# jtschwar/tomo_TV

Measured on AMD Instinct MI355X. Metric: SART+TV Gvoxel-updates/s (ASD-POCS outer iterations x voxels, 512x512x512 x 90 tilts, at 1/2/4/8 GPU), higher is better.
Workload: dtype f32; 1 GPU; ASD-POCS iteration (SART sweep beta0=0.25 + 10 TV-GD steps) on ONE 512x512x512 volume, 90 tilts -70..70 deg (headline SART+TV 512^3x90 = BASELINE configs[2] shape), 512 slices on rank 0; volume=512x512x512, slices_per_gpu=512, nray=512, nproj=90, sub_slab_engines_per_gpu=1, sart_chains_per_engine=1

## Files before the change

### tomo_tv_amd/csrc/engine_api.inc

```


const char *tomo_last_error(void) { return g_err.c_str(); }

int tomo_device_count(int *count)
{
    if (!count) return fail(TOMO_ERR_ARG, "null count");
    int n = 0;
    hipError_t err = hipGetDeviceCount(&n);
    if (err != hipSuccess) { n = 0; (void)hipGetLastError(); }
    *count = n;
    return TOMO_OK;
}

int tomo_system_matrix(int nray, int nproj, const double *angles_rad, int64_t cap, float *rows, float *cols,
                       float *vals, int64_t *nnz)
{
    if (!angles_rad || !nnz) return fail(TOMO_ERR_ARG, "null argument");
    int rc = check_dims(1, nray, nproj);
    if (rc) return rc;
    Coo m;
    build_parallel_ray(nray, nproj, angles_rad, m);
    *nnz = m.ptr[m.nrow];
    if (cap == 0) return TOMO_OK;
    if (cap < *nnz || !rows || !cols || !vals) return fail(TOMO_ERR_ARG, "output capacity too small");
    for (int64_t r = 0; r < m.nrow; ++r)
        for (int64_t k = m.ptr[r]; k < m.ptr[r + 1]; ++k) { rows[k] = (float)r; cols[k] = (float)m.col[k]; vals[k] = m.val[k]; }
    return TOMO_OK;
}

int tomo_create(int nslice, int nray, int nproj, const double *angles_rad, int device, tomo_engine **out)
{
    if (!angles_rad || !out) return fail(TOMO_ERR_ARG, "null argument");
    int rc = check_dims(nslice, nray, nproj);
    if (rc) return rc;
    tomo_engine *e = new_engine(nslice, nray, nproj, device);
    const double t_begin = std::chrono::duration<double>(std::chrono::steady_clock::now().time_since_epoch()).count();
    e->angles.assign(angles_rad, angles_rad + nproj);
    Coo m;
    build_parallel_ray(nray, nproj, angles_rad, m);
    return finish_create(e, m, out, t_begin);
}

int tomo_create_from_matrix(int nslice, int nray, int nproj, int64_t nnz, const float *rows, const float *cols,
                            const float *vals, int device, tomo_engine **out)
{
    if (!rows || !cols || !vals || !out) return fail(TOMO_ERR_ARG, "null argument");
    int rc = check_dims(nslice, nray, nproj);
    if (rc) return rc;
    const double t_begin = std::chrono::duration<double>(std::chrono::steady_clock::now().time_since_epoch()).count();
    Coo m;
    std::string err;
    if (!coo_from_triplets((int64_t)nray * nproj, (int64_t)nray * nray, nnz, rows, cols, vals, m, err))
        return fail(TOMO_ERR_ARG, err);
    tomo_engine *e = new_engine(nslice, nray, nproj, device);
    return finish_create(e, m, out, t_begin);
}

static void free_geometry(tomo_engine *e)
{
    e->pool.release_life(GEOMETRY);
    e->rs_ok = false; e->rs_angs_cap = 0; e->rs_angs_host.clear(); e->seg_ready = false;
    e->pdhg_begun = false;
    e->yk_claim.valid = false;
    e->g_prev_valid = e->mom_p_ok = e->mom.set = false;
    e->geometry_released = true;
}

int tomo_destroy(tomo_engine *e)
{
    if (!e) return TOMO_OK;
    (void)hipSetDevice(e->device);
    if (e->stream) (void)hipStreamSynchronize(e->stream);
    if (e->aux) { (void)hipStreamSynchronize(e->aux); (void)hipStreamDestroy(e->aux); (void)hipEventDestroy(e->ev_fork); (void)hipEventDestroy(e->ev_join); }
    for (int u = 0; u < tomo_engine::MAX_CHAINS; ++u) if (e->sub_stream[u]) { (void)hipStreamSynchronize(e->sub_stream[u]); (void)hipStreamDestroy(e->sub_stream[u]); (void)hipEventDestroy(e->ev_sjoin[u]); }
    for (int w = 0; w < 2; ++w) if (e->fp_red_stream[w]) { (void)hipStreamSynchronize(e->fp_red_stream[w]); (void)hipStreamDestroy(e->fp_red_stream[w]); for (int h = 0; h < 2; ++h) { (void)hipEventDestroy(e->ev_fp_tile[w][h]); (void)hipEventDestroy(e->ev_fp_red[w][h]); } }
    comm_release(e);
    if (e->ev_sfork) (void)hipEventDestroy(e->ev_sfork);
    if (e->ev_peer) (void)hipEventDestroy(e->ev_peer);
    if (e->ev_snap) (void)hipEventDestroy(e->ev_snap);
    if (e->h_snap) (void)hipHostFree(e->h_snap);
    if (e->rs_abort) (void)hipHostFree(e->rs_abort);
    if (e->rs_done) (void)hipHostFree(e->rs_done);
    e->pool.release_all();
    for (auto &p : e->prof) { for (auto ev : p.ev) (void)hipEventDestroy(ev); if (p.ref) (void)hipEventDestroy(p.ref); }
    if (e->own_stream && e->stream) (void)hipStreamDestroy(e->stream);
    delete e;
    return TOMO_OK;
}

int tomo_release_geometry(tomo_engine *e)
{
    NEED(e);
    HIPCHK(hipStreamSynchronize(e->stream));
    if (e->aux) HIPCHK(hipStreamSynchronize(e->aux));
    for (int u = 0; u < tomo_engine::MAX_CHAINS; ++u) if (e->sub_stream[u]) HIPCHK(hipStreamSynchronize(e->sub_stream[u]));
    e->async_pending = false;
    free_geometry(e);
    return TOMO_OK;
}

int tomo_adopt_volumes(tomo_engine *dst, tomo_engine *src)
{
    if (!dst || !src) return fail(TOMO_ERR_ARG, "null engine");
    if (dst->nx != src->nx || dst->n != src->n || dst->sx != src->sx || dst->device != src->device) return fail(TOMO_ERR_ARG, "engines differ in slab shape or device");
    HIPCHK(hipSetDevice(dst->device));
    HIPCHK(hipStreamSynchronize(src->stream));
    if (src->aux) HIPCHK(hipStreamSynchronize(src->aux));
    for (int u = 0; u < tomo_engine::MAX_CHAINS; ++u) if (src->sub_stream[u]) HIPCHK(hipStreamSynchronize(src->sub_stream[u]));
    src->async_pending = false;
    HIPCHK(hipStreamSynchronize(dst->stream));
    for (int i = 0; i < TOMO_VOL_SLOTS; ++i) {
        if (!src->vol[i]) continue;
        if (dst->vol[i] && dst->pool.release(dst->vol[i])) return fail(TOMO_ERR_STATE, "a volume of the adopting engine is not its own");
        if (src->pool.move_to(dst->pool, src->vol[i], (void **)&dst->vol[i])) return fail(TOMO_ERR_STATE, "a volume of the adopted engine is not its own");
        src->vol[i] = nullptr;
    }
    dst->old_is_recon = src->old_is_recon;
    src->old_is_recon = false;
    for (int i = 0; i < TOMO_VOL_SLOTS; ++i) ++dst->vol_version[i];
    g_clear(dst);
    return TOMO_OK;
}

int tomo_set_stream(tomo_engine *e, void *hip_stream)
{
    NEED(e);
    HIPCHK(hipStreamSynchronize(e->stream));
    if (e->own_stream) { HIPCHK(hipStreamDestroy(e->stream)); e->own_stream = false; }
    e->stream = (hipStream_t)hip_stream;
    return TOMO_OK;
}

int tomo_synchronize(tomo_engine *e) { NEED(e); HIPCHK(hipStreamSynchronize(e->stream)); return TOMO_OK; }
int tomo_get_device(tomo_engine *e, int *device) { if (!e || !device) return fail(TOMO_ERR_ARG, "null"); *device = e->device; return TOMO_OK; }
int tomo_get_dims(tomo_engine *e, int *nslice, int *nray, int *nproj, int64_t *nnz)
{
    if (!e) return fail(TOMO_ERR_ARG, "null engine");
    if (nslice) *nslice = e->nx;
    if (nray) *nray = e->n;
    if (nproj) *nproj = e->np;
    if (nnz) *nnz = e->nnz;
    return TOMO_OK;
}

int tomo_sart_chain_count(tomo_engine *e, int *count)
{
    if (!e || !count) return fail(TOMO_ERR_ARG, "null");
    *count = chain_count(e);
    return TOMO_OK;
}

static int upload(tomo_engine *e, const float *host, float *dst, int64_t m)
{
    size_t bytes = (size_t)e->nx * m * sizeof(float);
    int rc = ensure_stage(e, bytes);
    if (rc) return rc;
    HIPCHK(hipMemcpyAsync(e->stage, host, bytes, hipMemcpyHostToDevice, e->stream));
    dim3 grid((unsigned)((m + 31) / 32), (unsigned)((e->sx + 31) / 32)), block(256);
    hipLaunchKernelGGL(k_transpose_in, grid, block, 0, e->stream, e->stage, dst, e->nx, m, e->sx);
    LAUNCHCHK();
    HIPCHK(hipStreamSynchronize(e->stream));
    return TOMO_OK;
}

static int download(tomo_engine *e, const float *src, float *host, int64_t m)
{
    size_t bytes = (size_t)e->nx * m * sizeof(float);
    int rc = ensure_stage(e, bytes);
    if (rc) return rc;
    dim3 grid((unsigned)((m + 31) / 32), (unsigned)((e->sx + 31) / 32)), block(256);
    hipLaunchKernelGGL(k_transpose_out, grid, block, 0, e->stream, src, e->stage, e->nx, m, e->sx);
    LAUNCHCHK();
    HIPCHK(hipMemcpyAsync(host, e->stage, bytes, hipMemcpyDeviceToHost, e->stream));
    HIPCHK(hipStreamSynchronize(e->stream));
    return TOMO_OK;
}

int tomo_set_sinogram(tomo_engine *e, int which, const float *b)
{
    NEED(e);
    if (!b) return fail(TOMO_ERR_ARG, "null sinogram");
    float *dst; int rc = sino_slot(e, which, &dst); if (rc) return rc;
    return upload(e, b, dst, e->nrows);
}

int tomo_set_tilt_series(tomo_engine *e, const float *b) { return tomo_set_sinogram(e, TOMO_SINO_B, b); }

int tomo_get_sinogram(tomo_engine *e, int which, float *out)
{
    NEED(e);
    if (!out) return fail(TOMO_ERR_ARG, "null output");
    if (which == TOMO_SINO_YK_MODEL) {
        const float *yk = projection_in_hand(e, TOMO_VOL_YK);
        if (!yk) return fail(TOMO_ERR_STATE, "no projection of the extrapolated point in hand (tomo_fista_project_yk)");
        return download(e, yk, out, e->nrows);
    }
    float *src;
    int rc = sino_slot(e, which, &src);
    if (rc) return rc;
    return download(e, src, out, e->nrows);
}

int tomo_set_volume(tomo_engine *e, int vol, const float *data)
{
    NEED(e);
    { int rc_ = order_after_async(e); if (rc_) return rc_; }
    float *dst; int rc = get_vol(e, vol, &dst); if (rc) return rc;
    if (!data) return fail(TOMO_ERR_ARG, "null volume");
    return upload(e, data, dst, e->npix);
}

int tomo_get_volume(tomo_engine *e, int vol, float *data)
{
    NEED(e);
    float *src; int rc = get_vol_ro(e, vol, &src); if (rc) return rc;
    if (!data) return fail(TOMO_ERR_ARG, "null volume");
    return download(e, src, data, e->npix);
}

int tomo_set_slice(tomo_engine *e, int vol, int s, const float *img)
{
    NEED(e);
    { int rc_ = order_after_async(e); if (rc_) return rc_; }
    float *dst; int rc = get_vol(e, vol, &dst); if (rc) return rc;
    if (s < 0 || s >= e->nx || !img) return fail(TOMO_ERR_ARG, "slice index out of range");
    if ((rc = ensure_stage(e, e->npix * sizeof(float)))) return rc;
    HIPCHK(hipMemcpyAsync(e->stage, img, e->npix * sizeof(float), hipMemcpyHostToDevice, e->stream));
    hipLaunchKernelGGL(k_scatter_slice, dim3((unsigned)((e->npix + 255) / 256)), dim3(256), 0, e->stream, e->stage, dst, e->npix, e->sx, s);
    LAUNCHCHK();
    HIPCHK(hipStreamSynchronize(e->stream));
    return TOMO_OK;
}

int tomo_get_slice(tomo_engine *e, int vol, int s, float *img)
{
    NEED(e);
    float *src; int rc = get_vol_ro(e, vol, &src); if (rc) return rc;
    if (s < 0 || s >= e->nx || !img) return fail(TOMO_ERR_ARG, "slice index out of range");
    if ((rc = ensure_stage(e, e->npix * sizeof(float)))) return rc;
    hipLaunchKernelGGL(k_gather_slice, dim3((unsigned)((e->npix + 255) / 256)), dim3(256), 0, e->stream, src, e->stage, e->npix, e->sx, s);
    LAUNCHCHK();
    HIPCHK(hipMemcpyAsync(img, e->stage, e->npix * sizeof(float), hipMemcpyDeviceToHost, e->stream));
    HIPCHK(hipStreamSynchronize(e->stream));
    return TOMO_OK;
}

int tomo_restart_recon(tomo_engine *e)
{
    NEED(e);
    { int rc_ = order_after_async(e); if (rc_) return rc_; }
    HIPCHK(hipMemsetAsync(e->vol[TOMO_VOL_RECON], 0, e->vol_elems() * sizeof(float), e->stream));
    if (e->vol[TOMO_VOL_YK]) HIPCHK(hipMemsetAsync(e->vol[TOMO_VOL_YK], 0, e->vol_elems() * sizeof(float), e->stream));
    if (e->vol[TOMO_VOL_RECON_OLD]) HIPCHK(hipMemsetAsync(e->vol[TOMO_VOL_RECON_OLD], 0, e->vol_elems() * sizeof(float), e->stream));
    e->old_is_recon = false;
    ++e->vol_version[TOMO_VOL_RECON]; ++e->vol_version[TOMO_VOL_YK]; ++e->vol_version[TOMO_VOL_RECON_OLD];
    return TOMO_OK;
}

int tomo_copy_volume(tomo_engine *e, int dst, int src)
{
    NEED(e);
    { int rc_ = order_after_async(e); if (rc_) return rc_; }
    float *d, *s; int rc;
    const bool g_src = g_is_projection_of(e, src);
    if ((rc = get_vol(e, dst, &d)) || (rc = get_vol_ro(e, src, &s))) return rc;
    if (d != s) HIPCHK(hipMemcpyAsync(d, s, e->vol_elems() * sizeof(float), hipMemcpyDeviceToDevice, e->stream));
    if (g_src && dst != src) { e->g_valid[1].vol = dst; e->g_valid[1].ver = e->vol_version[dst]; }
    return TOMO_OK;
}

int tomo_forward_projection(tomo_engine *e, int vol, int sino)
{
    NEED(e);
    { int rc_ = order_after_async(e); if (rc_) return rc_; }
    float *x, *g; int rc;
    if ((rc = get_vol_ro(e, vol, &x))) return rc;
    if ((rc = sino_slot(e, sino, &g))) return rc;
    if ((rc = launch_fp_all<FP_STORE>(e, x, nullptr, g))) return rc;
    if (sino == TOMO_SINO_G) g_set(e, vol);
    return TOMO_OK;
}

int tomo_back_projection(tomo_engine *e, int sino, int vol)
{
    NEED(e);
    float *x, *g; int rc;
    if ((rc = get_vol(e, vol, &x))) return rc;
    if ((rc = sino_slot(e, sino, &g))) return rc;
    return launch_bp_all(e, x, g, nullptr, 0.f, 1.f, 0);
}

int tomo_lipschitz(tomo_engine *e, float *L) { if (!e || !L) return fail(TOMO_ERR_ARG, "null"); *L = e->lipschitz; return TOMO_OK; }
int tomo_lipschitz_cimmino(tomo_engine *e, float *L) { if (!e || !L) return fail(TOMO_ERR_ARG, "null"); *L = e->lipschitz_cimmino; return TOMO_OK; }
int tomo_row_inner_product(tomo_engine *e) { if (!e) return fail(TOMO_ERR_ARG, "null engine"); return TOMO_OK;  }

int tomo_sirt_landweber(tomo_engine *e, int vol, float beta, int niter)
{
    NEED(e);
    float *x, *r; int rc;
    if ((rc = get_vol(e, vol, &x)) || (rc = get_sino(e, &e->sino[TOMO_SINO_R], &r))) return rc;
    for (int it = 0; it < niter; ++it) {
        if ((rc = launch_fp_all<FP_RESID>(e, x, e->sino[TOMO_SINO_B], r))) return rc;
        if ((rc = launch_bp_all(e, x, r, nullptr, 1.f, beta, 1))) return rc;
    }
    return TOMO_OK;
}

int tomo_sirt_cimmino(tomo_engine *e, int vol, float beta, int niter)
{
    NEED(e);
    float *x, *r; int rc;
    if ((rc = get_vol(e, vol, &x)) || (rc = get_sino(e, &e->sino[TOMO_SINO_R], &r))) return rc;
    for (int it = 0; it < niter; ++it) {
        if ((rc = launch_fp_all<FP_RESID_MUL>(e, x, e->sino[TOMO_SINO_B], r, e->d_rowinner))) return rc;
        if ((rc = launch_bp_all(e, x, r, nullptr, 1.f, beta / (float)e->nrows, 1))) return rc;
    }
    return TOMO_OK;
}

int tomo_sirt(tomo_engine *e, int vol, int niter) { return tomo_sirt_data(e, vol, TOMO_SINO_B, niter); }

int tomo_sirt_data(tomo_engine *e, int vol, int sino_b, int niter)
{
    NEED(e);
    float *x, *r, *b; int rc;
    const float *have = (niter > 0 && sino_b != TOMO_SINO_G) ? projection_in_hand(e, vol) : nullptr;
    const bool reuse = have != nullptr;
    if (reuse) { if ((rc = order_after_async(e))) return rc; }
    if ((rc = get_vol(e, vol, &x)) || (rc = get_sino(e, &e->sino[TOMO_SINO_R], &r)) || (rc = sino_slot(e, sino_b, &b))) return rc;
    for (int it = 0; it < niter; ++it) {
        if (it == 0 && reuse) { if ((rc = launch_sino_resid<FP_RESID_NORM>(e, b, have, r))) return rc; }
        else if ((rc = launch_fp_all<FP_RESID_NORM>(e, x, b, r))) return rc;
        if ((rc = launch_bp_all(e, x, r, e->d_colsum_all, 1.f, 1.f, 1))) return rc;
    }
    return TOMO_OK;
}

static std::mutex g_rs_mu;
static hipEvent_t g_rs_last[64] = {};

static int launch_sart_resident(tomo_engine *e, float *x, float beta, int64_t steps, const std::function<int(int64_t)> &angle_at, float *track,
                                std::vector<std::pair<int, int>> &failed)
{
    failed.clear();
    if (steps > (int64_t)1 << 24) return fail(TOMO_ERR_ARG, "too many SART steps in one call");
    const Chunks all = chunks64(e, whole(e));
    const int c0 = all.c0, nc = all.n;
    const int groups = std::max(1, std::min(e->rs_groups, nc)), rounds = (nc + groups - 1) / groups;
    {
        std::vector<int> seq((size_t)steps);
        for (int64_t k = 0; k < steps; ++k) seq[(size_t)k] = angle_at(k);
        if (seq != e->rs_angs_host) {
            HIPCHK(hipStreamSynchronize(e->stream));
            if ((size_t)steps > e->rs_angs_cap) {
                if (e->d_rs_angs) { e->pool.release(e->d_rs_angs); e->rs_angs_cap = 0; }
                if (int rc = dev_alloc(e, GEOMETRY, (void **)&e->d_rs_angs, (size_t)steps * sizeof(int), false)) return rc;
                e->rs_angs_cap = (size_t)steps;
            }
            HIPCHK(hipMemcpy(e->d_rs_angs, seq.data(), (size_t)steps * sizeof(int), hipMemcpyHostToDevice));
            e->rs_angs_host.swap(seq);
        }
    }
    const uint64_t need = (uint64_t)rounds * (uint64_t)steps;
    if ((uint64_t)e->rs_epoch + need + 16 > 0xFFFFFFFFull) {
        HIPCHK(hipMemsetAsync(e->rs_pb, 0, e->rs_pb_bytes, e->stream));
        HIPCHK(hipMemsetAsync(e->rs_rb, 0, e->rs_rb_bytes, e->stream));
        e->rs_epoch = 0;
    }
    if (c0 != 0 || nc != e->sxc / 64) return fail(TOMO_ERR_STATE, "the resident sweep covers the whole slab");
    if (e->rs_commit_dirty || e->rs_commit_base > 0x7F000000u) {
        HIPCHK(hipMemsetAsync(e->d_rs_commit, 0, (size_t)(e->sxc / 64) * sizeof(unsigned), e->stream));
        e->rs_commit_base = 0; e->rs_commit_dirty = false;
    }
    if (++e->rs_seq >= 0x7FFFFFF0u) { std::memset(e->rs_done, 0, (size_t)(e->sxc / 64) * sizeof(int)); e->rs_seq = 1; }
    RsArgs A{};
    A.x = x; A.b = e->cur_b; A.rowsum = e->d_rowsum; A.hdr = e->d_rs_hdr; A.cell = e->d_rs_cell; A.ts = e->d_rs_ts; A.rl = e->d_rs_rl;
    A.pb = e->rs_pb; A.rb = e->rs_rb; A.angs = e->d_rs_angs; A.track = track; A.part = e->d_part; A.abort_word = e->d_rs_abort; A.abort_host = e->rs_abort;
    A.commit = e->d_rs_commit; A.done_host = e->rs_done; A.seq = e->rs_seq; A.commit_base = e->rs_commit_base; A.test_fail = e->rs_test_fail;
    A.n = e->n; A.sx = e->sx; A.np = e->np; A.ntiles = e->rs_ntiles; A.tiles = e->rs_tiles; A.rpt = e->rs_rpt; A.steps = (int)steps; A.chunk0 = c0; A.nchunk = nc;
    A.epoch0 = e->rs_epoch; A.spin_limit = e->rs_spin_limit; A.beta = beta; A.prof = nullptr;
    e->rs_epoch += (uint32_t)need;
    if (e->device < 0 || e->device >= 64) return fail(TOMO_ERR_ARG, "device index");
    {
        std::lock_guard<std::mutex> lk(g_rs_mu);
        hipEvent_t &last = g_rs_last[e->device];
        if (!last) HIPCHK(hipEventCreateWithFlags(&last, hipEventDisableTiming));
        else HIPCHK(hipStreamWaitEvent(e->stream, last, 0));
        {
            ProfScope ps(e, TOMO_K_SART_RESIDENT);
            hipLaunchKernelGGL(k_sart_resident, dim3((unsigned)(e->rs_ntiles * groups)), dim3(RS_THREADS), 0, e->stream, A);
            LAUNCHCHK();
        }
        HIPCHK(hipEventRecord(last, e->stream));
    }
    HIPCHK(hipStreamSynchronize(e->stream));
    int nfailed = 0;
    for (int c = c0; c < c0 + nc; ++c) {
        if (e->rs_done[c] == (int)e->rs_seq) continue;
        ++nfailed;
        if (!failed.empty() && failed.back().first + failed.back().second == c) ++failed.back().second;
        else failed.emplace_back(c, 1);
    }
    if (nfailed) {
        e->rs_commit_dirty = true;
        e->rs_last_code = *e->rs_abort;
        *e->rs_abort = 0;
        HIPCHK(hipMemsetAsync(e->d_rs_abort, 0, sizeof(int), e->stream));
        ++e->rs_fallbacks;
        e->rs_fallback_chunks += nfailed;
        e->rs_backoff = std::min(64, std::max(1, 2 * e->rs_backoff));
        e->rs_skip = e->rs_backoff;
    } else {
        e->rs_commit_base += (unsigned)e->rs_ntiles;
        e->rs_backoff = 0;
    }
    return TOMO_OK;
}

int tomo_sart(tomo_engine *e, int vol, float beta, int niter, const int32_t *order)
{
    return tomo_sart_data(e, vol, TOMO_SINO_B, beta, niter, order);
}

static int sart_impl(tomo_engine *e, int vol, int sino_b, float beta, int niter, const int32_t *order, int track_vol, int slot)
{
    NEED(e);
    float *x, *r, *track = nullptr; int rc;
    if ((rc = get_vol(e, vol, &x)) || (rc = get_sino(e, &e->sino[TOMO_SINO_R], &r)) || (rc = sino_slot(e, sino_b, &e->cur_b))) return rc;
    if (track_vol >= 0) {
        if (track_vol == vol) return fail(TOMO_ERR_ARG, "the tracked volume must differ from the swept one");
        if (slot < 0 || slot >= TOMO_S_COUNT) return fail(TOMO_ERR_ARG, "bad scalar slot");
        if ((rc = get_vol(e, track_vol, &track))) return rc;
        if ((int64_t)niter * e->np <= 0) {
            if ((rc = tomo_diff_norm_sq(e, vol, track_vol, slot))) return rc;
            return tomo_copy_volume(e, track_vol, vol);
        }
        if ((rc = reduce_begin(e))) return rc;
    }
    auto finish = [&]() -> int { return track ? reduce_end(e, slot) : TOMO_OK; };
    if (order) {
        std::vector<char> seen(e->np, 0);
        for (int q = 0; q < e->np; ++q) {
            if (order[q] < 0 || order[q] >= e->np || seen[order[q]]) return fail(TOMO_ERR_ARG, "SART order is not a permutation of the angles");
            seen[order[q]] = 1;
        }
    }
    const int64_t steps = (int64_t)niter * e->np;
    auto angle_at = [&](int64_t k) { int q = (int)(k % e->np); return order ? order[q] : q; };
    if (!e->sart_fused) {
        for (int64_t k = 0; k < steps; ++k) {
            int i = angle_at(k);
            {
                ProfScope ps(e, TOMO_K_FP_ANGLE);
                if ((rc = launch_fp<FP_RESID_NORM>(e, x, i * e->n, e->n, e->cur_b, r))) return rc;
            }
            if ((rc = launch_bp_angle(e, x, i, r + (size_t)i * e->n * e->sx, beta, k == steps - 1 ? track : nullptr))) return rc;
        }
        return finish();
    }
    if (steps <= 0) return TOMO_OK;
    int form = select_forms(e).sart;
    if (form == TOMO_FORM_SART_RESIDENT && e->rs_skip > 0 && e->sart_resident != 1) {
        --e->rs_skip;
        form = TOMO_FORM_SART_TILE;
    }
    auto sweep_tiles = [&](const std::vector<std::pair<int, int>> *ranges) -> int {
        const bool coop = e->sart_coop && e->np >= 2 && steps >= 2 && !ranges;
        int rc2;
        if ((rc2 = sart_tile_prepare(e, coop))) return rc2;
        const uint32_t epoch0 = e->st_epoch + 1;
        if (coop) e->st_epoch += (uint32_t)(steps + 1);
        auto link = [&](int64_t k, const Sub &sb) -> int {
            int rc3;
            if (coop) {
                float *pk = (k & 1) ? e->st_partial2 : e->st_partial, *pk1 = (k & 1) ? e->st_partial : e->st_partial2;
                if (k == 0) return launch_sart_tile<false>(e, sb, x, 0, angle_at(0), r, beta, pk, false);
                if (k == steps) {
                    int last = angle_at(steps - 1);
                    if ((rc3 = launch_resid_finish_tile(e, sb, pk1, last, r))) return rc3;
                    return launch_bp_angle(e, sb, x, last, r + (size_t)last * e->n * e->sx, beta, track);
                }
                return launch_sart_coop(e, sb, x, angle_at(k - 1), angle_at(k), r, beta, pk1, pk, epoch0 + (uint32_t)k, k);
            }
            if (k == 0) return launch_sart_tile<false>(e, sb, x, 0, angle_at(0), r, beta);
            if (k == steps) { int last = angle_at(steps - 1); return launch_bp_angle(e, sb, x, last, r + (size_t)last * e->n * e->sx, beta, track); }
            int prev = angle_at(k - 1), next = angle_at(k);
            if (prev == next) {
                if ((rc3 = launch_bp_angle(e, sb, x, prev, r + (size_t)prev * e->n * e->sx, beta))) return rc3;
                return launch_sart_tile<false>(e, sb, x, 0, next, r, beta);
            }
            return launch_sart_tile<true>(e, sb, x, prev, next, r, beta, nullptr, true, k);
        };
        auto chain = [&](const Sub &sb) -> int {
            for (int64_t k = 0; k <= steps; ++k) { int rc3 = link(k, sb); if (rc3) return rc3; }
            return TOMO_OK;
        };
        if (!ranges) return run_chains(e, chain);
        for (const auto &rg : *ranges) {
            const int c0 = rg.first, nc = rg.second;
            const int vec = (c0 % 4 == 0 && nc % 4 == 0) ? 4 : (c0 % 2 == 0 && nc % 2 == 0) ? 2 : 1;
            if ((rc2 = chain(Sub{e->stream, c0, nc, vec}))) return rc2;
        }
        return TOMO_OK;
    };
    if (form == TOMO_FORM_SART_RESIDENT) {
        std::vector<std::pair<int, int>> failed;
        if ((rc = launch_sart_resident(e, x, beta, steps, angle_at, track, failed))) return rc;
        if (!failed.empty() && (rc = sweep_tiles(&failed))) return rc;
        return finish();
    }
    if (e->sart_resident == 1 && !e->rs_ok) return fail(TOMO_ERR_STATE, "\"sart_resident\" = 1, but this engine has no tables of the resident sweep (N not a multiple of 8, more 32 x 32 tiles than CUs, or a matrix whose ray windows do not fit)");
    if (form == TOMO_FORM_SART_TILE) {
        if ((rc = sweep_tiles(nullptr))) return rc;
        return finish();
    }
    float *alt;
    if ((rc = ensure_seg_tables(e))) return rc;
    if ((rc = get_scratch(e, &e->sart_alt, &alt))) return rc;
    float *cur = x;
    if ((rc = launch_sart_seg<false>(e, cur, nullptr, 0, angle_at(0), r, beta))) return rc;
    for (int64_t k = 1; k < steps; ++k) {
        int prev = angle_at(k - 1), next = angle_at(k);
        if (prev == next) {
            if ((rc = launch_bp_angle(e, cur, prev, r + (size_t)prev * e->n * e->sx, beta))) return rc;
            if ((rc = launch_fp<FP_RESID_NORM>(e, cur, next * e->n, e->n, e->cur_b, r))) return rc;
            continue;
        }
        if ((rc = launch_sart_seg<true>(e, cur, alt, prev, next, r, beta))) return rc;
        std::swap(cur, alt);
    }
    int last = angle_at(steps - 1);
    if ((rc = launch_bp_angle(e, cur, last, r + (size_t)last * e->n * e->sx, beta, track))) return rc;
    if (cur != x) { e->vol[vol] = cur; e->sart_alt = x; }
    return finish();
}

int tomo_sart_data(tomo_engine *e, int vol, int sino_b, float beta, int niter, const int32_t *order)
{
    return sart_impl(e, vol, sino_b, beta, niter, order, -1, 0);
}

int tomo_sart_tracked(tomo_engine *e, int vol, int sino_b, float beta, int niter, const int32_t *order, int track_vol, int slot)
{
    return sart_impl(e, vol, sino_b, beta, niter, order, track_vol, slot);
}

int tomo_art(tomo_engine *e, float beta) { return tomo_art_order(e, beta, nullptr); }

int tomo_art_order(tomo_engine *e, float beta, const int32_t *order_host)
{
    NEED(e);
    float *x;
    { int rc_ = get_vol(e, TOMO_VOL_RECON, &x); if (rc_) return rc_; }
    int32_t *d_order = nullptr;
    if (order_host) {
        std::vector<char> seen(e->nrows, 0);
        for (int64_t q = 0; q < e->nrows; ++q) {
            if (order_host[q] < 0 || order_host[q] >= e->nrows || seen[order_host[q]]) return fail(TOMO_ERR_ARG, "row order is not a permutation");
            seen[order_host[q]] = 1;
        }
        int rc = ensure_stage(e, e->nrows * sizeof(int32_t)); if (rc) return rc;
        HIPCHK(hipMemcpyAsync(e->stage, order_host, e->nrows * sizeof(int32_t), hipMemcpyHostToDevice, e->stream));
        d_order = (int32_t *)e->stage;
    }
    if (!order_host && e->art_chain && e->art_chain_ok) {
        float *d, *a; int rc;
        if ((rc = get_sino(e, &e->sino[TOMO_SINO_G], &d)) || (rc = get_sino(e, &e->sino[TOMO_SINO_R], &a))) return rc;
        const float *b = e->sino[TOMO_SINO_B];
        if (e->art_tile && e->sart_tile && e->st_ok && e->np >= 1) {
            if ((rc = sart_tile_prepare(e, false))) return rc;
            e->cur_b = const_cast<float *>(b);
            const int np = e->np;
            auto chain = [&](const Sub &sb) -> int {
                const Chunks ch = chunks64(e, sb);
                for (int i = 0; i < np; ++i) {
                    int rc2 = i == 0 ? launch_sart_tile<false, true>(e, sb, x, 0, 0, a, beta, nullptr, true, -1, d)
                                     : launch_sart_tile<true, true>(e, sb, x, i - 1, i, a, beta, nullptr, true, i, d);
                    if (rc2) return rc2;
                    hipLaunchKernelGGL(k_art_chain, dim3((unsigned)ch.n), dim3(64 * ART_CW), 0, sb.stream, d, b, e->d_rowinner, e->d_rowcross, a, beta, i * e->n, e->n, e->sx, ch.c0);
                    LAUNCHCHK();
                }
                return launch_bp_art(e, sb, x, np - 1, a, beta);
            };
            if ((rc = run_chains(e, chain))) return rc;
            return tomo_positivity(e, TOMO_VOL_RECON);
        }
        for (int i = 0; i < e->np; ++i) {
            if ((rc = launch_fp<FP_STORE>(e, x, i * e->n, e->n, nullptr, d))) return rc;
            hipLaunchKernelGGL(k_art_chain, dim3((unsigned)(e->sx / 64)), dim3(64 * ART_CW), 0, e->stream, d, b, e->d_rowinner, e->d_rowcross, a, beta, i * e->n, e->n, e->sx, 0);
            LAUNCHCHK();
            if ((rc = launch_bp_art(e, whole(e), x, i, a, beta))) return rc;
        }
        return tomo_positivity(e, TOMO_VOL_RECON);
    }
    hipLaunchKernelGGL(k_art, dim3(e->sxc / 64), dim3(64 * ART_WAVES), 0, e->stream, x, e->d_rptr, e->d_rent, e->sino[TOMO_SINO_B], e->d_rowinner, beta, (int)e->nrows, e->sx, d_order);
    LAUNCHCHK();
    int rc = tomo_positivity(e, TOMO_VOL_RECON);
    if (!rc && order_host) HIPCHK(hipStreamSynchronize(e->stream));
    return rc;
}

int tomo_poisson_ml(tomo_engine *e, float lambda)
{
    int rc;
    if ((rc = tomo_poisson_residual(e, TOMO_VOL_RECON, TOMO_SINO_B, TOMO_SINO_R))) return rc;
    float *x;
    if ((rc = get_vol(e, TOMO_VOL_RECON, &x))) return rc;
    return launch_bp_all(e, x, e->sino[TOMO_SINO_R], nullptr, 1.f, -(lambda / e->lipschitz), 1);
}

int tomo_poisson_residual(tomo_engine *e, int vol, int sino_b, int sino_out)
{
    NEED(e);
    float *x, *b, *r; int rc;
    if ((rc = get_vol(e, vol, &x)) || (rc = sino_slot(e, sino_b, &b)) || (rc = sino_slot(e, sino_out, &r))) return rc;
    if ((rc = reduce_begin(e))) return rc;
    if ((rc = launch_fp_all<FP_POISSON>(e, x, b, r))) return rc;
    return reduce_end(e, TOMO_S_COST);
}

static int slice_sumsq(tomo_engine *e, const float *v, int64_t m, double *sums)
{
    const int cols = e->sx / 4, per = cols >= 256 ? 256 : (cols >= 128 ? 128 : 64);
    const int nby = (int)std::min<int64_t>(1024, std::max<int64_t>(1, (m + 63) / 64));
    const int rpb = (int)((m + nby - 1) / nby);
    if (!e->cg_part) { int rc = dev_alloc(e, ENGINE, (void **)&e->cg_part, (size_t)1024 * e->sx * sizeof(double), false); if (rc) return rc; }
    dim3 grid((unsigned)((cols + per - 1) / per), (unsigned)nby);
    hipLaunchKernelGGL(k_slice_sumsq, grid, dim3(256), 0, e->stream, v, e->cg_part, m, e->sx, rpb);
    LAUNCHCHK();
    hipLaunchKernelGGL(k_slice_sumsq_finish, dim3((e->sx + 255) / 256), dim3(256), 0, e->stream, (const double *)e->cg_part, sums, nby, e->sx);
    LAUNCHCHK();
    return TOMO_OK;
}

static unsigned slice_grid(const tomo_engine *e, int64_t n4)
{
    const int64_t unit = std::max(1, e->sx / 64);
    int64_t b = std::min<int64_t>((n4 + 255) / 256, 8192);
    b = std::max<int64_t>(unit, (b / unit) * unit);
    return (unsigned)b;
}

int tomo_cgls(tomo_engine *e, int vol, int niter)
{
    NEED(e);
    float *x, *r, *b, *w; int rc;
    const bool reuse_g = g_is_projection_of(e, vol);
    if (reuse_g) { if ((rc = order_after_async(e))) return rc; }
    if ((rc = get_vol(e, vol, &x)) || (rc = get_sino(e, &e->sino[TOMO_SINO_R], &r)) || (rc = sino_slot(e, TOMO_SINO_B, &b))) return rc;
    if ((rc = get_scratch(e, &e->cg_p, &w)) || (rc = get_scratch(e, &e->cg_z, &w))) return rc;
    if ((rc = get_sino(e, &e->cg_w, &w))) return rc;
    if (!e->cg_sums) { if ((rc = dev_alloc(e, ENGINE, (void **)&e->cg_sums, 2 * e->sx * sizeof(double), true))) return rc; }
    if (!e->cg_coef) { if ((rc = dev_alloc(e, ENGINE, (void **)&e->cg_coef, e->sx * sizeof(float), true))) return rc; }
    double *gam = e->cg_sums, *tmp = e->cg_sums + e->sx;
    const int64_t nv = (int64_t)e->vol_elems(), ns = (int64_t)e->sino_elems();
    auto ratio = [&](const double *num, const double *den) {
        hipLaunchKernelGGL(k_slice_ratio, dim3((e->sx + 255) / 256), dim3(256), 0, e->stream, num, den, e->cg_coef, e->sx);
    };
    if (reuse_g) { if ((rc = launch_sino_resid<FP_RESID>(e, b, e->sino[TOMO_SINO_G], r))) return rc; }
    else if ((rc = launch_fp_all<FP_RESID>(e, x, b, r))) return rc;
    if ((rc = launch_bp_all(e, e->cg_z, r, nullptr, 0.f, 1.f, 0))) return rc;
// ... 21 lines not shown
    if (!taps_host) return fail(TOMO_ERR_ARG, "null filter");
    float *x, *b, *g; int rc;
    if ((rc = get_vol(e, TOMO_VOL_RECON, &x)) || (rc = sino_slot(e, TOMO_SINO_B, &b)) || (rc = get_sino(e, &e->sino[TOMO_SINO_R], &g))) return rc;
    if (!e->fbp_h) { if ((rc = dev_alloc(e, GEOMETRY, (void **)&e->fbp_h, e->n * sizeof(float), false))) return rc; }
    HIPCHK(hipMemcpyAsync(e->fbp_h, taps_host, e->n * sizeof(float), hipMemcpyHostToDevice, e->stream));
    HIPCHK(hipStreamSynchronize(e->stream));
    int nchunk = e->sxc / (64 * e->vec);
    int64_t waves = e->nrows * nchunk;
    dim3 grid((unsigned)((waves + 3) / 4)), block(256);
    with_vec(e->vec, [&](auto V) {
        hipLaunchKernelGGL((k_filter_rows<V()>), grid, block, 0, e->stream, b, g, e->fbp_h, e->n, (int)e->nrows, e->sx, nchunk);
    });
    LAUNCHCHK();
    return launch_bp_all(e, x, g, nullptr, 0.f, scale, apply_positivity ? 1 : 0);
}

int tomo_scale_volume(tomo_engine *e, int vol, float factor)
{
    NEED(e);
    { int rc_ = order_after_async(e); if (rc_) return rc_; }
    float *x; int rc; if ((rc = get_vol(e, vol, &x))) return rc;
    int64_t n4 = e->vol_elems() / 4;
    hipLaunchKernelGGL(k_scale, dim3(grid_1d(n4)), dim3(256), 0, e->stream, (f4 *)x, factor, n4);
    LAUNCHCHK();
    return TOMO_OK;
}

int tomo_sino_diff_norm_sq(tomo_engine *e, int a, int b, int slot)
{
    NEED(e);
    if (slot < 0 || slot >= TOMO_S_COUNT) return fail(TOMO_ERR_ARG, "bad scalar slot");
    float *pa, *pb; int rc;
    if ((rc = sino_slot(e, a, &pa)) || (rc = sino_slot(e, b, &pb))) return rc;
    if ((rc = reduce_begin(e))) return rc;
    int64_t n4 = e->sino_elems() / 4;
    hipLaunchKernelGGL(k_sqdiff, dim3(grid_1d(n4)), dim3(256), 0, e->stream, (const f4 *)pa, (const f4 *)pb, e->d_part, n4);
    LAUNCHCHK();
    return reduce_end(e, slot);
}

int tomo_sino_proj_max(tomo_engine *e, int sino, float *out_host)
{
    NEED(e);
    float *g; int rc; if ((rc = sino_slot(e, sino, &g))) return rc;
    if (!out_host) return fail(TOMO_ERR_ARG, "null output");
    if ((rc = ensure_stage(e, e->np * sizeof(float)))) return rc;
    hipLaunchKernelGGL(k_proj_max, dim3(e->np), dim3(256), 0, e->stream, g, e->stage, e->n, e->nx, e->sx);
    LAUNCHCHK();
    HIPCHK(hipMemcpyAsync(out_host, e->stage, e->np * sizeof(float), hipMemcpyDeviceToHost, e->stream));
    HIPCHK(hipStreamSynchronize(e->stream));
    return TOMO_OK;
}

int tomo_sino_proj_scale(tomo_engine *e, int sino, const float *div_host, const float *mul_host)
{
    NEED(e);
    float *g; int rc; if ((rc = sino_slot(e, sino, &g))) return rc;
    if (!div_host || !mul_host) return fail(TOMO_ERR_ARG, "null factors");
    if ((rc = ensure_stage(e, 2 * e->np * sizeof(float)))) return rc;
    HIPCHK(hipMemcpyAsync(e->stage, div_host, e->np * sizeof(float), hipMemcpyHostToDevice, e->stream));
    HIPCHK(hipMemcpyAsync(e->stage + e->np, mul_host, e->np * sizeof(float), hipMemcpyHostToDevice, e->stream));
    hipLaunchKernelGGL(k_proj_scale, dim3(e->np), dim3(256), 0, e->stream, g, e->stage, e->n, e->sx);
    LAUNCHCHK();
    HIPCHK(hipStreamSynchronize(e->stream));
    return TOMO_OK;
}

int tomo_copy_volume_from(tomo_engine *dst, int dst_vol, tomo_engine *src, int src_vol)
{
    if (!dst || !src) return fail(TOMO_ERR_ARG, "null engine");
    if (dst->nx != src->nx || dst->n != src->n || dst->sx != src->sx || dst->device != src->device) return fail(TOMO_ERR_ARG, "engines differ in slab shape or device");
    HIPCHK(hipSetDevice(dst->device));
    float *d, *s; int rc;
    if ((rc = get_vol(dst, dst_vol, &d)) || (rc = get_vol(src, src_vol, &s))) return rc;
    HIPCHK(hipStreamSynchronize(src->stream));
    HIPCHK(hipMemcpyAsync(d, s, dst->vol_elems() * sizeof(float), hipMemcpyDeviceToDevice, dst->stream));
    HIPCHK(hipStreamSynchronize(dst->stream));
    return TOMO_OK;
}

int tomo_get_stream(tomo_engine *e, void **out) { if (!e || !out) return fail(TOMO_ERR_ARG, "null"); *out = (void *)e->stream; return TOMO_OK; }

static int mm_check(tomo_engine *a, tomo_engine *b, int nel)
{
    if (!a || !b) return fail(TOMO_ERR_ARG, "null engine");
    if (a->nx != b->nx || a->n != b->n || a->sx != b->sx || a->device != b->device) return fail(TOMO_ERR_ARG, "engines differ in slab shape or device");
    if (a->stream != b->stream) return fail(TOMO_ERR_STATE, "engines must share one stream (tomo_set_stream)");
    if (nel < 1 || nel > MM_MAX_EL) return fail(TOMO_ERR_ARG, "element count out of range");
    return TOMO_OK;
}

int tomo_mm_model(tomo_engine *ce, const int32_t *xvols, int nel, const float *w, float gamma, tomo_engine *he, int model_vol)
{
    int rc = mm_check(ce, he, nel); if (rc) return rc;
    HIPCHK(hipSetDevice(ce->device));
    MMArgs a{};
    a.nel = nel; a.gamma = gamma;
    for (int i = 0; i < nel; ++i) { float *p; if ((rc = get_vol(ce, xvols[i], &p))) return rc; a.x[i] = p; a.w[i] = w[i]; }
    float *m; if ((rc = get_vol(he, model_vol, &m))) return rc;
    int64_t n4 = ce->vol_elems() / 4;
    hipLaunchKernelGGL(k_mm_model, dim3(grid_1d(n4)), dim3(256), 0, ce->stream, a, (f4 *)m, n4);
    LAUNCHCHK();
    return TOMO_OK;
}

int tomo_mm_update(tomo_engine *ce, const int32_t *xvols, const int32_t *uvols, int nel, const float *w, float gamma,
                   float lamC_over_L, float lamH, tomo_engine *he, int upd_vol, int model_vol)
{
    int rc = mm_check(ce, he, nel); if (rc) return rc;
    HIPCHK(hipSetDevice(ce->device));
    MMArgs a{};
    a.nel = nel; a.gamma = gamma;
    for (int i = 0; i < nel; ++i) {
        float *p, *u;
        if ((rc = get_vol(ce, xvols[i], &p)) || (rc = get_vol(ce, uvols[i], &u))) return rc;
        a.x[i] = p; a.u[i] = u; a.w[i] = w[i];
    }
    float *upd = nullptr, *m = nullptr;
    if (lamH != 0.f) { if ((rc = get_vol(he, upd_vol, &upd)) || (rc = get_vol(he, model_vol, &m))) return rc; }
    int64_t n4 = ce->vol_elems() / 4;
    hipLaunchKernelGGL(k_mm_update, dim3(grid_1d(n4)), dim3(256), 0, ce->stream, a, (const f4 *)upd, (const f4 *)m, lamC_over_L, lamH, n4);
    LAUNCHCHK();
    return TOMO_OK;
}

int tomo_positivity(tomo_engine *e, int vol)
{
    NEED(e);
    { int rc_ = order_after_async(e); if (rc_) return rc_; }
    float *x; int rc; if ((rc = get_vol(e, vol, &x))) return rc;
    int64_t n4 = e->vol_elems() / 4;
    hipLaunchKernelGGL(k_clamp, dim3(grid_1d(n4)), dim3(256), 0, e->stream, (f4 *)x, n4);
    LAUNCHCHK();
    return TOMO_OK;
}

int tomo_soft_threshold(tomo_engine *e, int vol, float lambda)
{
    NEED(e);
    float *x; int rc; if ((rc = get_vol(e, vol, &x))) return rc;
    int64_t n4 = e->vol_elems() / 4;
    hipLaunchKernelGGL(k_soft_threshold, dim3(grid_1d(n4)), dim3(256), 0, e->stream, (f4 *)x, lambda, n4);
    LAUNCHCHK();
    return TOMO_OK;
}

int tomo_fista_momentum(tomo_engine *e, float beta)
{
    NEED(e);
    { int rc_ = order_after_async(e); if (rc_) return rc_; }
    e->mom_p_ok = e->g_prev_valid && e->mom.set && e->vol_version[TOMO_VOL_RECON] == e->mom.ver_recon
                  && e->vol_version[TOMO_VOL_RECON_OLD] == e->mom.ver_old && e->g_prev_recon_ver == e->vol_version[TOMO_VOL_RECON];
    float *x, *yk, *old; int rc;
    const bool aliased = e->old_is_recon;
    if ((rc = get_vol_ro(e, TOMO_VOL_RECON, &x)) || (rc = get_vol_ro(e, TOMO_VOL_YK, &yk))) return rc;
    if (aliased) old = x;
    else if ((rc = get_vol_ro(e, TOMO_VOL_RECON_OLD, &old))) return rc;
    int64_t n4 = e->vol_elems() / 4;
    hipLaunchKernelGGL(k_momentum, dim3(grid_1d(n4)), dim3(256), 0, e->stream, (const f4 *)yk, (const f4 *)old, (f4 *)x, beta, n4);
    LAUNCHCHK();
    ++e->vol_version[TOMO_VOL_RECON]; ++e->vol_version[TOMO_VOL_YK]; ++e->vol_version[TOMO_VOL_RECON_OLD];
    e->vol[TOMO_VOL_RECON] = yk;
    e->vol[TOMO_VOL_YK] = x;
    e->old_is_recon = true;
    e->mom.beta = beta; e->mom.set = true;
    e->mom.ver_recon = e->vol_version[TOMO_VOL_RECON]; e->mom.ver_yk = e->vol_version[TOMO_VOL_YK]; e->mom.ver_old = e->vol_version[TOMO_VOL_RECON_OLD];
    return TOMO_OK;
}

int tomo_fista_project_yk(tomo_engine *e, int *done)
{
    NEED(e);
    if (done) *done = 0;
    if (!e->fp_reuse || !g_is_projection_of(e, TOMO_VOL_RECON) || !e->mom.set) return TOMO_OK;
    if (e->vol_version[TOMO_VOL_RECON] != e->mom.ver_recon || e->vol_version[TOMO_VOL_YK] != e->mom.ver_yk) return TOMO_OK;
    { int rc_ = order_after_async(e); if (rc_) return rc_; }
    int rc; float *p, *q;
    if ((rc = get_sino(e, &e->g_prev, &p)) || (rc = get_sino(e, &e->g_yk, &q))) return rc;
    const float *g = e->sino[TOMO_SINO_G];
    const int64_t n4 = (int64_t)e->sino_elems() / 4;
    const bool have_prev = e->mom_p_ok;
    e->yk_claim.valid = false;
    if (have_prev) {
        hipLaunchKernelGGL(k_sino_extrapolate, dim3(grid_1d(n4)), dim3(256), 0, e->stream, (const VecOf<4>::T *)g, (VecOf<4>::T *)p, (VecOf<4>::T *)q, e->mom.beta, n4);
        LAUNCHCHK();
    } else {
        HIPCHK(hipMemcpyAsync(p, g, e->sino_elems() * sizeof(float), hipMemcpyDeviceToDevice, e->stream));
    }
    e->g_prev_valid = true;
    e->g_prev_recon_ver = e->vol_version[TOMO_VOL_RECON];
    if (have_prev) {
        e->yk_claim.valid = true; e->yk_claim.ver = e->vol_version[TOMO_VOL_YK];
        if (done) *done = 1;
    } else if (e->mom.beta == 0.f) {
        e->g_valid[1].vol = TOMO_VOL_YK; e->g_valid[1].ver = e->vol_version[TOMO_VOL_YK];
        if (done) *done = 1;
    }
    return TOMO_OK;
}

int tomo_data_distance_sq(tomo_engine *e, int vol)
{
    NEED(e);
    float *x, *g; int rc;
    if ((rc = get_vol_ro(e, vol, &x)) || (rc = get_sino(e, &e->sino[TOMO_SINO_G], &g))) return rc;
    if ((rc = reduce_begin(e))) return rc;
    if ((rc = launch_fp_all<FP_DD>(e, x, e->sino[TOMO_SINO_B], g))) return rc;
    g_set(e, vol);
    return reduce_end(e, TOMO_S_DD);
}

int tomo_data_distance_sq_async(tomo_engine *e, int vol)
{
    NEED(e);
    if (e->async_pending) return fail(TOMO_ERR_STATE, "an asynchronous evaluation is already in flight");
    if (!e->aux) {
        HIPCHK(hipStreamCreateWithFlags(&e->aux, hipStreamNonBlocking));
        HIPCHK(hipEventCreateWithFlags(&e->ev_fork, hipEventDisableTiming));
        HIPCHK(hipEventCreateWithFlags(&e->ev_join, hipEventDisableTiming));
        if (int rc = dev_alloc(e, ENGINE, (void **)&e->d_part_aux, NPART * sizeof(double), true)) return rc;
    }
    float *tmp; int rc;
    if ((rc = get_vol_ro(e, vol, &tmp)) || (rc = get_sino(e, &e->sino[TOMO_SINO_G], &tmp))) return rc;
    HIPCHK(hipEventRecord(e->ev_fork, e->stream));
    HIPCHK(hipStreamWaitEvent(e->aux, e->ev_fork, 0));
    hipStream_t main_stream = e->stream;
    double *main_part = e->d_part;
    e->stream = e->aux; e->d_part = e->d_part_aux;
    rc = tomo_data_distance_sq(e, vol);
    e->stream = main_stream; e->d_part = main_part;
    if (rc) return rc;
    HIPCHK(hipEventRecord(e->ev_join, e->aux));
    e->async_pending = true;
    return TOMO_OK;
}

int tomo_async_wait(tomo_engine *e)
{
    NEED(e);
    if (e->async_pending) {
        HIPCHK(hipStreamWaitEvent(e->stream, e->ev_join, 0));
        e->async_pending = false;
    }
    return TOMO_OK;
}

int tomo_diff_norm_sq(tomo_engine *e, int a, int b, int slot)
{
    NEED(e);
    if (slot < 0 || slot >= TOMO_S_COUNT) return fail(TOMO_ERR_ARG, "bad scalar slot");
    float *pa, *pb; int rc;
    if ((rc = get_vol_ro(e, a, &pa)) || (rc = get_vol_ro(e, b, &pb))) return rc;
    if ((rc = reduce_begin(e))) return rc;
    int64_t n4 = e->vol_elems() / 4;
    hipLaunchKernelGGL(k_sqdiff, dim3(grid_1d(n4)), dim3(256), 0, e->stream, (const f4 *)pa, (const f4 *)pb, e->d_part, n4);
    LAUNCHCHK();
    return reduce_end(e, slot);
}

int tomo_l1_norm(tomo_engine *e, int vol)
{
    NEED(e);
    float *x; int rc; if ((rc = get_vol_ro(e, vol, &x))) return rc;
    if ((rc = reduce_begin(e))) return rc;
    int64_t n4 = e->vol_elems() / 4;
    hipLaunchKernelGGL(k_l1, dim3(grid_1d(n4)), dim3(256), 0, e->stream, (const f4 *)x, e->d_part, n4);
    LAUNCHCHK();
    return reduce_end(e, TOMO_S_L1);
}

int tomo_read_scalars(tomo_engine *e, double *out, int count)
{
    NEED(e);
    if (!out || count < 0 || count > TOMO_S_COUNT) return fail(TOMO_ERR_ARG, "bad scalar count");
    { int rc = tomo_async_wait(e); if (rc) return rc; }
    HIPCHK(hipMemcpyAsync(out, e->d_scal, count * sizeof(double), hipMemcpyDeviceToHost, e->stream));
    HIPCHK(hipStreamSynchronize(e->stream));
    return TOMO_OK;
}

int tomo_scalars_snapshot(tomo_engine *e)
{
    NEED(e);
    { int rc = tomo_async_wait(e); if (rc) return rc; }
    if (!e->h_snap) {
        HIPCHK(hipHostMalloc((void **)&e->h_snap, TOMO_S_COUNT * sizeof(double), hipHostMallocDefault));
        HIPCHK(hipEventCreateWithFlags(&e->ev_snap, hipEventDisableTiming));
    }
    hipLaunchKernelGGL(k_scalars_to_host, dim3(1), dim3(64), 0, e->stream, (const double *)e->d_scal, e->h_snap, (int)TOMO_S_COUNT);
    LAUNCHCHK();
    HIPCHK(hipEventRecord(e->ev_snap, e->stream));
    e->snap_pending = true;
    return TOMO_OK;
}

int tomo_scalars_snapshot_read(tomo_engine *e, double *out, int count)
{
    NEED(e);
    if (!out || count < 0 || count > TOMO_S_COUNT) return fail(TOMO_ERR_ARG, "bad scalar count");
    if (!e->snap_pending) return fail(TOMO_ERR_STATE, "no scalar snapshot in flight");
    HIPCHK(hipEventSynchronize(e->ev_snap));
    std::memcpy(out, e->h_snap, count * sizeof(double));
    e->snap_pending = false;
    return TOMO_OK;
}

// ... 8 lines not shown
```

### tomo_tv_amd/csrc/engine_options.inc

```

int tomo_get_option(tomo_engine *e, const char *name, int *value)
{
    if (!e || !name || !value) return fail(TOMO_ERR_ARG, "null argument");
    if (std::strcmp(name, "fp_strip") == 0) { *value = e->fp_strip; return TOMO_OK; }
    if (std::strcmp(name, "fp_strip_ready") == 0) { *value = e->fs_ok ? 1 : 0; return TOMO_OK; }
    if (std::strcmp(name, "fp_strip_slots") == 0) { *value = e->fs_ok ? e->fs_kused : 0; return TOMO_OK; }
    if (std::strcmp(name, "fp_tile") == 0) { *value = e->fp_tile; return TOMO_OK; }
    if (std::strcmp(name, "bp_tile") == 0) { *value = e->bp_tile; return TOMO_OK; }
    if (std::strcmp(name, "bp_list") == 0) { *value = e->bp_list; return TOMO_OK; }
    if (std::strcmp(name, "fgp_pair") == 0) { *value = e->fgp_pair; return TOMO_OK; }
    if (std::strcmp(name, "fp_list") == 0) { *value = e->fp_list; return TOMO_OK; }
    if (std::strcmp(name, "fp_list_ready") == 0) { *value = e->fl_ok ? 1 : 0; return TOMO_OK; }
    if (std::strcmp(name, "bp_list_ready") == 0) { *value = e->bl_ok ? 1 : 0; return TOMO_OK; }
    if (std::strcmp(name, "fp_reuse") == 0) { *value = e->fp_reuse; return TOMO_OK; }
    if (std::strcmp(name, "art_chain_ready") == 0) { *value = e->art_chain_ok ? 1 : 0; return TOMO_OK; }
    if (std::strcmp(name, "sart_tile") == 0) { *value = e->sart_tile; return TOMO_OK; }
    if (std::strcmp(name, "sart_resident") == 0) { *value = e->sart_resident; return TOMO_OK; }
    if (std::strcmp(name, "sart_resident_ready") == 0) { *value = e->rs_ok ? 1 : 0; return TOMO_OK; }
    if (std::strcmp(name, "sart_resident_active") == 0) { *value = (e->rs_ok && e->sart_resident != 0) ? 1 : 0; return TOMO_OK; }
    if (std::strcmp(name, "sart_resident_spin") == 0) { *value = (int)std::min<uint32_t>(e->rs_spin_limit, 0x7FFFFFFFu); return TOMO_OK; }
    if (std::strcmp(name, "sart_resident_fallbacks") == 0) { *value = e->rs_fallbacks; return TOMO_OK; }
    if (std::strcmp(name, "sart_resident_fallback_chunks") == 0) { *value = e->rs_fallback_chunks; return TOMO_OK; }
    if (std::strcmp(name, "sart_resident_skip") == 0) { *value = e->rs_skip; return TOMO_OK; }
    if (std::strcmp(name, "sart_resident_last_code") == 0) { *value = e->rs_last_code; return TOMO_OK; }
    if (std::strcmp(name, "table_kib") == 0) { *value = (int)std::min<size_t>(e->table_bytes >> 10, 0x7FFFFFFF); return TOMO_OK; }
    if (std::strcmp(name, "create_ms") == 0) { *value = (int)std::min(e->create_ms + 0.5, 2147483647.0); return TOMO_OK; }
    if (std::strcmp(name, "tv_halo_fold") == 0) { *value = e->tv_halo_fold; return TOMO_OK; }
    if (std::strcmp(name, "form_fp") == 0) { *value = select_forms(e).fp; return TOMO_OK; }
    if (std::strcmp(name, "form_bp") == 0) { *value = select_forms(e).bp; return TOMO_OK; }
    if (std::strcmp(name, "form_sart") == 0) { *value = select_forms(e).sart; return TOMO_OK; }
    if (std::strcmp(name, "rccl_version") == 0) { *value = g_rccl.version; return TOMO_OK; }
    if (std::strcmp(name, "comm_rounds") == 0) { *value = (int)std::min<int64_t>(e->comm_rounds, 0x7FFFFFFF); return TOMO_OK; }
    return fail(TOMO_ERR_ARG, std::string("unknown option ") + name);
}

int tomo_set_option(tomo_engine *e, const char *name, int value)
{
    if (!e || !name) return fail(TOMO_ERR_ARG, "null argument");
    if (std::strcmp(name, "fgp_fused") == 0) { e->fgp_fused = value ? 1 : 0; return TOMO_OK; }
    if (std::strcmp(name, "fgp_pair") == 0) { e->fgp_pair = value ? 1 : 0; return TOMO_OK; }
    if (std::strcmp(name, "sart_fused") == 0) { e->sart_fused = value ? 1 : 0; return TOMO_OK; }
    if (std::strcmp(name, "fp_all_lpr") == 0) { e->fp_all_lpr = (value == 16 || value == 32) ? value : 0; return TOMO_OK; }
    if (std::strcmp(name, "art_chain") == 0) { e->art_chain = value ? 1 : 0; return TOMO_OK; }
    if (std::strcmp(name, "sart_tile") == 0) { e->sart_tile = value ? 1 : 0; return TOMO_OK; }
    if (std::strcmp(name, "sart_resident") == 0) { e->sart_resident = value < 0 ? -1 : (value ? 1 : 0); e->rs_skip = e->rs_backoff = 0; return TOMO_OK; }
    if (std::strcmp(name, "sart_resident_spin") == 0) { e->rs_spin_limit = value < 0 ? (1u << 21) : (uint32_t)value; return TOMO_OK; }
    if (std::strcmp(name, "sart_resident_test_fail") == 0) { e->rs_test_fail = std::max(0, value); return TOMO_OK; }
    if (std::strcmp(name, "fp_reuse") == 0) { e->fp_reuse = value != 0; g_clear(e); e->yk_claim.valid = false; return TOMO_OK; }
    if (std::strcmp(name, "fp_tile_pipe") == 0) { e->fp_tile_pipe = std::max(0, value); return TOMO_OK; }
    if (std::strcmp(name, "sart_streams") == 0) { e->sart_streams = value >= 2 ? std::min(value, (int)tomo_engine::MAX_CHAINS) : (value == 1 ? 1 : 0); return TOMO_OK; }
    if (std::strcmp(name, "art_tile") == 0) { e->art_tile = value ? 1 : 0; return TOMO_OK; }
    if (std::strcmp(name, "sart_skip_same") == 0) { e->sart_skip_same = value ? 1 : 0; return TOMO_OK; }
    if (std::strcmp(name, "sart_nt") == 0) { e->sart_nt = value < 0 ? -1 : (value ? 1 : 0); return TOMO_OK; }
    if (std::strcmp(name, "sart_coop") == 0) { e->sart_coop = value ? 1 : 0; return TOMO_OK; }
    if (std::strcmp(name, "sart_coop_spin") == 0) { e->sart_coop_spin = value < 0 ? -1 : value; return TOMO_OK; }
    if (std::strcmp(name, "bp_tile") == 0) { e->bp_tile = value ? 1 : 0; return TOMO_OK; }
    if (std::strcmp(name, "bp_list") == 0) { e->bp_list = value ? 1 : 0; return TOMO_OK; }
    if (std::strcmp(name, "bp_list_band") == 0) { e->bp_list_band = value ? 1 : 0; return TOMO_OK; }
    if (std::strcmp(name, "fp_list") == 0) { e->fp_list = value ? 1 : 0; return TOMO_OK; }
    if (std::strcmp(name, "fp_strip") == 0) { e->fp_strip = value ? 1 : 0; return TOMO_OK; }
    if (std::strcmp(name, "fp_tile") == 0) { e->fp_tile = value ? 1 : 0; e->fp_strip = 0; return TOMO_OK; }
    if (std::strcmp(name, "fp_tile_chunks_per_pass") == 0) {
        if (value < 0 || e->ft_part || e->ft_part_aux || e->fs_part || e->fs_part_aux || e->fl_part || e->fl_part_aux) return fail(TOMO_ERR_STATE, "fp_tile_chunks_per_pass must be set before the first projection");
        e->ft_ncp_forced = value; e->ft_ncp = 0; e->fs_ncp = 0; e->fl_ncp = 0; return TOMO_OK;
    }
    if (std::strcmp(name, "fp_tile_scratch_mib") == 0) {
        if (value <= 0 || e->ft_part || e->ft_part_aux || e->fs_part || e->fs_part_aux || e->fl_part || e->fl_part_aux) return fail(TOMO_ERR_STATE, "fp_tile_scratch_mib must be positive and set before the first projection");
        e->ft_scratch_cap = (size_t)value << 20; e->ft_ncp = 0; e->fs_ncp = 0; e->fl_ncp = 0; return TOMO_OK;
    }
    if (std::strcmp(name, "tv_gnorm_slot") == 0) {
        if (value < 0 || value >= TOMO_S_COUNT) return fail(TOMO_ERR_ARG, "bad scalar slot");
        e->gnorm_slot = value; return TOMO_OK;
    }
    if (std::strcmp(name, "tv_tz") == 0) { e->tv_tz = value == 4 ? 4 : 8; return TOMO_OK; }
    if (std::strcmp(name, "tv_halo_fold") == 0) { e->tv_halo_fold = value < 0 ? -1 : (value ? 1 : 0); return TOMO_OK; }
    if (std::strcmp(name, "tv_march4") == 0) { e->tv_march4 = value ? 1 : 0; return TOMO_OK; }
    if (std::strcmp(name, "tv_yseg") == 0) { e->tv_yseg = value < 0 ? 0 : value; return TOMO_OK; }
    if (std::strcmp(name, "tv_recompute") == 0) { e->tv_recompute = value ? 1 : 0; return TOMO_OK; }
    if (std::strcmp(name, "tv_lds") == 0) { e->tv_lds = value; return TOMO_OK; }
    return fail(TOMO_ERR_ARG, std::string("unknown option ") + name);
}

int tomo_profile_enable(tomo_engine *e, int kernel, int on)
{
    NEED(e);
    if (kernel < 0 || kernel >= PROF_MAX_KERNELS) return fail(TOMO_ERR_ARG, "bad kernel id");
    HIPCHK(hipStreamSynchronize(e->stream));
    e->prof[kernel].on = on != 0;
    e->prof[kernel].stride = on > 1 ? (unsigned)on : 1u;
    e->prof[kernel].seen = 0;
    e->prof[kernel].used = 0;
    e->prof[kernel].dropped = 0;
    if (on) {
        if (!e->prof[kernel].ref) HIPCHK(hipEventCreate(&e->prof[kernel].ref));
        HIPCHK(hipEventRecord(e->prof[kernel].ref, e->stream));
    }
    return TOMO_OK;
}

int tomo_profile_read2(tomo_engine *e, int kernel, int64_t *launches, double *total_ms, double *busy_ms)
{
    NEED(e);
    if (kernel < 0 || kernel >= PROF_MAX_KERNELS || !launches || !total_ms) return fail(TOMO_ERR_ARG, "bad argument");
    HIPCHK(hipStreamSynchronize(e->stream));
    for (int u = 0; u < tomo_engine::MAX_CHAINS; ++u) if (e->sub_stream[u]) HIPCHK(hipStreamSynchronize(e->sub_stream[u]));
    if (e->aux) HIPCHK(hipStreamSynchronize(e->aux));
    ProfSlot &p = e->prof[kernel];
    double tot = 0;
    std::vector<std::pair<float, float>> iv;
    for (size_t i = 0; i + 1 < p.used; i += 2) {
        float ms = 0;
        HIPCHK(hipEventElapsedTime(&ms, p.ev[i], p.ev[i + 1]));
        tot += ms;
        if (busy_ms && p.ref) {
            float t0 = 0;
            HIPCHK(hipEventElapsedTime(&t0, p.ref, p.ev[i]));
            iv.emplace_back(t0, t0 + ms);
        }
    }
    if (busy_ms) {
        std::sort(iv.begin(), iv.end());
        double busy = 0; float cur_a = 0, cur_b = -1;
        for (auto &q : iv) {
            if (cur_b < cur_a || q.first > cur_b) { if (cur_b >= cur_a) busy += cur_b - cur_a; cur_a = q.first; cur_b = q.second; }
            else cur_b = std::max(cur_b, q.second);
        }
        if (cur_b >= cur_a) busy += cur_b - cur_a;
        *busy_ms = busy;
    }
    *launches = (int64_t)(p.used / 2);
    *total_ms = tot;
    p.used = 0;
    if (p.dropped) {
        std::string msg = std::to_string(p.dropped) + " launches were not recorded (event log full)";
        p.dropped = 0;
        return fail(TOMO_ERR_STATE, msg);
    }
    return TOMO_OK;
}

int tomo_profile_intervals(tomo_engine *e, int kernel, tomo_engine *ref_engine, double *t0, double *t1, int cap, int *count)
{
    NEED(e);
    if (kernel < 0 || kernel >= PROF_MAX_KERNELS || !ref_engine || !count) return fail(TOMO_ERR_ARG, "bad argument");
    HIPCHK(hipStreamSynchronize(e->stream));
    ProfSlot &p = e->prof[kernel];
    hipEvent_t ref = ref_engine->prof[kernel].ref;
    if (!ref) return fail(TOMO_ERR_STATE, "the reference engine's log is not enabled");
    int n = (int)(p.used / 2);
    *count = n;
    if (!t0 || !t1 || cap < n) return cap == 0 ? TOMO_OK : fail(TOMO_ERR_ARG, "interval buffers too small");
    for (int i = 0; i < n; ++i) {
        float a = 0, d = 0;
        HIPCHK(hipEventElapsedTime(&a, ref, p.ev[2 * i]));
        HIPCHK(hipEventElapsedTime(&d, p.ev[2 * i], p.ev[2 * i + 1]));
        t0[i] = a; t1[i] = a + d;
    }
    return TOMO_OK;
}

int tomo_profile_read(tomo_engine *e, int kernel, int64_t *launches, double *total_ms)
{
    return tomo_profile_read2(e, kernel, launches, total_ms, nullptr);
}
```

### tomo_tv_amd/csrc/engine_tv.inc

```

static int field_ptr(tomo_engine *e, int field, float **out)
{
    if (field == TOMO_FIELD_FGP_D) return get_scratch(e, &e->tvg, out);
    if (field == TOMO_FIELD_FGP_P1) return get_scratch(e, &e->fgp_p[0], out);
    return get_vol_ro(e, field, out);
}

int tomo_bind_halo(tomo_engine *e, void *device_lo, void *device_hi)
{
    NEED(e);
    HIPCHK(hipStreamSynchronize(e->stream));
    e->halo_lo = device_lo ? (float *)device_lo : e->halo_lo_own;
    e->halo_hi = device_hi ? (float *)device_hi : e->halo_hi_own;
    return TOMO_OK;
}

int tomo_halo_pack(tomo_engine *e, int field, int last, void *device_dst)
{
    NEED(e);
    float *x; int rc; if ((rc = field_ptr(e, field, &x))) return rc;
    if (!device_dst) return fail(TOMO_ERR_ARG, "null destination");
    hipLaunchKernelGGL(k_halo_pack, dim3((unsigned)((e->npix + 255) / 256)), dim3(256), 0, e->stream, x, (float *)device_dst, (int)e->npix, e->sx, last ? e->nx - 1 : 0);
    LAUNCHCHK();
    return TOMO_OK;
}

int tomo_halo_pack_both(tomo_engine *e, int field, void *first_plane, void *last_plane)
{
    NEED(e);
    float *x; int rc; if ((rc = field_ptr(e, field, &x))) return rc;
    if (!first_plane || !last_plane) return fail(TOMO_ERR_ARG, "null destination");
    hipLaunchKernelGGL(k_halo_wrap, dim3((unsigned)((e->npix + 255) / 256)), dim3(256), 0, e->stream, x, (float *)last_plane, (float *)first_plane, (int)e->npix, e->sx, e->nx);
    LAUNCHCHK();
    return TOMO_OK;
}

int tomo_halo_local(tomo_engine *e, int field)
{
    NEED(e);
    float *x; int rc; if ((rc = field_ptr(e, field, &x))) return rc;
    hipLaunchKernelGGL(k_halo_wrap, dim3((unsigned)((e->npix + 255) / 256)), dim3(256), 0, e->stream, x, e->halo_lo, e->halo_hi, (int)e->npix, e->sx, e->nx);
    LAUNCHCHK();
    return TOMO_OK;
}


int tomo_wait_for(tomo_engine *e, tomo_engine *other)
{
    NEED(e);
    if (!other) return fail(TOMO_ERR_ARG, "null engine");
    if (other->device != e->device) return fail(TOMO_ERR_ARG, "engines on different devices");
    if (other == e || other->stream == e->stream) return TOMO_OK;
    if (!other->ev_peer) HIPCHK(hipEventCreateWithFlags(&other->ev_peer, hipEventDisableTiming));
    HIPCHK(hipEventRecord(other->ev_peer, other->stream));
    HIPCHK(hipStreamWaitEvent(e->stream, other->ev_peer, 0));
    return TOMO_OK;
}

int tomo_halo_from(tomo_engine *e, int field, tomo_engine *lo_src, tomo_engine *hi_src)
{
    NEED(e);
    if (!lo_src || !hi_src) return fail(TOMO_ERR_ARG, "null engine");
    if (lo_src->n != e->n || hi_src->n != e->n || lo_src->device != e->device || hi_src->device != e->device) return fail(TOMO_ERR_ARG, "engines differ in image size or device");
    float *xl, *xh; int rc;
    if ((rc = field_ptr(lo_src, field, &xl)) || (rc = field_ptr(hi_src, field, &xh))) return rc;
    dim3 grid((unsigned)((e->npix + 255) / 256));
    hipLaunchKernelGGL(k_halo_pack, grid, dim3(256), 0, e->stream, xl, e->halo_lo, (int)e->npix, lo_src->sx, lo_src->nx - 1);
    hipLaunchKernelGGL(k_halo_pack, grid, dim3(256), 0, e->stream, xh, e->halo_hi, (int)e->npix, hi_src->sx, 0);
    LAUNCHCHK();
    return TOMO_OK;
}

int tomo_scalar_sum_from(tomo_engine *e, int dst_slot, tomo_engine **srcs, int n, int src_slot)
{
    NEED(e);
    if (!srcs || n < 1 || n > 8 || dst_slot < 0 || dst_slot >= TOMO_S_COUNT || src_slot < 0 || src_slot >= TOMO_S_COUNT) return fail(TOMO_ERR_ARG, "bad argument");
    SumSrc s{};
    s.n = n;
    for (int i = 0; i < n; ++i) { if (!srcs[i] || srcs[i]->device != e->device) return fail(TOMO_ERR_ARG, "bad source engine"); s.p[i] = srcs[i]->d_scal + src_slot; }
    hipLaunchKernelGGL(k_sum_doubles, dim3(1), dim3(1), 0, e->stream, s, e->d_scal + dst_slot);
    LAUNCHCHK();
    return TOMO_OK;
}

int tomo_set_slab_edges(tomo_engine *e, int is_first, int is_last)
{
    if (!e) return fail(TOMO_ERR_ARG, "null engine");
    e->is_first = is_first ? 1 : 0; e->is_last = is_last ? 1 : 0;
    return TOMO_OK;
}

static int tv_grid(tomo_engine *e)
{
    int64_t items = e->npix * (e->sx / 64);
    return (int)std::min<int64_t>((items + 3) / 4, 256 * 16);
}

int tomo_tv_partial(tomo_engine *e, int vol, float eps)
{
    NEED(e);
    float *x; int rc; if ((rc = get_vol_ro(e, vol, &x))) return rc;
    Halo h{e->halo_lo, e->halo_hi};
    if (e->tv_lds != 8 && e->tv_lds != 1) {
        if ((rc = reduce_begin(e))) return rc;
        hipLaunchKernelGGL(k_tv_value, dim3(tv_grid(e)), dim3(256), 0, e->stream, x, h, e->d_part, eps, e->n, e->nx, e->sx);
        LAUNCHCHK();
        return reduce_end(e, TOMO_S_TV);
    }
    if (!e->d_part_tv) { if ((rc = dev_alloc(e, ENGINE, (void **)&e->d_part_tv, NPART * sizeof(double), true))) return rc; }
    if ((rc = part_begin(e, e->d_part_tv))) return rc;
    const int yseg = 32;
    if (e->tv_lds == 1 && e->tv_march4 && e->nx % 64 == 0 && e->n % 8 == 0) {
        hipLaunchKernelGGL((k_tv_march4<8, true, TVM_VALUE, false>), dim3(tv_march_grid(e->n, 8, e->sxc / 64, (e->n + yseg - 1) / yseg)), dim3(256), 0, e->stream, x, h, (double *)nullptr, eps, e->n, e->nx, e->sx, yseg, e->d_part_tv, TvUpd{});
    } else if (e->tv_lds == 1) {
        hipLaunchKernelGGL((k_tv_grad_reg<8, true, false>), dim3(tv_march_grid(e->n, 8, e->sxc / 64, (e->n + yseg - 1) / yseg)), dim3(256), 0, e->stream, x, h, (float *)nullptr, (double *)nullptr, eps, e->n, e->nx, e->sx, yseg, e->d_part_tv, TvUpd{});
    } else {
        dim3 grid((unsigned)(((e->n + 7) / 8) * (e->sxc / 64)), (unsigned)((e->n + yseg - 1) / yseg));
        hipLaunchKernelGGL((k_tv_grad_lds<8, true, false>), grid, dim3(256), 0, e->stream, x, h, (float *)nullptr, (double *)nullptr, eps, e->n, e->nx, e->sx, yseg, e->d_part_tv);
    }
    LAUNCHCHK();
    return part_end(e, e->d_part_tv, TOMO_S_TV);
}

static int tv_rows_per_wave(const tomo_engine *e, int tz)
{
    if (e->tv_yseg > 0) return e->tv_yseg;
    const int64_t cols = (int64_t)((e->n + tz - 1) / tz) * (e->sxc / 64);
    int yseg = 32;
    while (yseg > TV_YSEG_MIN && cols * ((e->n + yseg - 1) / yseg) < TV_WAVES_WANTED) yseg >>= 1;
    return yseg;
}

static int tv_grad_impl(tomo_engine *e, float eps, bool with_tv, float *g_first = nullptr, float *g_last = nullptr)
{
    NEED(e);
    float *x, *g; int rc;
    if ((rc = get_vol(e, e->tv_target, &x))) return rc;
    if ((rc = get_scratch(e, &e->tvg, &g))) return rc;
    if ((rc = reduce_begin(e))) return rc;
    Halo h{e->halo_lo, e->halo_hi};
    if ((g_first || g_last) && !(e->tv_lds == 1 && e->tv_recompute)) return fail(TOMO_ERR_STATE, "gradient planes need the recompute form of the TV march (tv_lds = 1, tv_recompute = 1)");
    if (with_tv && e->tv_lds != 8 && e->tv_lds != 1) with_tv = false;
    if (with_tv) {
        if (!e->d_part_tv) { if ((rc = dev_alloc(e, ENGINE, (void **)&e->d_part_tv, NPART * sizeof(double), true))) return rc; }
        if ((rc = part_begin(e, e->d_part_tv))) return rc;
    }
    {
        ProfScope ps(e, TOMO_K_TV_GRAD);
        e->tv_last_eps = eps;
        double *part_tv = with_tv ? e->d_part_tv : nullptr;
        if (e->tv_lds == 1 && e->tv_recompute) {
            TvUpd gp{};
            gp.wrap_lo = g_last; gp.wrap_hi = g_first;
            const int tz = e->tv_tz == 4 ? 4 : 8, yseg = tv_rows_per_wave(e, tz);
            dim3 grid(tv_march_grid(e->n, tz, e->sxc / 64, (e->n + yseg - 1) / yseg));
            const bool edge = e->nx % 64 != 0 || e->n % 8 != 0;
            with_flag(with_tv, [&](auto W) {
                if (tz == 8 && e->tv_march4) with_flag(edge, [&](auto E) {
                    hipLaunchKernelGGL((k_tv_march4<8, W(), TVM_NORM, E()>), grid, dim3(256), 0, e->stream, x, h, e->d_part, eps, e->n, e->nx, e->sx, yseg, part_tv, gp);
                });
                else with_int<4, 8>(tz, [&](auto TZ) {
                    hipLaunchKernelGGL((k_tv_grad_reg<TZ(), W(), true, TVM_NORM>), grid, dim3(256), 0, e->stream, x, h, (float *)nullptr, e->d_part, eps, e->n, e->nx, e->sx, yseg, part_tv, gp);
                });
            });
        } else if (e->tv_lds == 1) {
            int yseg = 32;
            dim3 grid(tv_march_grid(e->n, 8, e->sxc / 64, (e->n + yseg - 1) / yseg));
            with_flag(with_tv, [&](auto W) {
                hipLaunchKernelGGL((k_tv_grad_reg<8, W()>), grid, dim3(256), 0, e->stream, x, h, g, e->d_part, eps, e->n, e->nx, e->sx, yseg, part_tv, TvUpd{});
            });
        } else if (e->tv_lds) {
            int yseg = 32;
            if (e->tv_lds == 16) {
                dim3 grid((unsigned)(((e->n + 15) / 16) * (e->sxc / 64)), (unsigned)((e->n + yseg - 1) / yseg));
                hipLaunchKernelGGL((k_tv_grad_lds<16, false>), grid, dim3(256), 0, e->stream, x, h, g, e->d_part, eps, e->n, e->nx, e->sx, yseg, (double *)nullptr);
            } else {
                dim3 grid((unsigned)(((e->n + 7) / 8) * (e->sxc / 64)), (unsigned)((e->n + yseg - 1) / yseg));
                with_flag(with_tv, [&](auto W) {
                    hipLaunchKernelGGL((k_tv_grad_lds<8, W()>), grid, dim3(256), 0, e->stream, x, h, g, e->d_part, eps, e->n, e->nx, e->sx, yseg, part_tv);
                });
            }
        } else {
            hipLaunchKernelGGL(k_tv_grad, dim3(tv_grid(e)), dim3(256), 0, e->stream, x, h, g, e->d_part, eps, e->n, e->nx, e->sx);
        }
    }
    LAUNCHCHK();
    if (with_tv && (rc = part_end(e, e->d_part_tv, TOMO_S_TV))) return rc;
    return reduce_end(e, TOMO_S_GNORM);
}

int tomo_tv_set_target(tomo_engine *e, int vol)
{
    NEED(e);
    float *x;
    int rc = get_vol(e, vol, &x);
    if (rc) return rc;
    e->tv_target = vol;
    return TOMO_OK;
}

int tomo_tv_grad(tomo_engine *e, float eps) { return tv_grad_impl(e, eps, false); }
int tomo_tv_grad_tv(tomo_engine *e, float eps)
{
    if (e && e->tv_lds != 8 && e->tv_lds != 1) {
        int rc = tomo_tv_partial(e, e->tv_target, eps);
        return rc ? rc : tv_grad_impl(e, eps, false);
    }
    return tv_grad_impl(e, eps, true);
}

int tomo_tv_grad_planes(tomo_engine *e, float eps, int with_tv, void *g_first, void *g_last)
{
    if (!g_first || !g_last) return fail(TOMO_ERR_ARG, "null plane buffer");
    return tv_grad_impl(e, eps, with_tv != 0, (float *)g_first, (float *)g_last);
}

int tomo_tv_halo_apply(tomo_engine *e, float dPOCS, int clamp, const void *g_lo, const void *g_hi)
{
    NEED(e);
    if (!g_lo || !g_hi) return fail(TOMO_ERR_ARG, "null plane buffer");
    hipLaunchKernelGGL(k_halo_apply, dim3((unsigned)((e->npix + 255) / 256)), dim3(256), 0, e->stream, e->halo_lo, e->halo_hi,
                       (const float *)g_lo, (const float *)g_hi, gnorm_ptr(e), dPOCS, clamp, (int)e->npix);
    LAUNCHCHK();
    return TOMO_OK;
}

static int halo_other_pair(tomo_engine *e, float **lo, float **hi)
{
    int rc;
    if (!e->halo_lo_alt) {
        if ((rc = dev_alloc(e, ENGINE, (void **)&e->halo_lo_alt, e->npix * sizeof(float), true))) return rc;
        if ((rc = dev_alloc(e, ENGINE, (void **)&e->halo_hi_alt, e->npix * sizeof(float), true))) return rc;
    }
    *lo = e->halo_lo == e->halo_lo_own ? e->halo_lo_alt : e->halo_lo_own;
    *hi = e->halo_hi == e->halo_hi_own ? e->halo_hi_alt : e->halo_hi_own;
    return TOMO_OK;
}

static int tv_update_impl(tomo_engine *e, float dPOCS, int clamp, int track_vol, int slot, bool wrap = false,
                          float *plane_last = nullptr, float *plane_first = nullptr, const float *hg_lo = nullptr, const float *hg_hi = nullptr)
{
    NEED(e);
    float *x, *g, *track = nullptr; int rc;
    if ((rc = get_vol(e, e->tv_target, &x))) return rc;
    if ((rc = get_scratch(e, &e->tvg, &g))) return rc;
    if (track_vol >= 0) {
        if (track_vol == e->tv_target) return fail(TOMO_ERR_ARG, "the tracked volume must differ from the one descended");
        if (slot < 0 || slot >= TOMO_S_COUNT) return fail(TOMO_ERR_ARG, "bad scalar slot");
        if ((rc = get_vol(e, track_vol, &track))) return rc;
        if ((rc = order_after_async(e))) return rc;
        if ((rc = reduce_begin(e))) return rc;
    }
    if (e->tv_lds == 1 && e->tv_recompute) {
        float *alt;
        if ((rc = get_scratch(e, &e->tv_alt, &alt))) return rc;
        const bool own_halo = e->halo_lo == e->halo_lo_own || e->halo_lo == e->halo_lo_alt;
        float *wl = plane_last, *wh = plane_first;
        if (wrap && own_halo && (rc = halo_other_pair(e, &wl, &wh))) return rc;
        Halo h{e->halo_lo, e->halo_hi};
        TvUpd up{alt, gnorm_ptr(e), dPOCS, clamp, track, wl, wh, slab_streams(e) ? 1 : 0, nullptr, nullptr, nullptr, nullptr};
        const bool fold = hg_lo && hg_hi && (e->tv_halo_fold < 0 ? e->sxc >= 128 : e->tv_halo_fold != 0) && own_halo && !wrap && e->tv_tz != 4 && e->tv_march4;
        if (fold) {
            up.hg_lo = hg_lo; up.hg_hi = hg_hi;
            if ((rc = halo_other_pair(e, &up.ho_lo, &up.ho_hi))) return rc;
        }
        {
            ProfScope ps(e, TOMO_K_TV_UPDATE);
            const int tz = e->tv_tz == 4 ? 4 : 8, yseg = tv_rows_per_wave(e, tz);
            dim3 grid(tv_march_grid(e->n, tz, e->sxc / 64, (e->n + yseg - 1) / yseg));
            const bool edge = e->nx % 64 != 0 || e->n % 8 != 0;
            if (tz == 8 && e->tv_march4) with_flag(edge, [&](auto E) { with_flag(track != nullptr, [&](auto T) { with_flag(up.stream != 0, [&](auto S) {
                hipLaunchKernelGGL((k_tv_march4<8, false, TVM_UPDATE, E(), T(), S()>), grid, dim3(256), 0, e->stream, x, h, e->d_part, e->tv_last_eps, e->n, e->nx, e->sx, yseg, (double *)nullptr, up);
            }); }); });
            else with_int<4, 8>(tz, [&](auto TZ) {
                hipLaunchKernelGGL((k_tv_grad_reg<TZ(), false, true, TVM_UPDATE>), grid, dim3(256), 0, e->stream, x, h, (float *)nullptr, e->d_part, e->tv_last_eps, e->n, e->nx, e->sx, yseg, (double *)nullptr, up);
            });
        }
        LAUNCHCHK();
        e->vol[e->tv_target] = alt; e->tv_alt = x;
        if (wrap && own_halo) { e->halo_lo = wl; e->halo_hi = wh; }
        else if (wrap) { if ((rc = tomo_halo_local(e, e->tv_target))) return rc; }
        if (fold) { e->halo_lo = up.ho_lo; e->halo_hi = up.ho_hi; }
        else if (hg_lo && hg_hi && (rc = tomo_tv_halo_apply(e, dPOCS, clamp, hg_lo, hg_hi))) return rc;
        return track ? reduce_end(e, slot) : TOMO_OK;
    }
    int64_t n4 = e->vol_elems() / 4;
    {
        ProfScope ps(e, TOMO_K_TV_UPDATE);
        float *wl = wrap ? e->halo_lo : plane_last, *wh = wrap ? e->halo_hi : plane_first;
        double *part = track ? e->d_part : nullptr;
        with_flag(track != nullptr, [&](auto T) {
            hipLaunchKernelGGL(k_tv_update<T()>, dim3(grid_1d(n4)), dim3(256), 0, e->stream, (f4 *)x, (const f4 *)g, gnorm_ptr(e), dPOCS, clamp, n4, (f4 *)track, part, wl, wh, e->nx, e->sx / 4);
        });
    }
    LAUNCHCHK();
    if (hg_lo && hg_hi && (rc = tomo_tv_halo_apply(e, dPOCS, clamp, hg_lo, hg_hi))) return rc;
    return track ? reduce_end(e, slot) : TOMO_OK;
}

int tomo_tv_update(tomo_engine *e, float dPOCS, int clamp) { return tv_update_impl(e, dPOCS, clamp, -1, 0); }

int tomo_tv_update_planes(tomo_engine *e, float dPOCS, int clamp, void *first_plane, void *last_plane)
{
    if (!first_plane || !last_plane) return fail(TOMO_ERR_ARG, "null plane buffer");
    return tv_update_impl(e, dPOCS, clamp, -1, 0, false, (float *)last_plane, (float *)first_plane);
}

int tomo_tv_update_tracked(tomo_engine *e, float dPOCS, int clamp, int track_vol, int slot)
{
    return tv_update_impl(e, dPOCS, clamp, track_vol, slot);
}

int tomo_fgp_begin(tomo_engine *e) { return tomo_fgp_begin_vol(e, TOMO_VOL_RECON); }

static int fgp_begin_impl(tomo_engine *e, int vol, bool zero_p)
{
    NEED(e);
    float *d, *p; int rc;
    if ((rc = get_vol(e, vol, &d))) return rc;
    e->fgp_target = vol;
    if (zero_p) {
        if ((rc = get_scratch(e, &e->tvg, &d))) return rc;
        HIPCHK(hipMemsetAsync(d, 0, e->vol_elems() * sizeof(float), e->stream));
    }
    for (int i = 0; i < 3; ++i) {
        if ((rc = get_scratch(e, &e->fgp_p[i], &p))) return rc;
        if (zero_p) HIPCHK(hipMemsetAsync(p, 0, e->vol_elems() * sizeof(float), e->stream));
    }
    return TOMO_OK;
}

int tomo_fgp_begin_vol(tomo_engine *e, int vol) { return fgp_begin_impl(e, vol, true); }

int tomo_fgp_obj(tomo_engine *e, float lambda)
{
    NEED(e);
    if (!e->tvg || !e->fgp_p[2]) return fail(TOMO_ERR_STATE, "tomo_fgp_begin has not been called");
    ProfScope ps(e, TOMO_K_FGP_OBJ);
    hipLaunchKernelGGL(k_fgp_obj, dim3(tv_grid(e)), dim3(256), 0, e->stream, e->vol[e->fgp_target], e->tvg, e->fgp_p[0], e->fgp_p[1], e->fgp_p[2], e->halo_lo, e->is_first, lambda, e->n, e->nx, e->sx);
    LAUNCHCHK();
    return TOMO_OK;
}

int tomo_fgp_grad(tomo_engine *e, float lambda)
{
    NEED(e);
    if (!e->tvg || !e->fgp_p[2]) return fail(TOMO_ERR_STATE, "tomo_fgp_begin has not been called");
    float multip = 1.0f / (26.0f * lambda);
    ProfScope ps(e, TOMO_K_FGP_GRAD);
    hipLaunchKernelGGL(k_fgp_grad, dim3(tv_grid(e)), dim3(256), 0, e->stream, e->tvg, e->fgp_p[0], e->fgp_p[1], e->fgp_p[2], e->halo_hi, e->is_last, multip, e->n, e->nx, e->sx);
    LAUNCHCHK();
    return TOMO_OK;
}

int tomo_fgp_end(tomo_engine *e, int iters)
{
    if (e && e->fgp_target >= 0 && e->fgp_target < TOMO_VOL_SLOTS) ++e->vol_version[e->fgp_target];

    NEED(e);
    if (!e->tvg) return fail(TOMO_ERR_STATE, "tomo_fgp_begin has not been called");
    (void)iters;
    HIPCHK(hipMemcpyAsync(e->vol[e->fgp_target], e->tvg, e->vol_elems() * sizeof(float), hipMemcpyDeviceToDevice, e->stream));
    return TOMO_OK;
}

int tomo_tv(tomo_engine *e, int vol, float eps)
{
    int rc;
    if ((rc = tomo_halo_local(e, vol))) return rc;
    return tomo_tv_partial(e, vol, eps);
}

static int tv_gd_impl(tomo_engine *e, int ng, float dPOCS, float eps, int track_vol, int slot)
{
    int rc;
    if (!e) return fail(TOMO_ERR_ARG, "null engine");
    const bool fold_tv = ng > 0 && (e->tv_lds == 8 || e->tv_lds == 1);
    if (fold_tv) { if ((rc = tomo_halo_local(e, e->tv_target))) return rc; }
    else if ((rc = tomo_tv(e, e->tv_target, eps))) return rc;
    for (int g = 0; g < ng; ++g) {
        if ((rc = tv_grad_impl(e, eps, fold_tv && g == 0))) return rc;
        if ((rc = tv_update_impl(e, dPOCS, g == ng - 1, g == ng - 1 ? track_vol : -1, slot, g < ng - 1))) return rc;
    }
    if (ng <= 0) {
        if ((rc = tomo_positivity(e, e->tv_target))) return rc;
        if (track_vol >= 0) {
            if ((rc = tomo_diff_norm_sq(e, e->tv_target, track_vol, slot))) return rc;
            return tomo_copy_volume(e, track_vol, e->tv_target);
        }
    }
    return TOMO_OK;
}

int tomo_tv_gd(tomo_engine *e, int ng, float dPOCS, float eps) { return tv_gd_impl(e, ng, dPOCS, eps, -1, 0); }

int tomo_tv_gd_tracked(tomo_engine *e, int ng, float dPOCS, float eps, int track_vol, int slot)
{
    if (track_vol < 0) return fail(TOMO_ERR_ARG, "bad tracked volume");
    return tv_gd_impl(e, ng, dPOCS, eps, track_vol, slot);
}

int tomo_tv_fgp(tomo_engine *e, int iters, float lambda) { return tomo_tv_fgp_vol(e, TOMO_VOL_RECON, iters, lambda); }

int tomo_bind_fgp_halo(tomo_engine *e, void *lo, void *hi, void *send_first, void *send_last)
{
    NEED(e);
    if (!lo || !hi || !send_first || !send_last) return fail(TOMO_ERR_ARG, "null plane buffer");
    HIPCHK(hipStreamSynchronize(e->stream));
    e->fgp_lo = (float *)lo; e->fgp_hi = (float *)hi; e->fgp_send_first = (float *)send_first; e->fgp_send_last = (float *)send_last;
    e->fgp_planes2 = false;
    return TOMO_OK;
}

int tomo_bind_fgp_halo2(tomo_engine *e, void *lo, void *hi, void *send_first, void *send_last)
{
    int rc = tomo_bind_fgp_halo(e, lo, hi, send_first, send_last);
    if (rc) return rc;
    e->fgp_planes2 = true;
    return TOMO_OK;
}

static bool fgp_sharded(const tomo_engine *e) { return !(e->is_first && e->is_last); }

int tomo_fgp_fused_begin(tomo_engine *e, int vol)
{
    int rc;
    if ((rc = fgp_begin_impl(e, vol, false))) return rc;
    float *q;
    for (int i = 0; i < 3; ++i) if ((rc = get_scratch(e, &e->fgp_q[i], &q))) return rc;
    if (fgp_sharded(e)) {
        if (!e->fgp_lo) return fail(TOMO_ERR_STATE, "slab-sharded fused FGP needs tomo_bind_fgp_halo");
        hipLaunchKernelGGL(k_halo_pack, dim3((unsigned)((e->npix + 255) / 256)), dim3(256), 0, e->stream, e->vol[vol], e->fgp_send_first, (int)e->npix, e->sx, 0);
// ... 120 lines not shown
```

### tomo_tv_amd/csrc/kernels_fp.hip.h

```cpp
#pragma once

namespace tomo {

constexpr int RAY_GROUP = 16;

__device__ __forceinline__ void ray_block_map(int bid, int nb, int nrows, int &chunk, int &rowidx)
{
    if ((nrows % (8 * RAY_GROUP)) == 0 && (nb & 7) == 0) {
        int xcd = bid & 7, l = bid >> 3;
        int per = nrows >> 3;
        chunk = l / per;
        int li = l - chunk * per;
        int g = li / RAY_GROUP, w = li - g * RAY_GROUP;
        rowidx = (g * 8 + xcd) * RAY_GROUP + w;
    } else {
        chunk = bid / nrows;
        rowidx = bid - chunk * nrows;
    }
}

enum { FP_STORE = 0, FP_RESID = 1, FP_RESID_NORM = 2, FP_DD = 3, FP_POISSON = 4, FP_RESID_MUL = 5 };

template <int VEC, int MODE>
__global__ __launch_bounds__(256) void k_fp_rows(const float *__restrict__ x, const uint32_t *__restrict__ rptr,
// ... 219 lines not shown
    for (; __any(b < nb); b += FT_PF, epn += FT_PF * FT_BATCH) {
        FT_ISSUE(e1, 1, xb, wb, lb) FT_CONSUME(e0, 0, xa, wa, la)
        FT_ISSUE(e2, 2, xa, wa, la) FT_CONSUME(e1, 1, xb, wb, lb)
        FT_ISSUE(e3, 3, xb, wb, lb) FT_CONSUME(e2, 2, xa, wa, la)
        FT_ISSUE(e4, 4, xa, wa, la) FT_CONSUME(e3, 3, xb, wb, lb)
        FT_ISSUE(e5, 5, xb, wb, lb) FT_CONSUME(e4, 4, xa, wa, la)
        FT_ISSUE(e6, 6, xa, wa, la) FT_CONSUME(e5, 5, xb, wb, lb)
        FT_ISSUE(e7, 7, xb, wb, lb) FT_CONSUME(e6, 6, xa, wa, la)
        FT_ISSUE(e0, FT_PF, xa, wa, la)
        FT_CONSUME(e7, 7, xb, wb, lb)
    }
#undef FT_CONSUME
#undef FT_ISSUE
#undef FT_FM1
#undef FT_LD1
}

constexpr int FS_W = 16, FS_H = 16, FS_PIX = FS_W * FS_H, FS_THREADS = 512, FS_WAVES = FS_THREADS / 64, FS_GROUPS = FS_THREADS / 16;
constexpr int FS_RING = 7;
struct FsItemD { int pass, v0; uint32_t tile0, ntiles, cnt0, g0, work, pad; };
#ifndef FS_DMA_STAGE
#define FS_DMA_STAGE 1
#endif

template <int K>
__global__ __launch_bounds__(FS_THREADS) __attribute__((amdgpu_waves_per_eu(4, 4)))
void k_fp_strip(const float *__restrict__ x, const FsItemD *__restrict__ items, const int *__restrict__ orient,
                const int *__restrict__ shift, const uint4 *__restrict__ cnt, const uint32_t *__restrict__ gstart,
                const uint32_t *__restrict__ gseg0, const uint2 *__restrict__ ent, float *__restrict__ part, int n, int sx,
                int nitems, int chunk0, int ncp, const float *__restrict__ zero16)
{
    typedef VecOf<4>::T V;
    static_assert(K >= 1 && K <= 16, "slots per lane group");
    __shared__ V fs_tile[(FS_PIX + 1) * 16];
    __shared__ uint2 fs_ring[FS_WAVES * FS_RING * 32];
    const int xcd = blockIdx.x & 7, l = blockIdx.x >> 3;
    const int it = (l / ncp) * 8 + xcd, c = l % ncp;
    if (it >= nitems) return;
    const FsItemD I = items[it];
    const int t = threadIdx.x, gl = t & 15, g = t >> 4;
    const int wave = __builtin_amdgcn_readfirstlane(t >> 6);
    const int o = orient[I.pass];
    const int *sh = shift + (size_t)I.pass * n;
    const float *xc = x + (size_t)(chunk0 + c) * 64 + gl * 4;
    const char *gsrc = reinterpret_cast<const char *>(ent + (size_t)gstart[I.g0 + g] * FT_BATCH) + gl * 4;
    uint2 *ring_w = fs_ring + wave * (FS_RING * 32);
    const uint32_t ring_l = (uint32_t)(size_t)(__attribute__((address_space(3))) uint2 *)(ring_w + ((t >> 4) & 3) * 8 + (gl & 7));
#define FS_DMA(SLOT) __builtin_amdgcn_global_load_lds((const __attribute__((address_space(1))) void *)gsrc, \
                                                      (__attribute__((address_space(3))) void *)(ring_w + (SLOT) * 32), 4, 0, 0); gsrc += 64;
#pragma unroll
    for (int b = 0; b < FS_RING; ++b) { FS_DMA(b) }
    float *pp = part + ((size_t)gseg0[I.g0 + g] * ncp + c) * 64 + gl * 4;
    const size_t pstep = (size_t)ncp * 64;
    V acc[K];
#pragma unroll
    for (int k = 0; k < K; ++k) acc[k] = vzero<4>();
    const char *base = reinterpret_cast<const char *>(fs_tile) + gl * 16;
    const uint4 *cp = cnt + I.cnt0 + wave;
    if (t < 16) fs_tile[FS_PIX * 16 + t] = vzero<4>();
    uint32_t slot = 0;
    uint2 en;
    asm volatile("s_waitcnt vmcnt(%1)\n\tds_read_b64 %0, %2" : "=v"(en) : "n"(FS_RING - 1), "v"(ring_l) : "memory");
    for (uint32_t tt = 0; tt < I.ntiles; ++tt) {
        if (tt) __syncthreads();
#if FS_DMA_STAGE
        {
            const int u0 = (int)(I.tile0 + tt) * FS_H;
#pragma unroll
            for (int i = 0; i < FS_PIX / FS_GROUPS; ++i) {
                const int q = g + FS_GROUPS * i;
                const int u = u0 + q / FS_W;
                const int vv = I.v0 + sh[min(u, n - 1)] + q % FS_W;
                const bool ok = u < n && (unsigned)vv < (unsigned)n;
                const size_t pix = o ? (size_t)vv * n + u : (size_t)u * n + vv;
                const float *src = ok ? xc + pix * sx : zero16 + gl * 4;
                __builtin_amdgcn_global_load_lds((const __attribute__((address_space(1))) void *)src,
                                                 (__attribute__((address_space(3))) void *)(fs_tile + (4 * wave + FS_GROUPS * i) * 16), 16, 0, 0);
            }
            asm volatile("s_waitcnt vmcnt(0)" ::: "memory");
        }
#else
        {
            const int u0 = (int)(I.tile0 + tt) * FS_H;
            V v[FS_PIX / FS_GROUPS];
#pragma unroll
            for (int i = 0; i < FS_PIX / FS_GROUPS; ++i) {
                const int q = g + FS_GROUPS * i;
                const int u = u0 + q / FS_W;
                const int vv = I.v0 + sh[min(u, n - 1)] + q % FS_W;
                const bool ok = u < n && (unsigned)vv < (unsigned)n;
                const size_t pix = o ? (size_t)vv * n + u : (size_t)u * n + vv;
                v[i] = ok ? nt_ld<16>(reinterpret_cast<const V *>(xc + pix * sx)) : vzero<4>();
            }
#pragma unroll
            for (int i = 0; i < FS_PIX / FS_GROUPS; ++i) fs_tile[(g + FS_GROUPS * i) * 16 + gl] = v[i];
        }
#endif
        __syncthreads();
        const uint4 c4 = cp[(size_t)tt * FS_WAVES];
#define FS_LD1(J) xv[J] = *reinterpret_cast<const V *>(base + row_ror<J>(off));
#define FS_FM1(J) acc[k] += __uint_as_float(row_ror<J>(wb)) * xv[J];
#define FS_NEXT                                                                                           \
        FS_DMA(slot)            \
        slot = slot == FS_RING - 1 ? 0u : slot + 1u;                                                      \
                            \
        asm volatile("s_waitcnt vmcnt(%1)\n\tds_read_b64 %0, %2" : "=v"(en) : "n"(FS_RING - 1), "v"(ring_l + slot * 256u) : "memory");
#define FS_UNIT(FULL)                                                                                     \
        {                                                                                                 \
            asm volatile("s_waitcnt lgkmcnt(0)" : "+v"(en) : : "memory");    \
            const uint2 e = en;                                                                           \
            FS_NEXT                                                                                       \
            const uint32_t off = e.x & 0x7FFFFFFFu, wb = e.y;                                             \
            V xv[FT_BATCH];                                                                               \
            FS_LD1(0) FS_LD1(1) FS_LD1(2) FS_LD1(3)                                                       \
            if (FULL) { FS_LD1(4) FS_LD1(5) FS_LD1(6) FS_LD1(7) }                                         \
            FS_FM1(0) FS_FM1(1) FS_FM1(2) FS_FM1(3)                                                       \
            if (FULL) { FS_FM1(4) FS_FM1(5) FS_FM1(6) FS_FM1(7) }                                         \
            if (e.x >> 31) {    \
                nt_st<32>(acc[k], reinterpret_cast<V *>(pp));                                             \
                acc[k] = vzero<4>();                                                                      \
                pp += pstep;                                                                              \
            }                                                                                             \
        }
#pragma unroll
        for (int k = 0; k < K; ++k) {
            const uint32_t word = k < 4 ? c4.x : k < 8 ? c4.y : k < 12 ? c4.z : c4.w;
            const uint32_t h = __builtin_amdgcn_readfirstlane((word >> (8 * (k & 3))) & 0xFFu);
            for (uint32_t b = h >> 1; b > 0; --b) FS_UNIT(true)
            if (h & 1) FS_UNIT(false)
        }
#undef FS_UNIT
#undef FS_NEXT
#undef FS_FM1
#undef FS_LD1
    }
    asm volatile("s_waitcnt vmcnt(0) lgkmcnt(0)" : "+v"(en) : : "memory");
#undef FS_DMA
}

template <int LPR, int MODE>
__global__ __launch_bounds__(256) void k_fp_tile_reduce(const float *__restrict__ part, const uint32_t *__restrict__ rsptr,
                                                         const uint32_t *__restrict__ rsidx, const float *__restrict__ b,
                                                         const float *__restrict__ rowsum, float *__restrict__ out,
                                                         double *__restrict__ dpart, int nrows, int sx, int chunk0, int ncp)
{
    typedef VecOf<4>::T V;
    constexpr int R = 64 / LPR, U = 8;
    const int lane = threadIdx.x & 63, wave = threadIdx.x >> 6;
    const int grp = lane / LPR, gl = lane - grp * LPR;
    const int spans = ncp * 16 / LPR;
    int64_t item = ((int64_t)blockIdx.x * 4 + wave) * R + grp;
    int row = (int)(item / spans), span = (int)(item - (int64_t)row * spans);
    bool valid = row < nrows;
    if (!__any(valid)) return;
    if (!valid) row = 0;
    uint32_t kb = rsptr[row], ke = valid ? rsptr[row + 1] : kb;
    const float *pp = part + (size_t)span * (LPR * 4) + gl * 4;
    V acc = vzero<4>();
    uint32_t sidx[U], sn[U];
#pragma unroll
    for (int u = 0; u < U; ++u) sidx[u] = (kb + u < ke) ? rsidx[kb + u] : 0xFFFFFFFFu;
    for (uint32_t k = kb; __any(k < ke); k += U) {
        V pv[U];
#pragma unroll
        for (int u = 0; u < U; ++u) pv[u] = (sidx[u] != 0xFFFFFFFFu) ? nt_ld<32>(reinterpret_cast<const V *>(pp + (size_t)sidx[u] * ncp * 64)) : vzero<4>();
#pragma unroll
        for (int u = 0; u < U; ++u) sn[u] = (k + U + u < ke) ? rsidx[k + U + u] : 0xFFFFFFFFu;
#pragma unroll
        for (int u = 0; u < U; ++u) acc += pv[u];
#pragma unroll
        for (int u = 0; u < U; ++u) sidx[u] = sn[u];
    }
    double local = 0.0;
    if (valid) {
        size_t o = (size_t)row * sx + (size_t)chunk0 * 64 + (size_t)span * (LPR * 4) + gl * 4;
        if (MODE == FP_STORE) {
            *reinterpret_cast<V *>(out + o) = acc;
        } else {
            V bv = *reinterpret_cast<const V *>(b + o);
            V r;
            if (MODE == FP_RESID) {
                r = bv - acc;
            } else if (MODE == FP_RESID_NORM) {
                float rs = rowsum[row];
                r = rs > 0.f ? (bv - acc) / rs : vzero<4>();
            } else if (MODE == FP_RESID_MUL) {
                r = (bv - acc) * rowsum[row];
            } else if (MODE == FP_DD) {
                r = acc;
#pragma unroll
                for (int i = 0; i < 4; ++i) { float d = acc[i] - bv[i]; local += (double)(d * d); }
            } else {
                const float eps = 1e-1f;
#pragma unroll
                for (int i = 0; i < 4; ++i) {
                    float a = acc[i], bb = bv[i];
                    r[i] = (a - bb) / (a + eps);
                    local += (double)(a - bb * logf(a + eps));
                }
            }
            *reinterpret_cast<V *>(out + o) = r;
        }
    }
    if (MODE == FP_DD || MODE == FP_POISSON) {
        local = wave_sum(local);
        if (lane == 0) atomicAdd(&dpart[blockIdx.x & (NPART - 1)], local);
    }
}

template <int MODE>
__global__ __launch_bounds__(256) void k_sino_resid(const float *__restrict__ b, const float *__restrict__ g,
                                                     const float *__restrict__ rowsum, float *__restrict__ out, int64_t n4, int sx4)
{
    typedef VecOf<4>::T V;
    for (int64_t i = (int64_t)blockIdx.x * 256 + threadIdx.x; i < n4; i += (int64_t)gridDim.x * 256) {
        V bv = reinterpret_cast<const V *>(b)[i], acc = reinterpret_cast<const V *>(g)[i], r;
        if (MODE == FP_RESID) {
            r = bv - acc;
        } else {
            float rs = rowsum[i / sx4];
            r = rs > 0.f ? (bv - acc) / rs : vzero<4>();
        }
        reinterpret_cast<V *>(out)[i] = r;
    }
}

__global__ __launch_bounds__(256) void k_sino_extrapolate(const VecOf<4>::T *__restrict__ g, VecOf<4>::T *__restrict__ p,
                                                          VecOf<4>::T *__restrict__ q, float beta, int64_t n4)
{
    for (int64_t i = (int64_t)blockIdx.x * 256 + threadIdx.x; i < n4; i += (int64_t)gridDim.x * 256) {
        VecOf<4>::T a = g[i], b = p[i];
        q[i] = a + beta * (a - b);
        p[i] = a;
    }
}

constexpr int FL_W = 16, FL_TH = 8, FL_PIX = FL_W * FL_TH, FL_THREADS = 1024, FL_WAVES = FL_THREADS / 64, FL_BATCH = 16, FL_PIXB = 512;
constexpr int FL_TILE_BYTES = 2 * FL_PIX * FL_PIXB, FL_MAXSTEPS = 64 * FL_TH, FL_LDS_BYTES = FL_TILE_BYTES + FL_MAXSTEPS * 4;
struct FlItemD { int pass, v0; uint32_t tile0, ntiles, lp0, work, pad0, pad1; };

#define FL_RD(SB, K)                                                                                      \
    "v_and_or_b32 v[32+2*" #K "], s[" #SB "+2*" #K "], %[mask], %[base]\n"                                \
    "ds_read_b64 v[32+2*" #K ":33+2*" #K "], v[32+2*" #K "]\n"
#define FL_FMA(SB, K, W)                                                                                  \
    "s_waitcnt lgkmcnt(" #W ")\n"                                                                         \
    "s_set_gpr_idx_on s[" #SB "+2*" #K "], gpr_idx(SRC2,DST)\n"                                           \
    "v_pk_fma_f32 v[64:65], s[" #SB "+2*" #K ":" #SB "+2*" #K "+1], v[32+2*" #K ":33+2*" #K "], v[64:65] op_sel:[1,0,0] op_sel_hi:[1,1,1]\n"
#define FL_READS(SB)                                                                                      \
    FL_RD(SB, 0) FL_RD(SB, 1) FL_RD(SB, 2) FL_RD(SB, 3) FL_RD(SB, 4) FL_RD(SB, 5) FL_RD(SB, 6) FL_RD(SB, 7)             \
    FL_RD(SB, 8) FL_RD(SB, 9) FL_RD(SB, 10) FL_RD(SB, 11) FL_RD(SB, 12) FL_RD(SB, 13) FL_RD(SB, 14) FL_RD(SB, 15)
#define FL_FMAS(SB)                                                                                       \
    FL_FMA(SB, 0, 15) FL_FMA(SB, 1, 14) FL_FMA(SB, 2, 13) FL_FMA(SB, 3, 12) FL_FMA(SB, 4, 11) FL_FMA(SB, 5, 10) FL_FMA(SB, 6, 9) FL_FMA(SB, 7, 8) \
    FL_FMA(SB, 8, 7) FL_FMA(SB, 9, 6) FL_FMA(SB, 10, 5) FL_FMA(SB, 11, 4) FL_FMA(SB, 12, 3) FL_FMA(SB, 13, 2) FL_FMA(SB, 14, 1) FL_FMA(SB, 15, 0) \
    "s_set_gpr_idx_off\n"
#define FL_CLOB4(P, A, B, C, D) #P #A, #P #B, #P #C, #P #D
#define FL_CLOBBERS                                                                                       \
    FL_CLOB4(s, 68, 69, 70, 71), FL_CLOB4(s, 72, 73, 74, 75), FL_CLOB4(s, 76, 77, 78, 79), FL_CLOB4(s, 80, 81, 82, 83),      \
    FL_CLOB4(s, 84, 85, 86, 87), FL_CLOB4(s, 88, 89, 90, 91), FL_CLOB4(s, 92, 93, 94, 95), FL_CLOB4(s, 96, 97, 98, 99),      \
    "s33",                                                                                                \
    FL_CLOB4(v, 32, 33, 34, 35), FL_CLOB4(v, 36, 37, 38, 39), FL_CLOB4(v, 40, 41, 42, 43), FL_CLOB4(v, 44, 45, 46, 47),      \
    FL_CLOB4(v, 48, 49, 50, 51), FL_CLOB4(v, 52, 53, 54, 55), FL_CLOB4(v, 56, 57, 58, 59), FL_CLOB4(v, 60, 61, 62, 63),      \
    "vcc", "scc", "memory"

__global__ __launch_bounds__(FL_THREADS)
void k_fp_list(const float *__restrict__ x, const FlItemD *__restrict__ items, const int *__restrict__ orient, const int *__restrict__ shift,
               const uint2 *__restrict__ lent, const uint32_t *__restrict__ lptr, const uint2 *__restrict__ fent, const uint32_t *__restrict__ fptr,
               float *__restrict__ part, int n, int sx, int nitems, int cpair0, int ncpp, int ncp, const float *__restrict__ zero)
{
    typedef VecOf<4>::T V;
    extern __shared__ V fl_lds[];
    const int xcd = blockIdx.x & 7, l = blockIdx.x >> 3;
    const int it = (l / ncpp) * 8 + xcd, c2 = l % ncpp;
    if (it >= nitems) return;
    const FlItemD I = items[it];
    const int t = threadIdx.x, lane = t & 63, jl = lane >> 5;
    const int wave = __builtin_amdgcn_readfirstlane(t >> 6);
    const int o = orient[I.pass];
    const int ntiles = (int)I.ntiles;
    int *sh_l = reinterpret_cast<int *>(reinterpret_cast<char *>(fl_lds) + FL_TILE_BYTES);
    {
        const int *sh = shift + (size_t)I.pass * n;
        for (int i = t; i < ntiles * FL_TH; i += FL_THREADS) sh_l[i] = sh[min((int)I.tile0 * FL_TH + i, n - 1)];
    }
    const float *xc = x + (size_t)(cpair0 + c2) * 128 + (lane & 31) * 4;
    const float *zsrc = zero + (lane & 31) * 4;
    const uint32_t *lp = lptr + I.lp0 + wave, *fp = fptr + I.lp0 + wave;
    uint32_t pv0 = 0, pv1 = 0, fv0 = 0, fv1 = 0;
    if (lane < ntiles) {
        pv0 = lp[(size_t)lane * FL_WAVES]; pv1 = lp[(size_t)lane * FL_WAVES + 1];
        fv0 = fp[(size_t)lane * FL_WAVES]; fv1 = fp[(size_t)lane * FL_WAVES + 1];
    }
    __syncthreads();
#define FL_STAGE(TT)                                                                                      \
    _Pragma("unroll") for (int q = 0; q < FL_PIX / 2 / FL_WAVES; ++q) {                                   \
        const int p = wave + FL_WAVES * q;                                                                \
        const int lu = p >> 3, u = ((int)I.tile0 + (TT)) * FL_TH + lu;                                    \
        const int vv = I.v0 + sh_l[(TT) * FL_TH + lu] + 2 * (p & 7) + jl;                                 \
        const bool ok = u < n && (unsigned)vv < (unsigned)n;                                              \
        const size_t pix = o ? (size_t)vv * n + u : (size_t)u * n + vv;                                   \
        const float *src = ok ? xc + pix * sx : zsrc;                                                     \
        __builtin_amdgcn_global_load_lds((const __attribute__((address_space(1))) void *)src,             \
                                         (__attribute__((address_space(3))) void *)(fl_lds + (((TT) & 1) * FL_PIX + 2 * p) * (FL_PIXB / 16)), 16, 0, 0); \
    }
#define FL_TOUCH(TT)                                                                                      \
    {                                                                                                     \
        const uint32_t t0 = __builtin_amdgcn_readlane(pv0, (TT)), t1 = __builtin_amdgcn_readlane(pv1, (TT)); \
        if (t0 + lane < t1) touched = *reinterpret_cast<const uint32_t *>(lent + (size_t)(t0 + lane) * FL_BATCH);    \
    }
    uint32_t touched = 0;
    FL_STAGE(0)
    FL_TOUCH(0)
    v32f acc_lo, acc_hi;
#pragma unroll
    for (int q = 0; q < 32; ++q) { acc_lo[q] = 0.f; acc_hi[q] = 0.f; }
    if ((uint32_t)(size_t)(__attribute__((address_space(3))) V *)fl_lds != 0u) __builtin_trap();
    const uint32_t base = (uint32_t)lane * 8u, mask = ~(uint32_t)(FL_PIXB - 1);
    const uint64_t pb = (uint64_t)(size_t)(part + (size_t)c2 * 128);
    const uint32_t pb_lo = (uint32_t)pb, pb_hi = (uint32_t)(pb >> 32), pstride = (uint32_t)ncp * 256u;
    asm volatile("s_waitcnt vmcnt(0)" : "+v"(touched) :: "memory");
    __syncthreads();
    for (int tt = 0; tt < ntiles; ++tt) {
        const uint32_t b0 = __builtin_amdgcn_readlane(pv0, tt);
        uint32_t nb = __builtin_amdgcn_readlane(pv1, tt) - b0;
        const uint2 *ep = lent + (size_t)b0 * FL_BATCH;
        u16v ea, eb;
        asm volatile("s_load_dwordx16 %0, %2, 0x0\n"
                     "s_load_dwordx16 %1, %2, 0x40\n" : "={s[36:51]}"(ea), "={s[52:67]}"(eb) : "s"(ep));
        if (tt + 1 < ntiles) { FL_STAGE(tt + 1) FL_TOUCH(tt + 1) }
        {
            asm volatile("s_waitcnt lgkmcnt(0)\n"
                         "s_cmp_eq_u32 %[nb], 0\n"
                         "s_cbranch_scc1 3f\n"
                         "s_mov_b32 s33, m0\n"
                         "s_mov_b64 vcc, %[ep]\n"
                         "1:\n"
                         "s_load_dwordx16 s[68:83], vcc, 0x80\n"
                         "s_load_dwordx16 s[84:99], vcc, 0xc0\n"
                         FL_READS(36)
                         FL_FMAS(36)
                         "s_sub_u32 %[nb], %[nb], 1\n"
                         "s_cmp_eq_u32 %[nb], 0\n"
                         "s_cbranch_scc1 2f\n"
                         "s_add_u32 vcc_lo, vcc_lo, 0x100\n"
                         "s_addc_u32 vcc_hi, vcc_hi, 0\n"
                         "s_load_dwordx16 s[36:51], vcc, 0x0\n"
                         "s_load_dwordx16 s[52:67], vcc, 0x40\n"
                         FL_READS(68)
                         FL_FMAS(68)
                         "s_sub_u32 %[nb], %[nb], 1\n"
                         "s_cmp_lg_u32 %[nb], 0\n"
                         "s_cbranch_scc1 1b\n"
                         "2:\n"
                         "s_waitcnt lgkmcnt(0)\n"
                         "s_mov_b32 m0, s33\n"
                         "3:\n"
                         : "+{v[64:95]}"(acc_lo), "+{v[96:127]}"(acc_hi), [nb] "+s"(nb), "+{s[36:51]}"(ea), "+{s[52:67]}"(eb)
                         : [ep] "s"(ep), [base] "v"(base), [mask] "v"(mask)
                         : FL_CLOBBERS);
        }
        asm volatile("s_waitcnt vmcnt(0)" : "+v"(touched) :: "memory");
// ... 48 lines not shown
```

### tomo_tv_amd/csrc/kernels_tv.hip.h

```cpp
#pragma once

namespace tomo {

struct Halo { const float *lo; const float *hi; };

__device__ __forceinline__ float ldx(const float *__restrict__ x, const Halo &h, int pix, int s, int nx, int sx)
{
    if (s < 0) return h.lo[pix];
    if (s >= nx) return h.hi[pix];
    return x[(size_t)pix * sx + s];
}

__global__ void k_halo_pack(const float *__restrict__ x, float *__restrict__ dst, int npix, int sx, int s)
{
    int i = blockIdx.x * blockDim.x + threadIdx.x;
    if (i < npix) dst[i] = x[(size_t)i * sx + s];
}

__global__ void k_scalars_to_host(const double *__restrict__ src, double *__restrict__ host_dst, int n)
{
    int i = threadIdx.x;
    if (i < n) host_dst[i] = src[i];
}

// ... 304 lines not shown
    int bs, bz, ys;
    bool live;
    if ((nzb & 7) == 0) {
        const int zpx = nzb >> 3;
        const int64_t li = (int64_t)(blockIdx.x >> 3) * 4 + wave;
        bs = (int)(li % nchunk); bz = (int)(blockIdx.x & 7) * zpx + (int)((li / nchunk) % zpx); ys = (int)(li / ((int64_t)nchunk * zpx));
        live = ys < nys;
    } else {
        const int64_t item = (int64_t)blockIdx.x * 4 + wave;
        bs = (int)(item % nchunk); bz = (int)((item / nchunk) % nzb); ys = (int)(item / ((int64_t)nchunk * nzb));
        live = ys < nys;
    }
    if (live) {
        const int y0 = ys * yseg, y1 = min(y0 + yseg, n);
        const int z0 = bz * TZ, s0 = bs * 64, s = s0 + lane;
        const int se = lane == 0 ? s0 - 1 : (lane == 63 ? s0 + 64 : s);
        int zc[TZ + 2];
#pragma unroll
        for (int j = 0; j < TZ + 2; ++j) { int z = (z0 - 1 + j) % n; zc[j] = z < 0 ? z + n : z; }
        auto yrow = [&](int y) { int r = y % n; return r < 0 ? r + n : r; };
        float cm[TZ + 2], c0[TZ + 2], cp[TZ + 2], cn[TZ + 2], E0[TZ + 2], Ep[TZ + 2], En[TZ + 2], Rm[TZ + 1], R0[TZ + 1];
        const bool interior = s0 > 0 && s0 + 64 < nx;
        auto fetch = [&](int y, float *c, float *E) {
            int yy = yrow(y) * n;
            if (interior) {
#pragma unroll
                for (int j = 0; j < TZ + 2; ++j) {
                    const float *rp = x + (size_t)(yy + zc[j]) * sx;
                    c[j] = nt_ld<8>(rp + (unsigned)s);
                    E[j] = nt_ld<8>(rp + (unsigned)se);
                }
            } else {
#pragma unroll
                for (int j = 0; j < TZ + 2; ++j) {
                    c[j] = tv_ld(x, h, yy + zc[j], s, nx, sx);
                    E[j] = tv_ld(x, h, yy + zc[j], se, nx, sx);
                }
            }
        };
#define TVR_RINV(C, IP, JP, KP, RR, DD)                                                                   \
        {                                                                                                 \
            float d1_ = (C) - (IP), d2_ = (C) - (JP), d3_ = (C) - (KP);                                   \
            float q_ = __fmaf_rn(d3_, d3_, __fmaf_rn(d2_, d2_, __fmaf_rn(d1_, d1_, eps)));                \
            RR = tv_rsqrt(q_);                                                                            \
            DD = __fmul_rn(q_, RR);                                                                       \
        }
        auto shr = [&](float old, float v) {
            return __builtin_bit_cast(float, __builtin_amdgcn_update_dpp(__builtin_bit_cast(int, old), __builtin_bit_cast(int, v), 0x138, 0xf, 0xf, false));
        };
        auto shl = [&](float old, float v) {
            return __builtin_bit_cast(float, __builtin_amdgcn_update_dpp(__builtin_bit_cast(int, old), __builtin_bit_cast(int, v), 0x130, 0xf, 0xf, false));
        };
        float PE0 = 0.f, PEp = 0.f, PEn = 0.f, PC0 = 0.f, PCn = 0.f;
        int zl;
        { int z = (z0 - 1 + (lane < TZ + 2 ? lane : 0)) % n; zl = z < 0 ? z + n : z; }
        auto fetch_ph = [&](int y, float &pe, float &pc) {
            int pix = yrow(y) * n + zl;
            pe = tv_ld(x, h, pix, s0 - 1, nx, sx);
            pc = tv_ld(x, h, pix, s0, nx, sx);
        };
        if (GRAD) fetch(y0 - 1, cm, En);
        fetch(y0, c0, E0);
        fetch(y0 + 1, cp, Ep);
        if (GRAD) { float pcp; fetch_ph(y0, PE0, PC0); fetch_ph(y0 + 1, PEp, pcp); PCn = pcp; }
#pragma unroll
        for (int j = 1; GRAD && j <= TZ; ++j) {
            float xip = shl(En[j], cm[j]), dd;
            TVR_RINV(cm[j], xip, c0[j], cm[j + 1], Rm[j], dd)
            (void)dd;
        }
        for (int y = y0; y < y1; ++y) {
            float PCp = PCn;
            if (y + 1 < y1) { fetch(y + 2, cn, En); if (GRAD) fetch_ph(y + 2, PEn, PCn); }
            float REp;
            if (GRAD) {
                float kp = __builtin_bit_cast(float, __builtin_amdgcn_update_dpp(0, __builtin_bit_cast(int, PE0), 0x101, 0xf, 0xf, false));
                float dd;
                TVR_RINV(PE0, PC0, PEp, kp, REp, dd)
                (void)dd;
            }
            float xip[TZ + 1];
#pragma unroll
            for (int j = 0; j <= TZ; ++j) {
                float dd;
                xip[j] = shl(E0[j], c0[j]);
                TVR_RINV(c0[j], xip[j], cp[j], c0[j + 1], R0[j], dd)
                if (WITH_TV && j >= 1 && z0 + j - 1 < n && s < nx) tvacc += (double)dd;
            }
#pragma unroll
            for (int j = 1; GRAD && j <= TZ; ++j) {
                float re = __builtin_bit_cast(float, __builtin_amdgcn_readlane(__builtin_bit_cast(int, REp), j));
                float rim = shr(re, R0[j]);
                float xim = shr(E0[j], c0[j]);
                float c = c0[j];
                float gv = tv_gval(c, xip[j], cp[j], c0[j + 1], R0[j], xim, rim, cm[j], Rm[j], c0[j - 1], R0[j - 1]);
                int z = z0 + j - 1;
                if (z < n && s < nx) {
                    if (MODE == TVM_STORE) {
                        float *gr = g + (size_t)(y * n + z) * sx;
                        gr[(unsigned)s] = gv;
                        acc += (double)(gv * gv);
                    } else if (MODE == TVM_NORM) {
                        acc += (double)(gv * gv);
                        if (up.wrap_lo) {
                            const size_t pix = (size_t)(y * n + z);
                            if (s == 0) up.wrap_hi[pix] = gv;
                            if (s == nx - 1) up.wrap_lo[pix] = gv;
                        }
                    } else {
                        const size_t pix = (size_t)(y * n + z);
                        float v = tv_step(c, gv, nrm_);
                        if (up.clamp) v = fmaxf(v, 0.f);
                        if (up.stream) __builtin_nontemporal_store(v, up.x_out + pix * sx + (unsigned)s);
                        else up.x_out[pix * sx + (unsigned)s] = v;
                        if (up.wrap_lo) {
                            if (s == 0) up.wrap_hi[pix] = v;
                            if (s == nx - 1) up.wrap_lo[pix] = v;
                        }
                        if (up.track) {
                            float *tr = up.track + pix * sx;
                            float d = v - tr[(unsigned)s];
                            acc += (double)(d * d);
                            if (up.stream) __builtin_nontemporal_store(v, tr + (unsigned)s);
                            else tr[(unsigned)s] = v;
                        }
                    }
                }
            }
#pragma unroll
            for (int j = 0; j < TZ + 2; ++j) { cm[j] = c0[j]; c0[j] = cp[j]; cp[j] = cn[j]; E0[j] = Ep[j]; Ep[j] = En[j]; }
            PE0 = PEp; PEp = PEn; PC0 = PCp;
#pragma unroll
            for (int j = 1; j <= TZ; ++j) Rm[j] = R0[j];
        }
#undef TVR_RINV
    }
    if (GRAD) block_accumulate(acc, part);
    if (WITH_TV) {
        __syncthreads();
        block_accumulate(tvacc, part_tv);
    }
}

#ifndef TV4_PACKED
#define TV4_PACKED 1
#endif
#ifndef TV4_PACKED_EDGE
#define TV4_PACKED_EDGE 0
#endif
#ifndef TV4_UPD_WAVES
#define TV4_UPD_WAVES 4
#endif
#define TV4_OCC __attribute__((amdgpu_waves_per_eu((MODE == TVM_UPDATE && !TRACK) ? TV4_UPD_WAVES : 4, (MODE == TVM_UPDATE && !TRACK) ? TV4_UPD_WAVES : 8)))
template <int TZ, bool WITH_TV, int MODE, bool EDGE, bool TRACK = false, bool STREAM = false>
__global__ __launch_bounds__(256) TV4_OCC void k_tv_march4(const float *__restrict__ x, Halo h, double *__restrict__ part, float eps,
                                                    int n, int nx, int sx, int yseg, double *__restrict__ part_tv, TvUpd up)
{
    static_assert(MODE == TVM_NORM || MODE == TVM_UPDATE || MODE == TVM_VALUE, "modes without a stored gradient");
    static_assert(MODE != TVM_VALUE || WITH_TV, "the value mode sums the TV integrand");
    const int lane = threadIdx.x & 63, wave = __builtin_amdgcn_readfirstlane(threadIdx.x >> 6);
    const int nzb = (n + TZ - 1) / TZ, nchunk = (nx + 63) >> 6   , nys = (n + yseg - 1) / yseg;
    double acc = 0.0, tvacc = 0.0;
    float nrm_ = 1.f;
    if (MODE == TVM_UPDATE) nrm_ = tv_step_len(up.dPOCS, up.gnorm2);
    int bs, bz, ys;
    if ((nzb & 7) == 0) {
        const int zpx = nzb >> 3;
        const int64_t li = (int64_t)(blockIdx.x >> 3) * 4 + wave;
        bs = (int)(li % nchunk); bz = (int)(blockIdx.x & 7) * zpx + (int)((li / nchunk) % zpx); ys = (int)(li / ((int64_t)nchunk * zpx));
    } else {
        const int64_t item = (int64_t)blockIdx.x * 4 + wave;
        bs = (int)(item % nchunk); bz = (int)((item / nchunk) % nzb); ys = (int)(item / ((int64_t)nchunk * nzb));
    }
    if (ys < nys) {
        const int y0 = ys * yseg, y1 = min(y0 + yseg, n);
        const int z0 = bz * TZ, s0 = bs * 64, s = s0 + lane;
        int zc[TZ + 2];
#pragma unroll
        for (int j = 0; j < TZ + 2; ++j) { int z = (z0 - 1 + j) % n; zc[j] = z < 0 ? z + n : z; }
        int zl;
        { int z = (z0 - 1 + (lane < TZ + 2 ? lane : 0)) % n; zl = z < 0 ? z + n : z; }
        auto yrow = [&](int y) { int r = y % n; return r < 0 ? r + n : r; };
        float rows[4][TZ + 2], Ta[TZ + 1], Tb[TZ + 1];
        float pe[4], pf[4], pc[4];
        const bool lo_in = s0 > 0, hi_in = s0 + 64 < nx;
        const unsigned zls = (unsigned)zl * (unsigned)sx;
        const unsigned off_lo = lo_in ? zls + (unsigned)(s0 - 1) : (unsigned)zl, off_hi = hi_in ? zls + (unsigned)(s0 + 64) : (unsigned)zl;
        constexpr bool SOFF = !EDGE && !(WITH_TV && MODE == TVM_NORM);
        unsigned vb[TZ + 2];
#pragma unroll
        for (int j = 0; j < TZ + 2; ++j) vb[j] = ((unsigned)zc[j] * (unsigned)sx + (unsigned)s0 + (unsigned)lane) * 4u;
        unsigned eb_c = (zls + (unsigned)s0) * 4u, eb_lo = off_lo * 4u, eb_hi = off_hi * 4u;
        auto fetch = [&](int y, float *c, float &e_lo, float &e_hi, float &e_c) __attribute__((always_inline)) {
            int yy = yrow(y) * n;
            if (!EDGE) {
                const float *rowp = x + (size_t)yy * sx;
                if constexpr (SOFF) {
                    const SBase rb = sgpr_base(rowp);
#pragma unroll
                    for (int j = 0; j < TZ + 2; ++j) c[j] = ld_so(rb, vb[j]);
                    e_c = ld_so(rb, eb_c);
                    e_lo = ld_so(sgpr_base(lo_in ? rowp : h.lo + yy), eb_lo);
                    e_hi = ld_so(sgpr_base(hi_in ? rowp : h.hi + yy), eb_hi);
                } else {
#pragma unroll
                    for (int j = 0; j < TZ + 2; ++j) c[j] = (rowp + ((unsigned)zc[j] * (unsigned)sx + (unsigned)s0))[(unsigned)lane];
                    e_c = rowp[zls + (unsigned)s0];
                    e_lo = (lo_in ? rowp : h.lo + yy)[off_lo];
                    e_hi = (hi_in ? rowp : h.hi + yy)[off_hi];
                }
            } else {
#pragma unroll
                for (int j = 0; j < TZ + 2; ++j) c[j] = tv_ld(x, h, yy + zc[j], s, nx, sx);
                e_lo = tv_ld(x, h, yy + zl, s0 - 1, nx, sx);
                e_hi = tv_ld(x, h, yy + zl, s0 + 64, nx, sx);
                e_c = tv_ld(x, h, yy + zl, s0, nx, sx);
            }
        };
        const float vmin = up.clamp ? 0.f : -INFINITY;
        const bool planes = up.wrap_lo != nullptr && (EDGE || s0 == 0 || s0 + 64 == nx);
#define TV4_RINV(C, IP, JP, KP, RR, DD, D1, D2, D3)                                                       \
        {                                                                                                 \
            D1 = (C) - (IP); D2 = (C) - (JP); D3 = (C) - (KP);                                            \
            float q_ = __fmaf_rn(D3, D3, __fmaf_rn(D2, D2, __fmaf_rn(D1, D1, eps)));                      \
            RR = tv_rsqrt(q_);                                                                            \
            DD = __fmul_rn(q_, RR);                                                                       \
        }
        auto shr = [&](float old, float v) {
            return __builtin_bit_cast(float, __builtin_amdgcn_update_dpp(__builtin_bit_cast(int, old), __builtin_bit_cast(int, v), 0x138, 0xf, 0xf, false));
        };
        auto shl = [&](float old, float v) {
            return __builtin_bit_cast(float, __builtin_amdgcn_update_dpp(__builtin_bit_cast(int, old), __builtin_bit_cast(int, v), 0x130, 0xf, 0xf, false));
        };
        auto col = [&](float packed, int j) {
            return __builtin_bit_cast(float, __builtin_amdgcn_readlane(__builtin_bit_cast(int, packed), j));
        };
        auto row = [&](int y, const float *c0, const float *cp, float *cn, float pe0, float pf0, float pc0, float pep,
                       float &pen, float &pfn, float &pcn, const float *Tp, float *Tn
                       ) __attribute__((always_inline)) {
            if (y + 1 < y1) fetch(y + 2, cn, pen, pfn, pcn);
            float TEp = 0.f;
            float out[TZ + 1];
            float tk_prev = 0.f;
            if constexpr (TV4_PACKED && (!EDGE || TV4_PACKED_EDGE)) {
            static_assert((TZ & 1) == 0, "column pairs");
#define TV4_RINV2(C, IP, JP, KP, RR, DD, D1, D2, D3)                                                      \
            {                                                                                             \
                D1 = (C) - (IP); D2 = (C) - (JP); D3 = (C) - (KP);                                        \
                const v2f q_ = fma2(D3, D3, fma2(D2, D2, fma2(D1, D1, v2f{eps, eps})));                   \
                RR = v2f{tv_rsqrt(q_.x), tv_rsqrt(q_.y)};                                                 \
                DD = nc_mul2(q_, RR);                                                                     \
            }
            {
                const float kpe = MODE != TVM_VALUE ? shl(0.f, pe0) : 0.f;
                const v2f c = {c0[0], pe0}, ip = {shl(col(pf0, 0), c0[0]), pc0}, jp = {cp[0], pep}, kp = {c0[1], kpe};
                v2f r, dd, d1, d2, d3;
                TV4_RINV2(c, ip, jp, kp, r, dd, d1, d2, d3)
                (void)dd; (void)d2;
                tk_prev = nc_mul(d3.x, r.x);
                if (MODE != TVM_VALUE) TEp = nc_mul(d1.y, r.y);
            }
#pragma unroll
            for (int j = 1; j < TZ; j += 2) {
                const v2f c = {c0[j], c0[j + 1]}, xip = {shl(col(pf0, j), c0[j]), shl(col(pf0, j + 1), c0[j + 1])};
                const v2f jp = {cp[j], cp[j + 1]}, kp = {c0[j + 1], c0[j + 2]};
                v2f r, dd, d1, d2, d3;
                TV4_RINV2(c, xip, jp, kp, r, dd, d1, d2, d3)
                const bool ok0 = !EDGE || (z0 + j - 1 < n && s < nx), ok1 = !EDGE || (z0 + j < n && s < nx);
                if (WITH_TV) { tvacc += (double)(ok0 ? dd.x : 0.f); tvacc += (double)(ok1 ? dd.y : 0.f); }
                const v2f tk = nc_mul2(d3, r);
                if (MODE != TVM_VALUE) {
                    const v2f ti = nc_mul2(d1, r);
                    const v2f tn = nc_mul2(d2, r);
                    Tn[j] = tn.x; Tn[j + 1] = tn.y;
                    #if TV_V1N_DIFFS
                    const v2f g1 = nc_mul2(nc_add2(nc_add2(d1, d2), d3), r);
#else
                    const v2f g1 = nc_mul2(nc_sub2(nc_sub2(fma2(v2f{3.0f, 3.0f}, c, -xip), jp), kp), r);
#endif
                    const v2f t2 = {shr(col(TEp, j), ti.x), shr(col(TEp, j + 1), ti.y)};
                    const v2f tp = {Tp[j], Tp[j + 1]}, tkp = {tk_prev, tk.x};
                    const v2f gv = nc_sub2(nc_sub2(nc_sub2(g1, t2), tp), tkp);
                    if (MODE == TVM_NORM) {
                        out[j] = gv.x; out[j + 1] = gv.y;
                        const v2f g2 = gv * gv;
                        acc += (double)(ok0 ? g2.x : 0.f);
                        acc += (double)(ok1 ? g2.y : 0.f);
                    } else {
                        const v2f xn = fma2(-gv, v2f{nrm_, nrm_}, c);
                        out[j] = fmaxf(xn.x, vmin); out[j + 1] = fmaxf(xn.y, vmin);
                    }
                }
                tk_prev = tk.y;
            }
#undef TV4_RINV2
            } else {
            if (MODE != TVM_VALUE) {
                float kp = shl(0.f, pe0), r_, dd_, d1, d2, d3;
                TV4_RINV(pe0, pc0, pep, kp, r_, dd_, d1, d2, d3)
                (void)dd_; (void)d2; (void)d3;
                TEp = nc_mul(d1, r_);
            }
#pragma unroll
            for (int j = 0; j <= TZ; ++j) {
                float dd, d1, d2, d3, r;
                const float c = c0[j], xip = shl(col(pf0, j), c);
                TV4_RINV(c, xip, cp[j], c0[j + 1], r, dd, d1, d2, d3)
                if (WITH_TV && j >= 1) tvacc += (double)((!EDGE || (z0 + j - 1 < n && s < nx)) ? dd : 0.f);
                const float tk = nc_mul(d3, r);
                if (j >= 1 && MODE != TVM_VALUE) {
                    const float ti = nc_mul(d1, r);
                    Tn[j] = nc_mul(d2, r);
                    #if TV_V1N_DIFFS
                    const float g1 = nc_mul(nc_add(nc_add(d1, d2), d3), r);
#else
                    const float g1 = nc_mul(nc_sub(nc_sub(__fmaf_rn(3.0f, c, -xip), cp[j]), c0[j + 1]), r);
#endif
                    const float t2 = shr(col(TEp, j), ti);
                    const float gv = nc_sub(nc_sub(nc_sub(g1, t2), Tp[j]), tk_prev);
                    const bool ok = !EDGE || (z0 + j - 1 < n && s < nx);
                    if (MODE == TVM_NORM) {
                        out[j] = gv;
                        float g2 = gv * gv;
                        acc += (double)(ok ? g2 : 0.f);
                    } else {
                        out[j] = fmaxf(tv_step(c, gv, nrm_), vmin);
                    }
                }
                tk_prev = tk;
            }
            }
            const size_t pix0 = (size_t)(y * n + z0);
            if (MODE == TVM_UPDATE) {
                const SBase xo = sgpr_base(up.x_out + (size_t)y * n * sx);
                float *xo_e = up.x_out + pix0 * sx + (unsigned)s0;
#pragma unroll
                for (int j = 1; j <= TZ; ++j) {
                    if (EDGE && !(z0 + j - 1 < n && s < nx)) continue;
                    if constexpr (SOFF) st_so<STREAM>(xo, vb[j], out[j]);
                    else if (STREAM) __builtin_nontemporal_store(out[j], xo_e + (size_t)(j - 1) * sx + (unsigned)lane);
                    else (xo_e + (size_t)(j - 1) * sx)[(unsigned)lane] = out[j];
                }
                if (TRACK) {
                    const SBase tr = sgpr_base(up.track + (size_t)y * n * sx);
                    float *tr_e = up.track + pix0 * sx + (unsigned)s0;
                    float told[TZ + 1];
#pragma unroll
                    for (int j = 1; j <= TZ; ++j) {
                        if constexpr (SOFF) told[j] = ld_so(tr, vb[j]);
                        else told[j] = (z0 + j - 1 < n && s < nx) ? (tr_e + (size_t)(j - 1) * sx)[(unsigned)lane] : out[j];
                    }
#pragma unroll
                    for (int j = 1; j <= TZ; ++j) {
                        float d = out[j] - told[j];
                        acc += (double)(d * d);
                        if (EDGE && !(z0 + j - 1 < n && s < nx)) continue;
                        if constexpr (SOFF) st_so<STREAM>(tr, vb[j], out[j]);
                        else if (STREAM) __builtin_nontemporal_store(out[j], tr_e + (size_t)(j - 1) * sx + (unsigned)lane);
                        else (tr_e + (size_t)(j - 1) * sx)[(unsigned)lane] = out[j];
                    }
                }
            }
            if (planes) {
                if (s == 0) {
#pragma unroll
                    for (int j = 1; j <= TZ; ++j) if (!EDGE || z0 + j - 1 < n) up.wrap_hi[pix0 + (j - 1)] = out[j];
                }
                if (s == nx - 1) {
#pragma unroll
                    for (int j = 1; j <= TZ; ++j) if (!EDGE || z0 + j - 1 < n) up.wrap_lo[pix0 + (j - 1)] = out[j];
                }
            }
            if (MODE == TVM_UPDATE && up.hg_lo != nullptr && (EDGE || s0 == 0 || s0 + 64 == nx)) {
                if (!EDGE) {
                    const unsigned hp = (unsigned)(y * n) + (unsigned)zl;
                    if (lane >= 1 && lane <= TZ) {
                        if (s0 == 0) up.ho_lo[hp] = fmaxf(tv_step(pe0, up.hg_lo[hp], nrm_), vmin);
                        if (s0 + 64 == nx) up.ho_hi[hp] = fmaxf(tv_step(pf0, up.hg_hi[hp], nrm_), vmin);
                    }
                } else {
                    if (s == 0) {
#pragma unroll
                        for (int j = 1; j <= TZ; ++j)
                            if (z0 + j - 1 < n) up.ho_lo[pix0 + (j - 1)] = fmaxf(tv_step(h.lo[pix0 + (j - 1)], up.hg_lo[pix0 + (j - 1)], nrm_), vmin);
                    }
                    if (s == nx - 1) {
#pragma unroll
                        for (int j = 1; j <= TZ; ++j)
                            if (z0 + j - 1 < n) up.ho_hi[pix0 + (j - 1)] = fmaxf(tv_step(h.hi[pix0 + (j - 1)], up.hg_hi[pix0 + (j - 1)], nrm_), vmin);
                    }
                }
            }
        };
        fetch(y0 - 1, rows[0], pe[0], pf[0], pc[0]);
        fetch(y0, rows[1], pe[1], pf[1], pc[1]);
        fetch(y0 + 1, rows[2], pe[2], pf[2], pc[2]);
#pragma unroll
        for (int j = 1; MODE != TVM_VALUE && j <= TZ; ++j) {
            float xi = shl(col(pf[0], j), rows[0][j]), r, dd, d1, d2, d3;
            TV4_RINV(rows[0][j], xi, rows[1][j], rows[0][j + 1], r, dd, d1, d2, d3)
            (void)dd; (void)d1; (void)d3;
            Ta[j] = nc_mul(d2, r);
        }
#define TV4_ROW(S0, SP, SN, TP, TN) row(y, rows[S0], rows[SP], rows[SN], pe[S0], pf[S0], pc[S0], pe[SP], pe[SN], pf[SN], pc[SN], TP, TN)
        for (int y = y0; y < y1;) {
            TV4_ROW(1, 2, 3, Ta, Tb); if (++y >= y1) break;
            TV4_ROW(2, 3, 0, Tb, Ta); if (++y >= y1) break;
            TV4_ROW(3, 0, 1, Ta, Tb); if (++y >= y1) break;
            TV4_ROW(0, 1, 2, Tb, Ta); ++y;
        }
#undef TV4_ROW
#undef TV4_RINV
    }
    if (MODE != TVM_VALUE) block_accumulate(acc, part);
    if (WITH_TV) {
        __syncthreads();
        block_accumulate(tvacc, part_tv);
    }
}

__global__ __launch_bounds__(256) void k_halo_apply(float *__restrict__ halo_lo, float *__restrict__ halo_hi,
                                                     const float *__restrict__ g_lo, const float *__restrict__ g_hi,
                                                     const double *__restrict__ gnorm2, float dPOCS, int clamp, int npix)
{
    const float len = tv_step_len(dPOCS, gnorm2);
    int p = blockIdx.x * 256 + threadIdx.x;
    if (p >= npix) return;
    float a = tv_step(halo_lo[p], g_lo[p], len);
    float b = tv_step(halo_hi[p], g_hi[p], len);
    if (clamp) { a = fmaxf(a, 0.f); b = fmaxf(b, 0.f); }
    halo_lo[p] = a;
    halo_hi[p] = b;
}

template <bool TRACK>
__global__ __launch_bounds__(256) void k_tv_update(f4 *__restrict__ x, const f4 *__restrict__ g,
                                                    const double *__restrict__ gnorm2, float dPOCS, int clamp,
                                                    int64_t n4, f4 *__restrict__ track, double *__restrict__ part,
                                                    float *__restrict__ wrap_lo, float *__restrict__ wrap_hi, int nx, int sx4)
{
    const float len = tv_step_len(dPOCS, gnorm2);
    double acc = 0.0;
    for (int64_t i = (int64_t)blockIdx.x * 256 + threadIdx.x; i < n4; i += (int64_t)gridDim.x * 256) {
        f4 xv = x[i], gv = g[i], v;
        v.x = tv_step(xv.x, gv.x, len); v.y = tv_step(xv.y, gv.y, len); v.z = tv_step(xv.z, gv.z, len); v.w = tv_step(xv.w, gv.w, len);
        if (clamp) { v.x = fmaxf(v.x, 0.f); v.y = fmaxf(v.y, 0.f); v.z = fmaxf(v.z, 0.f); v.w = fmaxf(v.w, 0.f); }
        x[i] = v;
        if (wrap_lo) {
            int64_t pix = i / sx4;
            int s = (int)(i - pix * sx4) * 4;
            if (s == 0) wrap_hi[pix] = v.x;
            int d = nx - 1 - s;
            if (d >= 0 && d < 4) wrap_lo[pix] = d == 0 ? v.x : d == 1 ? v.y : d == 2 ? v.z : v.w;
        }
        if (TRACK) {
            f4 d = v - track[i];
            acc += (double)(d.x * d.x) + (double)(d.y * d.y) + (double)(d.z * d.z) + (double)(d.w * d.w);
            track[i] = v;
        }
    }
    if (TRACK) block_accumulate(acc, part);
}

}
```

### tomo_tv_amd/csrc/sart_resident.hip.h

```cpp
#pragma once

namespace tomo {

typedef float v16f __attribute__((ext_vector_type(16)));
typedef unsigned long long rs_u64;
typedef uint32_t rs_u2 __attribute__((ext_vector_type(2)));
constexpr int RS_T = 32, RS_WAVES = 16, RS_THREADS = RS_WAVES * 64, RS_MAXWIN = 48, RS_RL = 32, RS_USABLE = 14;
struct RsHdrD { uint16_t jbase, nrays; uint32_t dw[4]; uint32_t pad[3]; };
static_assert(sizeof(RsHdrD) == 32, "header layout (resident.h)");
struct RsArgs {
    float *x;
    const float *b, *rowsum;
    const RsHdrD *hdr;
    const uint4 *cell;
    const uint2 *ts;
    const uint16_t *rl;
    rs_u64 *pb, *rb;
    const int *angs;
    float *track;
    double *part;
    int *abort_word, *abort_host;
    unsigned *commit;
    int *done_host;
    unsigned seq, commit_base;
    int test_fail;
    int n, sx, np, ntiles, tiles, rpt, steps, chunk0, nchunk;
    unsigned epoch0, spin_limit;
    float beta;
    long long *prof;
};
#ifdef RS_PROF
#define RS_STAMP(q) { const long long now_ = (long long)__builtin_amdgcn_s_memrealtime(); if (wave == 0) tacc[q] += now_ - tprev; tprev = now_; }
#define RS_TL(q) { if (k == 40 && blockIdx.x == 37 && lane == 0) rs_args()->prof[2048 + wave * 8 + (q)] = (long long)__builtin_amdgcn_s_memrealtime(); }
#else
#define RS_STAMP(q)
#define RS_TL(q)
#endif

__device__ __forceinline__ rs_u64 rs_gld(const rs_u64 *p)
{
    return __hip_atomic_load((const __attribute__((address_space(1))) rs_u64 *)p, __ATOMIC_RELAXED, __HIP_MEMORY_SCOPE_AGENT);
}
__device__ __forceinline__ void rs_gst(rs_u64 *p, float v, unsigned ep)
{
    __hip_atomic_store((__attribute__((address_space(1))) rs_u64 *)p, ((rs_u64)ep << 32) | (rs_u64)__float_as_uint(v), __ATOMIC_RELAXED, __HIP_MEMORY_SCOPE_AGENT);
}
__device__ __forceinline__ int rs_abort_ld(const int *p)
{
    return __hip_atomic_load((const __attribute__((address_space(1))) int *)p, __ATOMIC_RELAXED, __HIP_MEMORY_SCOPE_AGENT);
}
__device__ __forceinline__ bool rs_give_up(unsigned &spins, unsigned spin_limit, int *abort_word, int *abort_host, int lane, int code)
{
    if (((++spins) & 31u) != 0u && spin_limit != 0u) return false;
    if (spins > spin_limit) {
        if (lane == 0) {
            __hip_atomic_store((__attribute__((address_space(1))) int *)abort_word, code, __ATOMIC_RELAXED, __HIP_MEMORY_SCOPE_AGENT);
            if (abort_host) __hip_atomic_store((__attribute__((address_space(1))) int *)abort_host, code, __ATOMIC_RELAXED, __HIP_MEMORY_SCOPE_SYSTEM);
        }
        return true;
    }
    return rs_abort_ld(abort_word) != 0;
}

constexpr unsigned RS_POISON = 0x80000000u;
__device__ __forceinline__ bool rs_commit(unsigned *w, unsigned base, unsigned ntiles, bool clean, unsigned spin_limit, const int *abort_word)
{
    typedef __attribute__((address_space(1))) unsigned *gp;
    if (!clean) { __hip_atomic_fetch_or((gp)w, RS_POISON, __ATOMIC_RELAXED, __HIP_MEMORY_SCOPE_AGENT); return false; }
    unsigned seen = __hip_atomic_fetch_add((gp)w, 1u, __ATOMIC_RELAXED, __HIP_MEMORY_SCOPE_AGENT) + 1u;
    const unsigned full = base + ntiles;
    for (unsigned spins = 0;;) {
        if (seen & RS_POISON) return false;
        if (seen == full) return true;
        if (++spins > spin_limit || ((spins & 31u) == 0u && rs_abort_ld(abort_word) != 0)) {
            unsigned expected = seen;
            if (__hip_atomic_compare_exchange_strong((gp)w, &expected, seen | RS_POISON, __ATOMIC_RELAXED, __ATOMIC_RELAXED, __HIP_MEMORY_SCOPE_AGENT)) return false;
            seen = expected;
            continue;
        }
        __builtin_amdgcn_s_sleep(4);
        seen = __hip_atomic_load((gp)w, __ATOMIC_RELAXED, __HIP_MEMORY_SCOPE_AGENT);
    }
}

#define RS_LD(OFF)                                                                                        \
    "s_load_dwordx16 s[36:51], %[cp], " #OFF "\n"                                                         \
    "s_load_dwordx16 s[52:67], %[cp], " #OFF "+0x40\n"                                                    \
    "s_load_dwordx16 s[68:83], %[cp], " #OFF "+0x80\n"                                                    \
    "s_load_dwordx16 s[84:99], %[cp], " #OFF "+0xc0\n"
#define RS_IDX(SB, K) "s_set_gpr_idx_idx s[" #SB "+4*" #K "]\n"
#define RS_BP1(SB, K, Q)                                                                                  \
    RS_IDX(SB, K)                                                                                         \
    "v_mul_f32 v48, s[" #SB "+4*" #K "+1], v32\n"                                                         \
    "v_fma_f32 v48, s[" #SB "+4*" #K "+2], v33, v48\n"                                                    \
    "v_mul_f32 v48, v48, s[" #SB "+4*" #K "+3]\n"                                                         \
    "v_fma_f32 v[64+" #Q "], v48, %[beta], v[64+" #Q "]\n"                                                \
    "v_max_f32 v[64+" #Q "], v[64+" #Q "], 0\n"
#define RS_FP1(SB, K, Q)                                                                                  \
    RS_IDX(SB, K)                                                                                         \
    "v_fma_f32 v32, s[" #SB "+4*" #K "+1], v[64+" #Q "], v32\n"                                           \
    "v_fma_f32 v33, s[" #SB "+4*" #K "+2], v[64+" #Q "], v33\n"
#define RS_BATCH(OP, B)                                                                                   \
    OP(36, 0, 16*B+0) OP(36, 1, 16*B+1) OP(36, 2, 16*B+2) OP(36, 3, 16*B+3) OP(36, 4, 16*B+4) OP(36, 5, 16*B+5) OP(36, 6, 16*B+6) OP(36, 7, 16*B+7) \
    OP(36, 8, 16*B+8) OP(36, 9, 16*B+9) OP(36, 10, 16*B+10) OP(36, 11, 16*B+11) OP(36, 12, 16*B+12) OP(36, 13, 16*B+13) OP(36, 14, 16*B+14) OP(36, 15, 16*B+15)
#define RS_WAIT "s_waitcnt lgkmcnt(0)\n"
#define RS_SWEEP(OP)                                                                                      \
    RS_BATCH(OP, 0) RS_LD(0x100) RS_WAIT RS_BATCH(OP, 1) RS_LD(0x200) RS_WAIT RS_BATCH(OP, 2) RS_LD(0x300) RS_WAIT RS_BATCH(OP, 3)
#define RS_CLOB4(P, A, B, C, D) #P #A, #P #B, #P #C, #P #D
#define RS_CLOBBERS                                                                                       \
    RS_CLOB4(s, 36, 37, 38, 39), RS_CLOB4(s, 40, 41, 42, 43), RS_CLOB4(s, 44, 45, 46, 47), RS_CLOB4(s, 48, 49, 50, 51),      \
    RS_CLOB4(s, 52, 53, 54, 55), RS_CLOB4(s, 56, 57, 58, 59), RS_CLOB4(s, 60, 61, 62, 63), RS_CLOB4(s, 64, 65, 66, 67),      \
    RS_CLOB4(s, 68, 69, 70, 71), RS_CLOB4(s, 72, 73, 74, 75), RS_CLOB4(s, 76, 77, 78, 79), RS_CLOB4(s, 80, 81, 82, 83),      \
    RS_CLOB4(s, 84, 85, 86, 87), RS_CLOB4(s, 88, 89, 90, 91), RS_CLOB4(s, 92, 93, 94, 95), RS_CLOB4(s, 96, 97, 98, 99),      \
    "s33", "v48", "memory"

#define RS_XROW(OP, R)                                                                                    \
    OP(8*R+0) OP(8*R+1) OP(8*R+2) OP(8*R+3) OP(8*R+4) OP(8*R+5) OP(8*R+6) OP(8*R+7)                       \
    "s_add_u32 s36, s36, %[rs]\n" "s_addc_u32 s37, s37, 0\n"
#define RS_XALL(OP) RS_XROW(OP, 0) RS_XROW(OP, 1) RS_XROW(OP, 2) RS_XROW(OP, 3) RS_XROW(OP, 4) RS_XROW(OP, 5) RS_XROW(OP, 6) RS_XROW(OP, 7)
#define RS_XLD1(Q) "global_load_dword v[64+" #Q "], %[voff], s[36:37]\n" "s_add_u32 s36, s36, %[ps]\n" "s_addc_u32 s37, s37, 0\n"
#define RS_XZ1(Q) "v_mov_b32 v[64+" #Q "], 0\n"
#define RS_XZROW(R) RS_XZ1(8*R+0) RS_XZ1(8*R+1) RS_XZ1(8*R+2) RS_XZ1(8*R+3) RS_XZ1(8*R+4) RS_XZ1(8*R+5) RS_XZ1(8*R+6) RS_XZ1(8*R+7)
#define RS_XST1(Q) "global_store_dword %[voff], v[64+" #Q "], s[36:37]\n" "s_add_u32 s36, s36, %[ps]\n" "s_addc_u32 s37, s37, 0\n"
#define RS_TLD1(C) "global_load_dword v[49+" #C "], %[voff], s[38:39]\n" "s_add_u32 s38, s38, %[ps]\n" "s_addc_u32 s39, s39, 0\n"
#define RS_TST1(R, C)                                                                                     \
    "v_sub_f32 v48, v[64+8*" #R "+" #C "], v[49+" #C "]\n"                                                \
    "v_mul_f32 v48, v48, v48\n"                                                                           \
    "v_cvt_f64_f32 v[58:59], v48\n"                                                                       \
    "v_add_f64 %[sum], %[sum], v[58:59]\n"                                                                \
    "global_store_dword %[voff], v[64+8*" #R "+" #C "], s[36:37]\n" "s_add_u32 s36, s36, %[ps]\n" "s_addc_u32 s37, s37, 0\n" \
    "global_store_dword %[voff], v[64+8*" #R "+" #C "], s[40:41]\n" "s_add_u32 s40, s40, %[ps]\n" "s_addc_u32 s41, s41, 0\n"
#define RS_TROW(R)                                                                                        \
    RS_TLD1(0) RS_TLD1(1) RS_TLD1(2) RS_TLD1(3) RS_TLD1(4) RS_TLD1(5) RS_TLD1(6) RS_TLD1(7)               \
    "s_waitcnt vmcnt(0)\n"                                                                                \
    RS_TST1(R, 0) RS_TST1(R, 1) RS_TST1(R, 2) RS_TST1(R, 3) RS_TST1(R, 4) RS_TST1(R, 5) RS_TST1(R, 6) RS_TST1(R, 7) \
    "s_add_u32 s36, s36, %[rs]\n" "s_addc_u32 s37, s37, 0\n"                                              \
    "s_add_u32 s38, s38, %[rs]\n" "s_addc_u32 s39, s39, 0\n"                                              \
    "s_add_u32 s40, s40, %[rs]\n" "s_addc_u32 s41, s41, 0\n"

#define RS_K __attribute__((address_space(4)))
typedef const RS_K RsArgs *RsArgsP;
__device__ __forceinline__ RsArgsP rs_args()
{
    RsArgsP p = (RsArgsP)__builtin_amdgcn_kernarg_segment_ptr();
    asm volatile("" : "+s"(p) :: "memory");
    return p;
}

__device__ __forceinline__ int rs_angle(RsArgsP A, int k)
{
    return ((const RS_K int *)A->angs)[k];
}

__device__ __forceinline__ void rs_touch(RsArgsP A, int tile, int wave, int lane, int an, float *dump)
{
    if (lane < 8 && an >= 0) {
        const uint32_t *tp = reinterpret_cast<const uint32_t *>(A->cell + (((size_t)an * A->ntiles + tile) * RS_WAVES + wave) * 64) + lane * 32;
        __builtin_amdgcn_global_load_lds((const __attribute__((address_space(1))) void *)tp, (__attribute__((address_space(3))) void *)dump, 4, 0, 0);
    }
}

__global__ __launch_bounds__(RS_THREADS) __attribute__((amdgpu_waves_per_eu(4, 4)))
void k_sart_resident(const RsArgs unused_by_name)
{
    __shared__ float rs_pbuf[RS_WAVES][16][64];
    __shared__ float rs_rbuf[RS_MAXWIN][64];
    __shared__ float rs_sbuf[RS_WAVES][64];
    __shared__ float rs_dump[RS_WAVES][64];
    __shared__ int rs_dirty, rs_go, rs_store;
    const int lane = threadIdx.x & 63;
    const int wave = __builtin_amdgcn_readfirstlane(threadIdx.x >> 6);
    v32f xlo, xhi;
    v16f rr;
#ifdef RS_PROF
    long long tacc[8] = {0, 0, 0, 0, 0, 0, 0, 0}, tprev = (long long)__builtin_amdgcn_s_memrealtime();
    const long long clk0 = (long long)__builtin_amdgcn_s_memtime(), rt0 = tprev;
#endif
    int tile, grp, ngrp, chunk, chunk_end, steps;
    {
        RsArgsP A = rs_args();
        tile = (int)blockIdx.x % A->ntiles; grp = (int)blockIdx.x / A->ntiles; ngrp = (int)gridDim.x / A->ntiles;
        chunk = A->chunk0 + grp; chunk_end = A->chunk0 + A->nchunk; steps = A->steps;
    }
    for (int it = 0; chunk < chunk_end; chunk += ngrp, ++it) {
        const uint32_t voff = (uint32_t)(chunk * 64 + lane) * 4u;
        {
            if (threadIdx.x == 0) { rs_dirty = 0; rs_go = rs_abort_ld(rs_args()->abort_word) == 0 ? 1 : 0; }
            __syncthreads();
            if (rs_go == 0) break;
        }
        {
            RsArgsP A = rs_args();
            rs_touch(A, tile, wave, lane, rs_angle(A, 0), rs_dump[wave]);
            if (steps > 1) rs_touch(A, tile, wave, lane, rs_angle(A, 1), rs_dump[wave]);
            const int n = A->n, sx = A->sx;
            const int ty = tile / A->tiles, tz = tile - ty * A->tiles;
            const int y0 = ty * RS_T + (wave >> 2) * 8, z0 = tz * RS_T + (wave & 3) * 8;
            const int in = __builtin_amdgcn_readfirstlane((y0 < n && z0 < n) ? 1 : 0);
            const float *xb = A->x + ((size_t)min(y0, n - 1) * n + min(z0, n - 1)) * sx;
            const uint32_t ps = (uint32_t)sx * 4u, rs = (uint32_t)(n - 8) * ps;
            asm volatile("s_cmp_eq_u32 %[in], 0\n"
                         "s_cbranch_scc1 1f\n"
                         "s_mov_b64 s[36:37], %[xb]\n"
                         RS_XALL(RS_XLD1)
                         "s_waitcnt vmcnt(0)\n"
                         "s_branch 2f\n"
                         "1:\n"
                         RS_XZROW(0) RS_XZROW(1) RS_XZROW(2) RS_XZROW(3) RS_XZROW(4) RS_XZROW(5) RS_XZROW(6) RS_XZROW(7)
                         "2:\n"
                         : "={v[64:95]}"(xlo), "={v[96:127]}"(xhi)
                         : [in] "s"(in), [xb] "s"(xb), [voff] "v"(voff), [ps] "s"(ps), [rs] "s"(rs)
                         : "s36", "s37", "scc", "memory");
        }
        int c_jbase = 0, c_nr = 0, c_dwv = 0;
        for (int k = -1; k < steps; ++k) {
            int f_nr = 0, f_jbase = 0, f_rpt = 1, f_rpt2 = 1, f_wpr = RS_WAVES, f_cpw = RS_RL / RS_WAVES, f_jr0 = 0, f_sub = 0;
            uint32_t f_dwv = 0;
            rs_u2 f_ts0 = {0u, 0u}, f_ts1 = {0u, 0u}, f_ts2 = {0u, 0u};
            rs_u2 f_ids0 = {0xFFFFFFFFu, 0xFFFFFFFFu};
            float f_rs0 = 0.f, f_bv0 = 0.f;
            if (k + 1 < steps) {
                RsArgsP A = rs_args();
                const int n = A->n;
                const int a = rs_angle(A, k + 1);
                const RS_K RsHdrD *h = (const RS_K RsHdrD *)A->hdr + (size_t)a * A->ntiles + tile;
                f_nr = h->nrays; f_jbase = h->jbase;
                f_dwv = (h->dw[wave >> 2] >> ((wave & 3) * 8)) & 255u;
                {
                    const RS_K rs_u2 *tsp = (const RS_K rs_u2 *)A->ts + ((size_t)a * A->ntiles + tile) * RS_MAXWIN;
                    f_ts0 = tsp[wave]; f_ts1 = tsp[wave + 16]; f_ts2 = tsp[wave + 32];
                }
                f_rpt = A->rpt;
                while (f_rpt2 < f_rpt && f_rpt2 < RS_WAVES) f_rpt2 *= 2;
                f_wpr = RS_WAVES / f_rpt2; f_cpw = RS_RL / f_wpr;
                f_jr0 = wave / f_wpr; f_sub = wave % f_wpr;
                const int j0 = min(tile * f_rpt + f_jr0, n - 1);
                f_ids0 = ((const RS_K rs_u2 *)A->rl)[(((size_t)a * n + j0) * RS_RL + f_sub * f_cpw) >> 2];
                f_rs0 = ((const RS_K float *)A->rowsum)[(size_t)a * n + j0];
                f_bv0 = A->b[((size_t)a * n + j0) * A->sx + (voff >> 2)];
            }
            RS_STAMP(7)
            if (k >= 0) {
                RsArgsP A = rs_args();
                const int n = A->n;
                const int a = rs_angle(A, k);
                const unsigned ep = A->epoch0 + (unsigned)it * (unsigned)steps + (unsigned)k + 1u;
                const int jbase = c_jbase, nr = c_nr, dwv = c_dwv;
                const rs_u64 *rrow = A->rb + (((size_t)grp * A->np + a) * n + jbase) * 64 + lane;
                {
                    const int i0 = wave, i1 = wave + 16, i2 = wave + 32;
                    rs_u64 g0 = 0, g1 = 0, g2 = 0;
                    unsigned spins = 0;
                    for (;;) {
                        if (i0 < nr) g0 = rs_gld(rrow + (size_t)i0 * 64);
                        if (i1 < nr) g1 = rs_gld(rrow + (size_t)i1 * 64);
                        if (i2 < nr) g2 = rs_gld(rrow + (size_t)i2 * 64);
                        bool ok = (i0 >= nr || (unsigned)(g0 >> 32) == ep) && (i1 >= nr || (unsigned)(g1 >> 32) == ep) && (i2 >= nr || (unsigned)(g2 >> 32) == ep);
                        if (__all(ok)) break;
                        if (rs_give_up(spins, A->spin_limit, A->abort_word, A->abort_host, lane, 1)) { rs_dirty = 1; break; }
                        __builtin_amdgcn_s_sleep(1);
                    }
                    if (i0 < nr) rs_rbuf[i0][lane] = __uint_as_float((uint32_t)g0);
                    if (i1 < nr) rs_rbuf[i1][lane] = __uint_as_float((uint32_t)g1);
                    if (i2 < nr) rs_rbuf[i2][lane] = __uint_as_float((uint32_t)g2);
                }
                RS_STAMP(0)
                RS_TL(0)
                __syncthreads();
#pragma unroll
                for (int s = 0; s < 16; ++s) rr[s] = (s < RS_USABLE && dwv + s < nr) ? rs_rbuf[dwv + s][lane] : 0.f;
                const uint4 *cp = A->cell + (((size_t)a * A->ntiles + tile) * RS_WAVES + wave) * 64;
                const float beta = A->beta;
                rs_touch(A, tile, wave, lane, k + 2 < steps ? rs_angle(A, k + 2) : -1, rs_dump[wave]);
                RS_STAMP(1)
                RS_TL(1)
                asm volatile("s_mov_b32 s33, m0\n"
                             RS_LD(0x000)
                             RS_WAIT
                             "s_set_gpr_idx_on s36, gpr_idx(SRC1)\n"
                             RS_SWEEP(RS_BP1)
                             "s_set_gpr_idx_off\n"
                             "s_mov_b32 m0, s33\n"
                             : "+{v[64:95]}"(xlo), "+{v[96:127]}"(xhi), "+{v[32:47]}"(rr)
                             : [cp] "s"(cp), [beta] "s"(beta)
                             : RS_CLOBBERS);
                RS_STAMP(2)
                RS_TL(2)
            }
            if (k + 1 < steps) {
                RsArgsP A = rs_args();
                const int n = A->n;
                const int a = rs_angle(A, k + 1);
                const unsigned ep = A->epoch0 + (unsigned)it * (unsigned)steps + (unsigned)k + 2u;
                const int nr = f_nr, rpt = f_rpt, rpt2 = f_rpt2, wpr = f_wpr, cpw = f_cpw, jr0 = f_jr0, sub = f_sub;
                const rs_u2 ids0 = f_ids0;
                const float rs0 = f_rs0, bv0 = f_bv0;
                c_jbase = f_jbase; c_nr = nr;
                c_dwv = (int)f_dwv;
#pragma unroll
                for (int s = 0; s < 16; ++s) rr[s] = 0.f;
                const uint4 *cp = A->cell + (((size_t)a * A->ntiles + tile) * RS_WAVES + wave) * 64;
                asm volatile("s_mov_b32 s33, m0\n"
                             RS_LD(0x000)
                             RS_WAIT
                             "s_set_gpr_idx_on s36, gpr_idx(SRC2,DST)\n"
                             RS_SWEEP(RS_FP1)
                             "s_set_gpr_idx_off\n"
                             "s_mov_b32 m0, s33\n"
                             : "+{v[64:95]}"(xlo), "+{v[96:127]}"(xhi), "+{v[32:47]}"(rr)
                             : [cp] "s"(cp)
                             : RS_CLOBBERS);
                RS_STAMP(3)
                RS_TL(3)
#pragma unroll
                for (int s = 0; s < 16; ++s) rs_pbuf[wave][s][lane] = rr[s];
                __syncthreads();
                rs_u64 *pb = A->pb + ((size_t)grp * A->ntiles + tile) * RS_MAXWIN * 64 + lane;
#pragma unroll
                for (int r3 = 0; r3 < 3; ++r3) {
                    const int i = wave + 16 * r3;
                    if (i < nr) {
                        const rs_u2 e = r3 == 0 ? f_ts0 : r3 == 1 ? f_ts1 : f_ts2;
                        const float *pr = &rs_pbuf[0][0][0] + lane;
                        float v[8];
#pragma unroll
                        for (int c = 0; c < 8; ++c) v[c] = pr[(((c < 4 ? e.x : e.y) >> ((c & 3) * 8)) & 255u) * 64];
                        float acc = v[0];
#pragma unroll
                        for (int c = 1; c < 8; ++c) acc += v[c];
                        rs_gst(pb + (size_t)i * 64, acc, ep);
                    }
                }
                RS_STAMP(4)
                RS_TL(4)
                const rs_u64 *pg = A->pb + (size_t)grp * A->ntiles * RS_MAXWIN * 64 + lane;
                for (int r0 = 0; r0 < rpt; r0 += rpt2) {
                    const int jr = r0 + jr0, j = tile * rpt + jr;
                    const bool active = jr < rpt && j < n;
                    if (active) {
                        float acc = 0.f;
                        const RS_K rs_u2 *list = (const RS_K rs_u2 *)A->rl + ((((size_t)a * n + j) * RS_RL + sub * cpw) >> 2);
                        for (int e0 = 0; e0 < cpw; e0 += 4) {
                            const rs_u2 ids = (r0 == 0 && e0 == 0) ? ids0 : list[e0 >> 2];
                            const int id0 = ids.x & 0xFFFF, id1 = ids.x >> 16, id2 = ids.y & 0xFFFF, id3 = ids.y >> 16;
                            if (id0 == 0xFFFF) break;
                            rs_u64 g0 = 0, g1 = 0, g2 = 0, g3 = 0;
                            unsigned spins = 0;
                            for (;;) {
                                g0 = rs_gld(pg + (size_t)id0 * 64);
                                if (id1 != 0xFFFF) g1 = rs_gld(pg + (size_t)id1 * 64);
                                if (id2 != 0xFFFF) g2 = rs_gld(pg + (size_t)id2 * 64);
                                if (id3 != 0xFFFF) g3 = rs_gld(pg + (size_t)id3 * 64);
                                bool ok = (unsigned)(g0 >> 32) == ep && (id1 == 0xFFFF || (unsigned)(g1 >> 32) == ep) &&
                                          (id2 == 0xFFFF || (unsigned)(g2 >> 32) == ep) && (id3 == 0xFFFF || (unsigned)(g3 >> 32) == ep);
                                if (__all(ok)) break;
                                if (rs_give_up(spins, A->spin_limit, A->abort_word, A->abort_host, lane, 2)) { rs_dirty = 1; break; }
                                __builtin_amdgcn_s_sleep(1);
                            }
                            acc += __uint_as_float((uint32_t)g0);
                            if (id1 != 0xFFFF) acc += __uint_as_float((uint32_t)g1);
                            if (id2 != 0xFFFF) acc += __uint_as_float((uint32_t)g2);
                            if (id3 != 0xFFFF) acc += __uint_as_float((uint32_t)g3);
                        }
                        rs_sbuf[wave][lane] = acc;
                    }
                    RS_STAMP(5)
                    RS_TL(5)
                    __syncthreads();
                    if (active && sub == 0) {
                        float tot = rs_sbuf[wave][lane];
                        for (int u = 1; u < wpr; ++u) tot += rs_sbuf[wave + u][lane];
                        const size_t row = (size_t)a * n + j;
                        const float bv = r0 == 0 ? bv0 : A->b[row * A->sx + (voff >> 2)], rs = r0 == 0 ? rs0 : ((const RS_K float *)A->rowsum)[row];
                        const float rv = rs > 0.f ? (bv - tot) / rs : 0.f;
                        rs_gst(A->rb + (((size_t)grp * A->np) * n + row) * 64 + lane, rv, ep);
                    }
                    if (r0 + rpt2 < rpt) __syncthreads();
                }
                RS_STAMP(6)
                RS_TL(6)
            }
        }
        {
            __syncthreads();
            if (threadIdx.x == 0) {
                RsArgsP A = rs_args();
                const bool clean = rs_dirty == 0 && rs_abort_ld(A->abort_word) == 0 && !(tile == 0 && A->test_fail == chunk + 1);
                const bool ok = rs_commit(A->commit + chunk, A->commit_base, (unsigned)A->ntiles, clean, A->spin_limit, A->abort_word);
                if (ok && tile == 0)
                    __hip_atomic_store((__attribute__((address_space(1))) int *)(A->done_host + chunk), (int)A->seq, __ATOMIC_RELAXED, __HIP_MEMORY_SCOPE_SYSTEM);
                rs_store = ok ? 1 : 0;
            }
            __syncthreads();
            if (rs_store == 0) continue;
        }
        {
            RsArgsP A = rs_args();
            const int n = A->n, sx = A->sx;
            const int ty = tile / A->tiles, tz = tile - ty * A->tiles;
            const int y0 = ty * RS_T + (wave >> 2) * 8, z0 = tz * RS_T + (wave & 3) * 8;
            const int in = __builtin_amdgcn_readfirstlane((y0 < n && z0 < n) ? 1 : 0);
            const size_t o0 = ((size_t)min(y0, n - 1) * n + min(z0, n - 1)) * sx;
            float *xb = A->x + o0;
            const uint32_t ps = (uint32_t)sx * 4u, rs = (uint32_t)(n - 8) * ps;
            if (A->track) {
                float *tb = A->track + o0;
                double local = 0.0;
                asm volatile("s_cmp_eq_u32 %[in], 0\n"
                             "s_cbranch_scc1 1f\n"
                             "s_mov_b64 s[36:37], %[xb]\n"
                             "s_mov_b64 s[38:39], %[tb]\n"
                             "s_mov_b64 s[40:41], %[tb]\n"
                             RS_TROW(0) RS_TROW(1) RS_TROW(2) RS_TROW(3) RS_TROW(4) RS_TROW(5) RS_TROW(6) RS_TROW(7)
                             "s_waitcnt vmcnt(0)\n"
                             "1:\n"
                             : [sum] "+v"(local)
                             : "{v[64:95]}"(xlo), "{v[96:127]}"(xhi), [in] "s"(in), [xb] "s"(xb), [tb] "s"(tb), [voff] "v"(voff), [ps] "s"(ps), [rs] "s"(rs)
                             : "s36", "s37", "s38", "s39", "s40", "s41", "v48", "v49", "v50", "v51", "v52", "v53", "v54", "v55", "v56", "v58", "v59", "scc", "memory");
                double *red = reinterpret_cast<double *>(&rs_pbuf[wave][0][0]);
                red[lane] = local;
                __builtin_amdgcn_wave_barrier();
                if (lane == 0) {
                    local = 0.0;
                    for (int l = 0; l < 64; ++l) local += red[l];
                    const uint32_t slot = (blockIdx.x & (NPART - 1)) * 8u;
                    double *part = A->part;
                    asm volatile("global_atomic_add_f64 %0, %1, %2" :: "v"(slot), "v"(local), "s"(part) : "memory");
                }
            } else {
                asm volatile("s_cmp_eq_u32 %[in], 0\n"
                             "s_cbranch_scc1 1f\n"
                             "s_mov_b64 s[36:37], %[xb]\n"
                             RS_XALL(RS_XST1)
                             "s_waitcnt vmcnt(0)\n"
                             "1:\n"
                             :
                             : "{v[64:95]}"(xlo), "{v[96:127]}"(xhi), [in] "s"(in), [xb] "s"(xb), [voff] "v"(voff), [ps] "s"(ps), [rs] "s"(rs)
                             : "s36", "s37", "scc", "memory");
            }
        }
    }
#ifdef RS_PROF
    if (threadIdx.x == 0) {
        RsArgsP A = rs_args();
        for (int q = 0; q < 8; ++q) A->prof[blockIdx.x * 8 + q] = tacc[q];
        if (blockIdx.x == 0) { A->prof[2048 + 126] = (long long)__builtin_amdgcn_s_memtime() - clk0; A->prof[2048 + 127] = (long long)__builtin_amdgcn_s_memrealtime() - rt0; }
    }
#endif
}
#undef RS_K
#undef RS_TROW
#undef RS_TST1
#undef RS_TLD1
#undef RS_XST1
#undef RS_XZROW
#undef RS_XZ1
#undef RS_XLD1
#undef RS_XALL
#undef RS_XROW
#undef RS_CLOBBERS
#undef RS_CLOB4
#undef RS_SWEEP
#undef RS_WAIT
#undef RS_BATCH
#undef RS_FP1
#undef RS_IDX
#undef RS_BP1
#undef RS_LD

}
```

### tomo_tv_amd/csrc/tomo_engine.hip

```cpp
#include "../../include/tomo_hip.h"
#include "kernels.hip.h"
#include "sart_resident.hip.h"
#include "sysmat.h"
#include "resident.h"
#include "dev_pool.h"

#include <dlfcn.h>
#if __has_include(<rccl/rccl.h>)
#include <rccl/rccl.h>
#else
#define NCCL_UNIQUE_ID_BYTES 128
typedef struct ncclComm *ncclComm_t;
typedef struct { char internal[NCCL_UNIQUE_ID_BYTES]; } ncclUniqueId;
typedef enum { ncclSuccess = 0 } ncclResult_t;
typedef enum { ncclFloat32 = 7, ncclFloat64 = 8 } ncclDataType_t;
typedef enum { ncclSum = 0 } ncclRedOp_t;
#endif

#include <algorithm>
#include <atomic>
#include <chrono>
#include <cmath>
#include <condition_variable>
#include <functional>
// ... 85 lines not shown
    int nx = 0, n = 0, np = 0, sx = 0, sxc = 0, vec = 1, device = 0;
    int64_t npix = 0, nrows = 0, nnz = 0;
    hipStream_t stream = nullptr;
    bool own_stream = false;
    uint32_t *d_rptr = nullptr;
    uint2 *d_rent = nullptr;
    float *d_rowsum = nullptr, *d_rowinner = nullptr, *d_colsum_all = nullptr, *d_rowcross = nullptr;
    bool art_chain_ok = false;
    int art_chain = 1;
    CellD *d_cell = nullptr;
    uint32_t *d_wptr = nullptr;
    uint2 *d_went = nullptr;
    float lipschitz = 0.f, lipschitz_cimmino = 0.f;
    int sart_fused = 1;
    int tv_lds = 1, fp_all_lpr = 16;
    int tv_recompute = 1, tv_tz = 8;
    int tv_yseg = 0;
    int tv_march4 = 1;
    int tv_halo_fold = -1;
    int gnorm_slot = TOMO_S_GNORM;
    double *gnorm_override = nullptr;
    hipEvent_t ev_peer = nullptr;
    float tv_last_eps = 1e-6f;
    float *tv_alt = nullptr, *halo_lo_alt = nullptr, *halo_hi_alt = nullptr;
    SegItemD *d_seg_exec = nullptr;
    std::vector<uint32_t> h_seg_exec_ptr;
    uint32_t *d_row_first = nullptr, *d_row_nseg = nullptr;
    float *seg_partial = nullptr;
    uint32_t max_items = 0;
    bool seg_ready = false;
    std::vector<double> angles;
    float *sart_alt = nullptr;
    int fp_tile = 1, ft_tiles_z = 0, ft_ntiles = 0;
    uint32_t ft_nseg = 0;
    uint32_t *d_ft_slot_ptr = nullptr, *d_ft_slot_seg0 = nullptr, *d_ft_rsptr = nullptr, *d_ft_rsidx = nullptr;
    uint2 *d_ft_tent = nullptr;
    float *ft_part = nullptr, *ft_part_aux = nullptr;
    int fp_strip = 1, fs_nitems = 0, fs_kused = 0, fs_ncp = 0;
    bool fs_ok = false, attr_fs = false;
    uint32_t fs_nseg = 0;
    FsItemD *d_fs_items = nullptr;
    int *d_fs_orient = nullptr, *d_fs_shift = nullptr;
    uint4 *d_fs_cnt = nullptr;
    uint32_t *d_fs_gstart = nullptr, *d_fs_gseg0 = nullptr, *d_fs_rsptr = nullptr, *d_fs_rsidx = nullptr;
    uint2 *d_fs_ent = nullptr;
    float *d_fs_zero = nullptr;
    float *fs_part = nullptr, *fs_part_aux = nullptr;
    int fp_list = 1, fl_nitems = 0, fl_ncp = 0;
    bool fl_ok = false, attr_fl = false;
    uint32_t fl_nseg = 0;
    FlItemD *d_fl_items = nullptr;
    int *d_fl_orient = nullptr, *d_fl_shift = nullptr;
    uint2 *d_fl_ent = nullptr, *d_fl_fent = nullptr;
    uint32_t *d_fl_ptr = nullptr, *d_fl_fptr = nullptr, *d_fl_rsptr = nullptr, *d_fl_rsidx = nullptr;
    float *d_fl_zero = nullptr, *fl_part = nullptr, *fl_part_aux = nullptr;
    int fp_tile_pipe = 0;
    hipStream_t fp_red_stream[2] = {nullptr, nullptr};
    hipEvent_t ev_fp_tile[2][2] = {{nullptr, nullptr}, {nullptr, nullptr}}, ev_fp_red[2][2] = {{nullptr, nullptr}, {nullptr, nullptr}};
    bool attr_fp = false, attr_bp = false, attr_st = false;
    int sart_streams = 0, sub_c0 = 0, sub_nc = 0;
    static constexpr int MAX_CHAINS = 4;
    hipStream_t sub_stream[MAX_CHAINS] = {nullptr, nullptr, nullptr, nullptr};
    hipEvent_t ev_sfork = nullptr, ev_sjoin[MAX_CHAINS] = {nullptr, nullptr, nullptr, nullptr};
    std::unique_ptr<ChainHelper> chain_helper[MAX_CHAINS];
    int sart_tile = 1;
    bool st_ok = false;
    int st_ntiles = 0, st_tiles_z = 0;
    uint32_t st_max_ids = 0;
    uint4 *d_st_cell = nullptr;
    uint32_t *d_st_win = nullptr, *d_st_segid = nullptr, *d_st_row_first = nullptr, *d_st_row_nseg = nullptr;
    uint2 *d_st_seg = nullptr, *d_st_ent = nullptr;
    float *st_partial = nullptr, *st_partial2 = nullptr;
    uint32_t *st_flags = nullptr;
    uint32_t st_epoch = 0;
    int sart_coop = 0, sart_coop_spin = 4096, st_resident = 0;
    int sart_resident = -1;
    bool rs_ok = false;
    int rs_ntiles = 0, rs_tiles = 0, rs_rpt = 0, rs_groups = 0, rs_cus = 0;
    RsHdrD *d_rs_hdr = nullptr;
    uint4 *d_rs_cell = nullptr;
    uint2 *d_rs_ts = nullptr;
    uint16_t *d_rs_rl = nullptr;
    rs_u64 *rs_pb = nullptr, *rs_rb = nullptr;
    size_t rs_pb_bytes = 0, rs_rb_bytes = 0;
    int *d_rs_angs = nullptr;
    size_t rs_angs_cap = 0;
    std::vector<int> rs_angs_host;
    int *rs_abort = nullptr, *d_rs_abort = nullptr;
    unsigned *d_rs_commit = nullptr;
    int *rs_done = nullptr;
    uint32_t rs_seq = 0, rs_commit_base = 0;
    bool rs_commit_dirty = false;
    size_t table_bytes = 0;
    double create_ms = 0.0;
    int rs_fallbacks = 0, rs_fallback_chunks = 0, rs_skip = 0, rs_backoff = 0, rs_last_code = 0, rs_test_fail = 0;
    uint32_t rs_epoch = 0;
    uint32_t rs_spin_limit = 1u << 21;
    int art_tile = 1;
    int sart_skip_same = 1;
    int sart_nt = -1;
    int bp_tile = 1;
    int bp_list = 1;
    bool attr_bp2 = false, bl_ok = false;
    int bp_list_band = 0;
    uint4 *d_bl_ent = nullptr;
    uint32_t *d_bl_ptr = nullptr, *d_bl_win = nullptr;
    int bl_tiles_z = 0, bl_ntiles = 0;
    bool fb_ok = false;
    uint4 *d_fb_cell = nullptr;
    uint32_t *d_fb_win = nullptr;
    int ft_ncp = 0, ft_ncp_forced = 0;
    size_t ft_scratch_cap = (size_t)8 << 30;
    float *vol[TOMO_VOL_SLOTS] = {};
    float *sino[TOMO_SINO_SLOTS] = {};
    int fgp_target = TOMO_VOL_RECON;
    int tv_target = TOMO_VOL_RECON;
    float *cur_b = nullptr;
    float *cg_p = nullptr, *cg_z = nullptr, *cg_w = nullptr, *fbp_h = nullptr;
    double *cg_sums = nullptr;
    double *cg_part = nullptr;
    float *cg_coef = nullptr;
    float *tvg = nullptr;
    float *fgp_p[3] = {nullptr, nullptr, nullptr};
    float *fgp_q[3] = {nullptr, nullptr, nullptr};
    int fgp_fused = 1;
    int fgp_pair = 1;
    float *pdhg_p[3] = {nullptr, nullptr, nullptr}, *pdhg_alt[4] = {nullptr, nullptr, nullptr, nullptr}, *pdhg_q = nullptr;
    bool pdhg_begun = false;
    float *stage = nullptr;
    size_t stage_bytes = 0;
    double *d_scal = nullptr, *d_scal_own = nullptr, *d_part = nullptr, *d_part_aux = nullptr, *d_part_tv = nullptr;
    double *h_snap = nullptr;
    hipEvent_t ev_snap = nullptr;
    bool snap_pending = false;
    bool part_open[3] = {false, false, false};
    hipStream_t aux = nullptr;
    hipEvent_t ev_fork = nullptr, ev_join = nullptr;
    bool async_pending = false;
    struct CommRef *comm = nullptr;
    int64_t comm_rounds = 0;
    float *comm_send_first = nullptr, *comm_send_last = nullptr, *comm_g_lo = nullptr, *comm_g_hi = nullptr;
    float *comm_fgp = nullptr;
    double *comm_scal = nullptr;
    uint64_t vol_version[TOMO_VOL_SLOTS] = {};
    struct { int vol = -1; uint64_t ver = 0; } g_valid[2];
    int fp_reuse = 1;
    float *g_prev = nullptr;
    float *g_yk = nullptr;
    struct { bool valid = false; uint64_t ver = 0; } yk_claim;
    bool g_prev_valid = false, mom_p_ok = false;
    uint64_t g_prev_recon_ver = 0;
    struct { float beta = 0.f; uint64_t ver_recon = 0, ver_yk = 0, ver_old = 0; bool set = false; } mom;
    bool old_is_recon = false;
    bool geometry_released = false;
    float *halo_lo = nullptr, *halo_hi = nullptr, *halo_lo_own = nullptr, *halo_hi_own = nullptr;
    float *fgp_lo = nullptr, *fgp_hi = nullptr, *fgp_send_first = nullptr, *fgp_send_last = nullptr;
    bool fgp_planes2 = false;
    int is_first = 1, is_last = 1;
    ProfSlot prof[PROF_MAX_KERNELS];
    std::mutex prof_mu;
    size_t vol_elems() const { return (size_t)npix * sx; }
    size_t sino_elems() const { return (size_t)nrows * sx; }
    DevPool pool{pool_alloc, pool_free};
};

static inline double *gnorm_ptr(const tomo_engine *e) { return e->gnorm_override ? e->gnorm_override : e->d_scal + e->gnorm_slot; }

constexpr DevPool::Life GEOMETRY = DevPool::GEOMETRY, COMM = DevPool::COMM, ENGINE = DevPool::ENGINE;
static int dev_alloc(tomo_engine *e, DevPool::Life life, void **p, size_t bytes, bool zero)
{
    if (int rc = e->pool.alloc(life, p, bytes)) return rc;
    if (zero) HIPCHK(hipMemsetAsync(*p, 0, bytes ? bytes : 4, e->stream));
    return TOMO_OK;
}

static void g_clear(tomo_engine *e) { e->g_valid[0].vol = e->g_valid[1].vol = -1; }
static void g_set(tomo_engine *e, int vol) { e->g_valid[0].vol = vol; e->g_valid[0].ver = e->vol_version[vol]; e->g_valid[1].vol = -1; }
static bool g_is_projection_of(const tomo_engine *e, int vol)
{
    if (!e->fp_reuse || vol < 0 || vol >= TOMO_VOL_SLOTS || !e->sino[TOMO_SINO_G]) return false;
    for (int k = 0; k < 2; ++k) if (e->g_valid[k].vol == vol && e->g_valid[k].ver == e->vol_version[vol]) return true;
    return false;
}

static const float *projection_in_hand(const tomo_engine *e, int vol)
{
    if (g_is_projection_of(e, vol)) return e->sino[TOMO_SINO_G];
    if (e->fp_reuse && vol == TOMO_VOL_YK && e->g_yk && e->yk_claim.valid && e->yk_claim.ver == e->vol_version[TOMO_VOL_YK]) return e->g_yk;
    return nullptr;
}

static int get_vol_ro(tomo_engine *e, int id, float **out)
{
    if (id < 0 || id >= TOMO_VOL_SLOTS) return fail(TOMO_ERR_ARG, "bad volume id");
    if (id == TOMO_VOL_RECON_OLD && e->old_is_recon) id = TOMO_VOL_RECON;
    if (!e->vol[id]) { int rc = dev_alloc(e, ENGINE, (void **)&e->vol[id], e->vol_elems() * sizeof(float), true); if (rc) return rc; }
    *out = e->vol[id];
    return TOMO_OK;
}

static int get_vol(tomo_engine *e, int id, float **out)
{
    if (id < 0 || id >= TOMO_VOL_SLOTS) return fail(TOMO_ERR_ARG, "bad volume id");
    ++e->vol_version[id];
    if (e->old_is_recon && (id == TOMO_VOL_RECON || id == TOMO_VOL_RECON_OLD)) {
        e->old_is_recon = false;
        float *src, *dst; int rc;
        if ((rc = get_vol_ro(e, TOMO_VOL_RECON, &src)) || (rc = get_vol_ro(e, TOMO_VOL_RECON_OLD, &dst))) return rc;
        HIPCHK(hipMemcpyAsync(dst, src, e->vol_elems() * sizeof(float), hipMemcpyDeviceToDevice, e->stream));
    }
    return get_vol_ro(e, id, out);
}

static int get_sino(tomo_engine *e, float **slot, float **out)
{
    if (slot == &e->sino[TOMO_SINO_G]) g_clear(e);
    if (!*slot) { int rc = dev_alloc(e, GEOMETRY, (void **)slot, e->sino_elems() * sizeof(float), true); if (rc) return rc; }
    *out = *slot;
    return TOMO_OK;
}

static int sino_slot(tomo_engine *e, int id, float **out)
{
    if (id < 0 || id >= TOMO_SINO_SLOTS) return fail(TOMO_ERR_ARG, "bad sinogram id");
    return get_sino(e, &e->sino[id], out);
}

static int get_scratch(tomo_engine *e, float **slot, float **out)
{
    if (!*slot) { int rc = dev_alloc(e, ENGINE, (void **)slot, e->vol_elems() * sizeof(float), true); if (rc) return rc; }
    *out = *slot;
    return TOMO_OK;
}

static int order_after_async(tomo_engine *e)
{
    if (e->async_pending) HIPCHK(hipStreamWaitEvent(e->stream, e->ev_join, 0));
    return TOMO_OK;
}

static int ensure_stage(tomo_engine *e, size_t bytes)
{
    if (e->stage_bytes >= bytes) return TOMO_OK;
    if (e->stage) { HIPCHK(hipStreamSynchronize(e->stream)); e->pool.release(e->stage); e->stage_bytes = 0; }
    if (int rc = dev_alloc(e, ENGINE, (void **)&e->stage, bytes, false)) return rc;
    e->stage_bytes = bytes;
    return TOMO_OK;
}

struct Sub {
    hipStream_t stream; int c0 = 0, nc = 0;
    int vec = 0;
};
static int sub_vec(const tomo_engine *e, const Sub &sb) { return sb.nc && sb.vec ? sb.vec : e->vec; }
static Sub whole(const tomo_engine *e) { return Sub{e->stream, e->sub_c0, e->sub_nc}; }

struct ProfScope {
    tomo_engine *e; int k; hipEvent_t stop = nullptr; hipStream_t st;
    ProfScope(tomo_engine *e_, int k_, hipStream_t st_ = nullptr, int64_t key = -1) : e(e_), k(k_), st(st_ ? st_ : e_->stream)
    {
        ProfSlot &p = e->prof[k];
        if (!p.on) return;
        hipEvent_t start;
        {
            std::lock_guard<std::mutex> lk(e->prof_mu);
            if (p.stride > 1 && ((key >= 0 ? (uint64_t)key : (uint64_t)p.seen++) % p.stride) != 0) return;
            if (p.used + 2 > p.ev.size()) {
                if (p.ev.size() >= PROF_MAX_EVENTS) { ++p.dropped; return; }
                hipEvent_t a, b;
                if (hipEventCreate(&a) != hipSuccess || hipEventCreate(&b) != hipSuccess) { ++p.dropped; return; }
                p.ev.push_back(a); p.ev.push_back(b);
            }
            start = p.ev[p.used];
            stop = p.ev[p.used + 1];
            p.used += 2;
        }
        (void)hipEventRecord(start, st);
    }
    ~ProfScope() { if (stop) (void)hipEventRecord(stop, st); }
};

static bool &part_open(tomo_engine *e, const double *part)
{
    return part == e->d_part_tv ? e->part_open[2] : part == e->d_part_aux ? e->part_open[1] : e->part_open[0];
}
static int part_begin(tomo_engine *e, double *part)
{
    bool &open = part_open(e, part);
    if (open) HIPCHK(hipMemsetAsync(part, 0, NPART * sizeof(double), e->stream));
    open = true;
    return TOMO_OK;
}
static int part_end(tomo_engine *e, double *part, int slot)
{
    hipLaunchKernelGGL(k_finalize, dim3(1), dim3(NPART), 0, e->stream, part, e->d_scal + slot);
    LAUNCHCHK();
    part_open(e, part) = false;
    return TOMO_OK;
}
static int reduce_begin(tomo_engine *e) { return part_begin(e, e->d_part); }
static int reduce_end(tomo_engine *e, int slot) { return part_end(e, e->d_part, slot); }

constexpr int TV_YSEG_MIN = 8, TV_WAVES_WANTED = 4096;
static int grid_1d(int64_t n4) { int64_t b = (n4 + 255) / 256; return (int)std::min<int64_t>(std::max<int64_t>(b, 1), 4096); }

#include "engine_launch.inc"
#include "engine_create.inc"

extern "C" {

#include "engine_api.inc"
#include "engine_tv.inc"
#include "engine_pdhg.inc"
#include "engine_comm.inc"
#include "engine_options.inc"

}
```

Before: 10.51 Gvoxel-updates/s.

## Alias tracked snapshot volume to swept volume to skip snapshot stores

Adds a lazy snapshot alias: when a SART or TV-march step tracks a copy of the volume it updates, the tracked slot is recorded as an alias of the target instead of being written out. The alias is materialised by a device copy only when another operation needs it. The resident SART kernel and the TV march4 kernel get variants that compute the difference norm without storing the snapshot volume, which removes a full-volume write per step. Per-wave norm partials are also summed in shared memory so each block issues one atomic. This adds bookkeeping complexity and a copy fallback when resident tiles fail.

```diff
diff --git a/tomo_tv_amd/csrc/engine_api.inc b/tomo_tv_amd/csrc/engine_api.inc
--- a/tomo_tv_amd/csrc/engine_api.inc
+++ b/tomo_tv_amd/csrc/engine_api.inc
@@ -117,6 +117,8 @@
     }
     dst->old_is_recon = src->old_is_recon;
     src->old_is_recon = false;
+    dst->snap_slot = src->snap_slot; dst->snap_of = src->snap_of;
+    src->snap_slot = src->snap_of = -1;
     for (int i = 0; i < TOMO_VOL_SLOTS; ++i) ++dst->vol_version[i];
     g_clear(dst);
     return TOMO_OK;
@@ -249,6 +251,7 @@
 {
     NEED(e);
     { int rc_ = order_after_async(e); if (rc_) return rc_; }
+    for (int id : {TOMO_VOL_RECON, TOMO_VOL_YK, TOMO_VOL_RECON_OLD}) { int rc_ = make_snap_real(e, id); if (rc_) return rc_; }
     HIPCHK(hipMemsetAsync(e->vol[TOMO_VOL_RECON], 0, e->vol_elems() * sizeof(float), e->stream));
     if (e->vol[TOMO_VOL_YK]) HIPCHK(hipMemsetAsync(e->vol[TOMO_VOL_YK], 0, e->vol_elems() * sizeof(float), e->stream));
     if (e->vol[TOMO_VOL_RECON_OLD]) HIPCHK(hipMemsetAsync(e->vol[TOMO_VOL_RECON_OLD], 0, e->vol_elems() * sizeof(float), e->stream));
@@ -375,7 +378,7 @@
     if (++e->rs_seq >= 0x7FFFFFF0u) { std::memset(e->rs_done, 0, (size_t)(e->sxc / 64) * sizeof(int)); e->rs_seq = 1; }
     RsArgs A{};
     A.x = x; A.b = e->cur_b; A.rowsum = e->d_rowsum; A.hdr = e->d_rs_hdr; A.cell = e->d_rs_cell; A.ts = e->d_rs_ts; A.rl = e->d_rs_rl;
-    A.pb = e->rs_pb; A.rb = e->rs_rb; A.angs = e->d_rs_angs; A.track = track; A.part = e->d_part; A.abort_word = e->d_rs_abort; A.abort_host = e->rs_abort;
+    A.pb = e->rs_pb; A.rb = e->rs_rb; A.angs = e->d_rs_angs; A.track = track; A.track_is_x = (track != nullptr && track == x) ? 1 : 0; A.part = e->d_part; A.abort_word = e->d_rs_abort; A.abort_host = e->rs_abort;
     A.commit = e->d_rs_commit; A.done_host = e->rs_done; A.seq = e->rs_seq; A.commit_base = e->rs_commit_base; A.test_fail = e->rs_test_fail;
     A.n = e->n; A.sx = e->sx; A.np = e->np; A.ntiles = e->rs_ntiles; A.tiles = e->rs_tiles; A.rpt = e->rs_rpt; A.steps = (int)steps; A.chunk0 = c0; A.nchunk = nc;
     A.epoch0 = e->rs_epoch; A.spin_limit = e->rs_spin_limit; A.beta = beta; A.prof = nullptr;
@@ -426,11 +429,13 @@
 {
     NEED(e);
     float *x, *r, *track = nullptr; int rc;
-    if ((rc = get_vol(e, vol, &x)) || (rc = get_sino(e, &e->sino[TOMO_SINO_R], &r)) || (rc = sino_slot(e, sino_b, &e->cur_b))) return rc;
+    const bool keep_snap = e->snapshot_alias && track_vol >= 0 && track_vol == e->snap_slot && vol == e->snap_of && e->sart_fused && (int64_t)niter * e->np > 0
+                           && select_forms(e).sart == TOMO_FORM_SART_RESIDENT && !(e->rs_skip > 0 && e->sart_resident != 1);
+    if ((rc = (keep_snap ? get_vol_keep_snap : get_vol)(e, vol, &x)) || (rc = get_sino(e, &e->sino[TOMO_SINO_R], &r)) || (rc = sino_slot(e, sino_b, &e->cur_b))) return rc;
     if (track_vol >= 0) {
         if (track_vol == vol) return fail(TOMO_ERR_ARG, "the tracked volume must differ from the swept one");
         if (slot < 0 || slot >= TOMO_S_COUNT) return fail(TOMO_ERR_ARG, "bad scalar slot");
-        if ((rc = get_vol(e, track_vol, &track))) return rc;
+        if ((rc = (keep_snap ? get_vol_keep_snap : get_vol)(e, track_vol, &track))) return rc;
         if ((int64_t)niter * e->np <= 0) {
             if ((rc = tomo_diff_norm_sq(e, vol, track_vol, slot))) return rc;
             return tomo_copy_volume(e, track_vol, vol);
@@ -506,7 +511,15 @@
     if (form == TOMO_FORM_SART_RESIDENT) {
         std::vector<std::pair<int, int>> failed;
         if ((rc = launch_sart_resident(e, x, beta, steps, angle_at, track, failed))) return rc;
-        if (!failed.empty() && (rc = sweep_tiles(&failed))) return rc;
+        if (keep_snap && failed.empty()) ++e->snap_stores_saved;
+        if (!failed.empty()) {
+            if (keep_snap) {
+                e->snap_slot = e->snap_of = -1;
+                if ((rc = get_vol_ro(e, track_vol, &track))) return rc;
+                HIPCHK(hipMemcpyAsync(track, x, e->vol_elems() * sizeof(float), hipMemcpyDeviceToDevice, e->stream));
+            }
+            if ((rc = sweep_tiles(&failed))) return rc;
+        }
         return finish();
     }
     if (e->sart_resident == 1 && !e->rs_ok) return fail(TOMO_ERR_STATE, "\"sart_resident\" = 1, but this engine has no tables of the resident sweep (N not a multiple of 8, more 32 x 32 tiles than CUs, or a matrix whose ray windows do not fit)");
@@ -834,6 +847,7 @@
     e->mom_p_ok = e->g_prev_valid && e->mom.set && e->vol_version[TOMO_VOL_RECON] == e->mom.ver_recon
                   && e->vol_version[TOMO_VOL_RECON_OLD] == e->mom.ver_old && e->g_prev_recon_ver == e->vol_version[TOMO_VOL_RECON];
     float *x, *yk, *old; int rc;
+    for (int id : {TOMO_VOL_RECON, TOMO_VOL_YK, TOMO_VOL_RECON_OLD}) if ((rc = make_snap_real(e, id))) return rc;
     const bool aliased = e->old_is_recon;
     if ((rc = get_vol_ro(e, TOMO_VOL_RECON, &x)) || (rc = get_vol_ro(e, TOMO_VOL_YK, &yk))) return rc;
     if (aliased) old = x;
diff --git a/tomo_tv_amd/csrc/engine_options.inc b/tomo_tv_amd/csrc/engine_options.inc
--- a/tomo_tv_amd/csrc/engine_options.inc
+++ b/tomo_tv_amd/csrc/engine_options.inc
@@ -26,6 +26,9 @@
     if (std::strcmp(name, "table_kib") == 0) { *value = (int)std::min<size_t>(e->table_bytes >> 10, 0x7FFFFFFF); return TOMO_OK; }
     if (std::strcmp(name, "create_ms") == 0) { *value = (int)std::min(e->create_ms + 0.5, 2147483647.0); return TOMO_OK; }
     if (std::strcmp(name, "tv_halo_fold") == 0) { *value = e->tv_halo_fold; return TOMO_OK; }
+    if (std::strcmp(name, "snapshot_alias") == 0) { *value = e->snapshot_alias; return TOMO_OK; }
+    if (std::strcmp(name, "snapshot_alias_set") == 0) { *value = e->snap_slot >= 0 ? 1 : 0; return TOMO_OK; }
+    if (std::strcmp(name, "snapshot_alias_saved") == 0) { *value = e->snap_stores_saved; return TOMO_OK; }
     if (std::strcmp(name, "form_fp") == 0) { *value = select_forms(e).fp; return TOMO_OK; }
     if (std::strcmp(name, "form_bp") == 0) { *value = select_forms(e).bp; return TOMO_OK; }
     if (std::strcmp(name, "form_sart") == 0) { *value = select_forms(e).sart; return TOMO_OK; }
@@ -73,6 +76,7 @@
         e->gnorm_slot = value; return TOMO_OK;
     }
     if (std::strcmp(name, "tv_tz") == 0) { e->tv_tz = value == 4 ? 4 : 8; return TOMO_OK; }
+    if (std::strcmp(name, "snapshot_alias") == 0) { e->snapshot_alias = value ? 1 : 0; return TOMO_OK; }
     if (std::strcmp(name, "tv_halo_fold") == 0) { e->tv_halo_fold = value < 0 ? -1 : (value ? 1 : 0); return TOMO_OK; }
     if (std::strcmp(name, "tv_march4") == 0) { e->tv_march4 = value ? 1 : 0; return TOMO_OK; }
     if (std::strcmp(name, "tv_yseg") == 0) { e->tv_yseg = value < 0 ? 0 : value; return TOMO_OK; }
diff --git a/tomo_tv_amd/csrc/engine_tv.inc b/tomo_tv_amd/csrc/engine_tv.inc
--- a/tomo_tv_amd/csrc/engine_tv.inc
+++ b/tomo_tv_amd/csrc/engine_tv.inc
@@ -135,7 +135,7 @@
 {
     NEED(e);
     float *x, *g; int rc;
-    if ((rc = get_vol(e, e->tv_target, &x))) return rc;
+    if ((rc = get_vol_keep_snap(e, e->tv_target, &x))) return rc;
     if ((rc = get_scratch(e, &e->tvg, &g))) return rc;
     if ((rc = reduce_begin(e))) return rc;
     Halo h{e->halo_lo, e->halo_hi};
@@ -242,12 +242,16 @@
 {
     NEED(e);
     float *x, *g, *track = nullptr; int rc;
-    if ((rc = get_vol(e, e->tv_target, &x))) return rc;
+    const bool out_of_place = e->tv_lds == 1 && e->tv_recompute;
+    const bool single = out_of_place && track_vol >= 0 && e->snapshot_alias && e->tv_tz != 4 && e->tv_march4 && select_forms(e).sart == TOMO_FORM_SART_RESIDENT;
+    const int snap_in = (out_of_place && e->snap_slot >= 0 && e->snap_of == e->tv_target && (track_vol < 0 || (track_vol == e->snap_slot && single))) ? e->snap_slot : -1;
+    if (single && snap_in < 0 && e->snap_slot >= 0 && (rc = make_snap_real(e, e->snap_slot))) return rc;
+    if ((rc = (snap_in >= 0 ? get_vol_keep_snap : get_vol)(e, e->tv_target, &x))) return rc;
     if ((rc = get_scratch(e, &e->tvg, &g))) return rc;
     if (track_vol >= 0) {
         if (track_vol == e->tv_target) return fail(TOMO_ERR_ARG, "the tracked volume must differ from the one descended");
         if (slot < 0 || slot >= TOMO_S_COUNT) return fail(TOMO_ERR_ARG, "bad scalar slot");
-        if ((rc = get_vol(e, track_vol, &track))) return rc;
+        if ((rc = (snap_in >= 0 ? get_vol_keep_snap : get_vol)(e, track_vol, &track))) return rc;
         if ((rc = order_after_async(e))) return rc;
         if ((rc = reduce_begin(e))) return rc;
     }
@@ -269,7 +273,10 @@
             const int tz = e->tv_tz == 4 ? 4 : 8, yseg = tv_rows_per_wave(e, tz);
             dim3 grid(tv_march_grid(e->n, tz, e->sxc / 64, (e->n + yseg - 1) / yseg));
             const bool edge = e->nx % 64 != 0 || e->n % 8 != 0;
-            if (tz == 8 && e->tv_march4) with_flag(edge, [&](auto E) { with_flag(track != nullptr, [&](auto T) { with_flag(up.stream != 0, [&](auto S) {
+            if (tz == 8 && e->tv_march4 && single) with_flag(edge, [&](auto E) { with_flag(up.stream != 0, [&](auto S) {
+                hipLaunchKernelGGL((k_tv_march4<8, false, TVM_UPDATE, E(), true, S(), false>), grid, dim3(256), 0, e->stream, x, h, e->d_part, e->tv_last_eps, e->n, e->nx, e->sx, yseg, (double *)nullptr, up);
+            }); });
+            else if (tz == 8 && e->tv_march4) with_flag(edge, [&](auto E) { with_flag(track != nullptr, [&](auto T) { with_flag(up.stream != 0, [&](auto S) {
                 hipLaunchKernelGGL((k_tv_march4<8, false, TVM_UPDATE, E(), T(), S()>), grid, dim3(256), 0, e->stream, x, h, e->d_part, e->tv_last_eps, e->n, e->nx, e->sx, yseg, (double *)nullptr, up);
             }); }); });
             else with_int<4, 8>(tz, [&](auto TZ) {
@@ -278,6 +285,11 @@
         }
         LAUNCHCHK();
         e->vol[e->tv_target] = alt; e->tv_alt = x;
+        if (snap_in >= 0 && !single) {
+            e->tv_alt = e->vol[snap_in]; e->vol[snap_in] = x;
+            e->snap_slot = e->snap_of = -1;
+        }
+        if (single) { e->snap_slot = track_vol; e->snap_of = e->tv_target; ++e->snap_stores_saved; }
         if (wrap && own_halo) { e->halo_lo = wl; e->halo_hi = wh; }
         else if (wrap) { if ((rc = tomo_halo_local(e, e->tv_target))) return rc; }
         if (fold) { e->halo_lo = up.ho_lo; e->halo_hi = up.ho_hi; }
diff --git a/tomo_tv_amd/csrc/kernels_fp.hip.h b/tomo_tv_amd/csrc/kernels_fp.hip.h
--- a/tomo_tv_amd/csrc/kernels_fp.hip.h
+++ b/tomo_tv_amd/csrc/kernels_fp.hip.h
@@ -395,7 +395,8 @@
     int64_t item = ((int64_t)blockIdx.x * 4 + wave) * R + grp;
     int row = (int)(item / spans), span = (int)(item - (int64_t)row * spans);
     bool valid = row < nrows;
-    if (!__any(valid)) return;
+    constexpr bool SUMS = MODE == FP_DD || MODE == FP_POISSON;
+    if (!SUMS && !__any(valid)) return;
     if (!valid) row = 0;
     uint32_t kb = rsptr[row], ke = valid ? rsptr[row + 1] : kb;
     const float *pp = part + (size_t)span * (LPR * 4) + gl * 4;
@@ -445,10 +446,7 @@
             *reinterpret_cast<V *>(out + o) = r;
         }
     }
-    if (MODE == FP_DD || MODE == FP_POISSON) {
-        local = wave_sum(local);
-        if (lane == 0) atomicAdd(&dpart[blockIdx.x & (NPART - 1)], local);
-    }
+    if (SUMS) block_accumulate(local, dpart);
 }
 
 template <int MODE>
diff --git a/tomo_tv_amd/csrc/kernels_tv.hip.h b/tomo_tv_amd/csrc/kernels_tv.hip.h
--- a/tomo_tv_amd/csrc/kernels_tv.hip.h
+++ b/tomo_tv_amd/csrc/kernels_tv.hip.h
@@ -480,7 +480,7 @@
 #define TV4_UPD_WAVES 4
 #endif
 #define TV4_OCC __attribute__((amdgpu_waves_per_eu((MODE == TVM_UPDATE && !TRACK) ? TV4_UPD_WAVES : 4, (MODE == TVM_UPDATE && !TRACK) ? TV4_UPD_WAVES : 8)))
-template <int TZ, bool WITH_TV, int MODE, bool EDGE, bool TRACK = false, bool STREAM = false>
+template <int TZ, bool WITH_TV, int MODE, bool EDGE, bool TRACK = false, bool STREAM = false, bool TSNAP = true>
 __global__ __launch_bounds__(256) TV4_OCC void k_tv_march4(const float *__restrict__ x, Halo h, double *__restrict__ part, float eps,
                                                     int n, int nx, int sx, int yseg, double *__restrict__ part_tv, TvUpd up)
 {
@@ -682,6 +682,7 @@
                     for (int j = 1; j <= TZ; ++j) {
                         float d = out[j] - told[j];
                         acc += (double)(d * d);
+                        if (!TSNAP) continue;
                         if (EDGE && !(z0 + j - 1 < n && s < nx)) continue;
                         if constexpr (SOFF) st_so<STREAM>(tr, vb[j], out[j]);
                         else if (STREAM) __builtin_nontemporal_store(out[j], tr_e + (size_t)(j - 1) * sx + (unsigned)lane);
diff --git a/tomo_tv_amd/csrc/sart_resident.hip.h b/tomo_tv_amd/csrc/sart_resident.hip.h
--- a/tomo_tv_amd/csrc/sart_resident.hip.h
+++ b/tomo_tv_amd/csrc/sart_resident.hip.h
@@ -24,6 +24,7 @@
     int *done_host;
     unsigned seq, commit_base;
     int test_fail;
+    int track_is_x;
     int n, sx, np, ntiles, tiles, rpt, steps, chunk0, nchunk;
     unsigned epoch0, spin_limit;
     float beta;
@@ -137,6 +138,18 @@
     "s_add_u32 s36, s36, %[rs]\n" "s_addc_u32 s37, s37, 0\n"                                              \
     "s_add_u32 s38, s38, %[rs]\n" "s_addc_u32 s39, s39, 0\n"                                              \
     "s_add_u32 s40, s40, %[rs]\n" "s_addc_u32 s41, s41, 0\n"
+#define RS_AST1(R, C)                                                                                     \
+    "v_sub_f32 v48, v[64+8*" #R "+" #C "], v[49+" #C "]\n"                                                \
+    "v_mul_f32 v48, v48, v48\n"                                                                           \
+    "v_cvt_f64_f32 v[58:59], v48\n"                                                                       \
+    "v_add_f64 %[sum], %[sum], v[58:59]\n"                                                                \
+    "global_store_dword %[voff], v[64+8*" #R "+" #C "], s[36:37]\n" "s_add_u32 s36, s36, %[ps]\n" "s_addc_u32 s37, s37, 0\n"
+#define RS_AROW(R)                                                                                        \
+    RS_TLD1(0) RS_TLD1(1) RS_TLD1(2) RS_TLD1(3) RS_TLD1(4) RS_TLD1(5) RS_TLD1(6) RS_TLD1(7)               \
+    "s_waitcnt vmcnt(0)\n"                                                                                \
+    RS_AST1(R, 0) RS_AST1(R, 1) RS_AST1(R, 2) RS_AST1(R, 3) RS_AST1(R, 4) RS_AST1(R, 5) RS_AST1(R, 6) RS_AST1(R, 7) \
+    "s_add_u32 s36, s36, %[rs]\n" "s_addc_u32 s37, s37, 0\n"                                              \
+    "s_add_u32 s38, s38, %[rs]\n" "s_addc_u32 s39, s39, 0\n"
 
 #define RS_K __attribute__((address_space(4)))
 typedef const RS_K RsArgs *RsArgsP;
@@ -168,8 +181,10 @@
     __shared__ float rs_sbuf[RS_WAVES][64];
     __shared__ float rs_dump[RS_WAVES][64];
     __shared__ int rs_dirty, rs_go, rs_store;
+    __shared__ double rs_norm[RS_WAVES];
     const int lane = threadIdx.x & 63;
     const int wave = __builtin_amdgcn_readfirstlane(threadIdx.x >> 6);
+    if (lane == 0) rs_norm[wave] = 0.0;
     v32f xlo, xhi;
     v16f rr;
 #ifdef RS_PROF
@@ -406,6 +421,18 @@
             if (A->track) {
                 float *tb = A->track + o0;
                 double local = 0.0;
+                if (A->track_is_x)
+                    asm volatile("s_cmp_eq_u32 %[in], 0\n"
+                                 "s_cbranch_scc1 1f\n"
+                                 "s_mov_b64 s[36:37], %[xb]\n"
+                                 "s_mov_b64 s[38:39], %[xb]\n"
+                                 RS_AROW(0) RS_AROW(1) RS_AROW(2) RS_AROW(3) RS_AROW(4) RS_AROW(5) RS_AROW(6) RS_AROW(7)
+                                 "s_waitcnt vmcnt(0)\n"
+                                 "1:\n"
+                                 : [sum] "+v"(local)
+                                 : "{v[64:95]}"(xlo), "{v[96:127]}"(xhi), [in] "s"(in), [xb] "s"(xb), [voff] "v"(voff), [ps] "s"(ps), [rs] "s"(rs)
+                                 : "s36", "s37", "s38", "s39", "v48", "v49", "v50", "v51", "v52", "v53", "v54", "v55", "v56", "v58", "v59", "scc", "memory");
+                else
                 asm volatile("s_cmp_eq_u32 %[in], 0\n"
                              "s_cbranch_scc1 1f\n"
                              "s_mov_b64 s[36:37], %[xb]\n"
@@ -423,9 +450,7 @@
                 if (lane == 0) {
                     local = 0.0;
                     for (int l = 0; l < 64; ++l) local += red[l];
-                    const uint32_t slot = (blockIdx.x & (NPART - 1)) * 8u;
-                    double *part = A->part;
-                    asm volatile("global_atomic_add_f64 %0, %1, %2" :: "v"(slot), "v"(local), "s"(part) : "memory");
+                    rs_norm[wave] += local;
                 }
             } else {
                 asm volatile("s_cmp_eq_u32 %[in], 0\n"
@@ -440,6 +465,16 @@
             }
         }
     }
+    if (rs_args()->track) {
+        __syncthreads();
+        if (threadIdx.x == 0) {
+            double local = 0.0;
+            for (int w = 0; w < RS_WAVES; ++w) local += rs_norm[w];
+            const uint32_t slot = (blockIdx.x & (NPART - 1)) * 8u;
+            double *part = rs_args()->part;
+            asm volatile("global_atomic_add_f64 %0, %1, %2" :: "v"(slot), "v"(local), "s"(part) : "memory");
+        }
+    }
 #ifdef RS_PROF
     if (threadIdx.x == 0) {
         RsArgsP A = rs_args();
@@ -449,6 +484,8 @@
 #endif
 }
 #undef RS_K
+#undef RS_AROW
+#undef RS_AST1
 #undef RS_TROW
 #undef RS_TST1
 #undef RS_TLD1
diff --git a/tomo_tv_amd/csrc/tomo_engine.hip b/tomo_tv_amd/csrc/tomo_engine.hip
--- a/tomo_tv_amd/csrc/tomo_engine.hip
+++ b/tomo_tv_amd/csrc/tomo_engine.hip
@@ -261,6 +261,8 @@
     uint64_t g_prev_recon_ver = 0;
     struct { float beta = 0.f; uint64_t ver_recon = 0, ver_yk = 0, ver_old = 0; bool set = false; } mom;
     bool old_is_recon = false;
+    int snapshot_alias = 1, snap_slot = -1, snap_of = -1;
+    int snap_stores_saved = 0;
     bool geometry_released = false;
     float *halo_lo = nullptr, *halo_hi = nullptr, *halo_lo_own = nullptr, *halo_hi_own = nullptr;
     float *fgp_lo = nullptr, *fgp_hi = nullptr, *fgp_send_first = nullptr, *fgp_send_last = nullptr;
@@ -303,22 +305,48 @@
 {
     if (id < 0 || id >= TOMO_VOL_SLOTS) return fail(TOMO_ERR_ARG, "bad volume id");
     if (id == TOMO_VOL_RECON_OLD && e->old_is_recon) id = TOMO_VOL_RECON;
+    if (id == e->snap_slot) id = e->snap_of;
     if (!e->vol[id]) { int rc = dev_alloc(e, ENGINE, (void **)&e->vol[id], e->vol_elems() * sizeof(float), true); if (rc) return rc; }
     *out = e->vol[id];
     return TOMO_OK;
 }
 
-static int get_vol(tomo_engine *e, int id, float **out)
-{
-    if (id < 0 || id >= TOMO_VOL_SLOTS) return fail(TOMO_ERR_ARG, "bad volume id");
-    ++e->vol_version[id];
+static int make_old_real(tomo_engine *e, int id)
+{
     if (e->old_is_recon && (id == TOMO_VOL_RECON || id == TOMO_VOL_RECON_OLD)) {
         e->old_is_recon = false;
         float *src, *dst; int rc;
         if ((rc = get_vol_ro(e, TOMO_VOL_RECON, &src)) || (rc = get_vol_ro(e, TOMO_VOL_RECON_OLD, &dst))) return rc;
         HIPCHK(hipMemcpyAsync(dst, src, e->vol_elems() * sizeof(float), hipMemcpyDeviceToDevice, e->stream));
     }
+    return TOMO_OK;
+}
+
+static int make_snap_real(tomo_engine *e, int id)
+{
+    if (e->snap_slot < 0 || (id != e->snap_slot && id != e->snap_of)) return TOMO_OK;
+    const int s = e->snap_slot, o = e->snap_of;
+    e->snap_slot = e->snap_of = -1;
+    float *src, *dst; int rc;
+    if ((rc = get_vol_ro(e, o, &src)) || (rc = get_vol_ro(e, s, &dst))) return rc;
+    HIPCHK(hipMemcpyAsync(dst, src, e->vol_elems() * sizeof(float), hipMemcpyDeviceToDevice, e->stream));
+    if (id == o) std::swap(e->vol[s], e->vol[o]);
+    return TOMO_OK;
+}
+
+static int get_vol_keep_snap(tomo_engine *e, int id, float **out)
+{
+    if (id < 0 || id >= TOMO_VOL_SLOTS) return fail(TOMO_ERR_ARG, "bad volume id");
+    ++e->vol_version[id];
+    if (int rc = make_old_real(e, id)) return rc;
     return get_vol_ro(e, id, out);
+}
+
+static int get_vol(tomo_engine *e, int id, float **out)
+{
+    if (id < 0 || id >= TOMO_VOL_SLOTS) return fail(TOMO_ERR_ARG, "bad volume id");
+    if (int rc = make_snap_real(e, id)) return rc;
+    return get_vol_keep_snap(e, id, out);
 }
 
 static int get_sino(tomo_engine *e, float **slot, float **out)
```

Measured after the change: 10.61 Gvoxel-updates/s, median of 6. No clear change (+0.9%).
